# swacisko/ALGA

Measured on AMD Instinct MI355X. Metric: overlap_edges_per_sec, higher is better.
Workload: dtype u32; 1 GPU; cfg4_50M_150bp: 50000000 x 150 bp reads, genome 250000000, seed 11, err 0.00 -> 90621096 nodes (both strands, duplicates removed), min_overlap 82, rsoemo 116; generated on the device (alga_amd.workload.device_build) in 0.9 s; nodes=90621096, edges=92350115

## Files before the change

alga_amd/csrc/engine.hip:

```cpp
#include <hip/hip_runtime.h>

#include <algorithm>
#include <chrono>
#include <cstdio>
#include <cstdlib>
#include <cstring>
#include <new>
#include <string>
#include <thread>
#include <vector>

#include "engine_internal.h"
#include "prefsuf_shard.h"

using namespace alga;

namespace {

using Prepared = AlgaPrepared;

int prepare(alga_engine *e, const alga_nodes *nodes, const alga_prefsuf_params *p, hipStream_t s, Prepared &out) {
    if (!nodes || !p) return alga_fail(e, ALGA_ERR_INVALID_ARGUMENT, "nodes/params must not be NULL");
    if (nodes->n < 0) return alga_fail(e, ALGA_ERR_INVALID_ARGUMENT, "negative node count");
    if (nodes->n > 0 && (!nodes->words || !nodes->len)) return alga_fail(e, ALGA_ERR_INVALID_ARGUMENT, "words/len must not be NULL");
    if (nodes->stride_words <= 0 && nodes->n > 0) return alga_fail(e, ALGA_ERR_INVALID_ARGUMENT, "stride_words must be positive");
    if (p->min_overlap < 1 || p->min_overlap > 501) return alga_fail(e, ALGA_ERR_INVALID_ARGUMENT, "min_overlap must be in [1, 501]");
    if (p->soes != 3) return alga_fail(e, ALGA_ERR_INVALID_ARGUMENT, "soes must be 3 (the reference hard-codes SOES = 3)");
    if (p->max_len_cap < 1 || p->max_len_cap > 500) return alga_fail(e, ALGA_ERR_INVALID_ARGUMENT, "max_len_cap must be in [1, 500]");
    if (p->rsoe_min_overlap < 0) return alga_fail(e, ALGA_ERR_INVALID_ARGUMENT, "rsoe_min_overlap must be >= 0");
    if (p->keys_shared < 0 || p->keys_shared > 2) return alga_fail(e, ALGA_ERR_INVALID_ARGUMENT, "keys_shared must be 0, 1 or 2");
    int rc;
    if ((rc = alga_ensure(e, e->counters, (CNT_TOTAL + 2) * sizeof(unsigned long long)))) return rc;
    HIP_TRY(e, hipMemsetAsync(e->counters.p, 0, (CNT_TOTAL + 2) * sizeof(unsigned long long), s));
    NodesDev nd;
    nd.words = nodes->words; nd.len = nodes->len; nd.from = nodes->align_from; nd.to = nodes->align_to;
    nd.n = nodes->n; nd.stride = nodes->stride_words;
    unsigned long long *cnt = (unsigned long long *) e->counters.p;
    int *d_maxlen = (int *) (cnt + CNT_TOTAL);
    unsigned long long mask_asym = 0;
    int min_len = 0;
    if (p->keys_shared == 2 && e->store_n == nodes->n && e->store_words == (const void *) nodes->words && e->stat_len == (const void *) nodes->len &&
        e->stat_from == (const void *) nodes->align_from && e->stat_to == (const void *) nodes->align_to) {
        out.max_len = e->stat_max_len; out.live = e->stat_live; mask_asym = e->stat_mask_asym; min_len = e->stat_min_len;
    } else {
        launch_node_stats(nd, cnt, d_maxlen, s);
        if ((rc = alga_check_launch(e, "k_node_stats"))) return rc;
        HIP_TRY(e, hipMemcpyAsync(e->h_counters, e->counters.p, (CNT_TOTAL + 2) * sizeof(unsigned long long), hipMemcpyDeviceToHost, s));
        HIP_TRY(e, hipStreamSynchronize(s));
        out.max_len = (int) (e->h_counters[CNT_TOTAL] & 0xFFFFFFFFull);
        min_len = out.max_len > 0 ? 0x7FFFFFFF - (int) (e->h_counters[CNT_TOTAL] >> 32) : 0;
        out.live = e->h_counters[CNT_LIVE_NODES];
        mask_asym = e->h_counters[CNT_MASK_ASYM];
        e->stat_max_len = out.max_len; e->stat_min_len = min_len; e->stat_live = out.live; e->stat_mask_asym = mask_asym;
        e->stat_len = (const void *) nodes->len; e->stat_from = (const void *) nodes->align_from; e->stat_to = (const void *) nodes->align_to;
    }
    out.nd = nd;
    out.uniform_len = (out.max_len > 0 && min_len == out.max_len && !nodes->align_from) ? out.max_len : 0;
    if ((int64_t) blocks_of(out.max_len) > (int64_t) nodes->stride_words)
        return alga_fail(e, ALGA_ERR_INVALID_ARGUMENT, "stride_words is smaller than the longest read needs");
    if (out.max_len > OL_MAX_NODE_LEN) return alga_fail(e, ALGA_ERR_CAPACITY, "a node is longer than 4 194 303 nt (overlap records keep the offset in 22 bits)");
    PrefSufCfg c;
    c.Lmin = p->min_overlap;
    c.rsoemo = p->rsoe_min_overlap;
    c.Lcap = std::min(out.max_len, p->max_len_cap) + 1;
    c.soes = p->soes;
    const int seed_nt = std::min(c.Lmin, SEED_MAX_NT);
    c.seed_words = (2 * seed_nt + 31) >> 5;
    c.seed_last_mask = (2 * seed_nt & 31) ? ((1u << (2 * seed_nt & 31)) - 1u) : 0xFFFFFFFFu;
    c.reversed = (c.rsoemo > c.Lcap) ? 1 : 0;
    c.stats = p->collect_stats ? 1 : 0;
    out.cfg = c;
    if (p->reduction < ALGA_REDUCTION_AUTO || p->reduction > ALGA_REDUCTION_SOURCE_SIDE)
        return alga_fail(e, ALGA_ERR_INVALID_ARGUMENT, "reduction must be an alga_reduction value");
    out.local_ok = out.max_len <= p->max_len_cap && out.max_len - c.Lmin <= LOCAL_MAX_SPAN && c.Lmin <= c.rsoemo && c.rsoemo <= c.Lcap &&
                   mask_asym == 0;
    out.local_sw = out.max_len - c.Lmin <= 63 ? 1 : 2;
    out.cluster_eq = 0;
    const bool wide = out.local_sw == 2 || blocks_of(out.max_len) > 13;
    if (out.local_ok && e->opt_probe != ALGA_PROBE_TABLE && !(wide && e->opt_probe == ALGA_PROBE_AUTO && out.live < (4ull << 20))) {
        int eq = 0;
        if (cluster_plan(c, out.max_len, out.live, e->opt_cluster_bucket_bias, &out.cluster, &eq)) out.cluster_eq = eq;
    }
    out.keys_shared = p->keys_shared;
    out.reduction = p->reduction;
    if (out.reduction == ALGA_REDUCTION_AUTO && e->opt_force_per_target) out.reduction = ALGA_REDUCTION_PER_TARGET;
    return ALGA_OK;
}

int cluster_alloc(alga_engine *e, const Prepared &pp) {
    int rc;
    const uint64_t n = (uint64_t) pp.nd.n;
    for (int k = 0; k < 2; k++) {
        if ((rc = alga_ensure(e, e->cl_keys[k], (n + ALGA_KEY_ARRAY_SLACK + 1) * sizeof(uint32_t)))) return rc;
        if ((rc = alga_ensure(e, e->cl_vals[k], (n + 1) * sizeof(uint32_t)))) return rc;
    }
    if ((rc = alga_ensure(e, e->cl_meta, (n + ALGA_KEY_ARRAY_SLACK + 1) * sizeof(uint32_t)))) return rc;
    if ((rc = alga_ensure(e, e->cl_runs, (n + 1) * CL_RMAX * 8))) return rc;
    if ((rc = alga_ensure(e, e->cl_nruns, n + 16))) return rc;
    if ((rc = alga_ensure(e, e->cl_store, (n + 2) * 16 * (size_t) pp.cluster_eq))) return rc;
    if ((rc = alga_ensure(e, e->cl_dir, ((size_t) pp.cluster.n_buckets + 2) * 16))) return rc;
    return alga_ensure(e, e->sort_temp, cluster_sort_temp_bytes(n));
}

int pile_alloc(alga_engine *e, uint64_t n, uint32_t n_buckets, hipStream_t s) {
    int rc;
    if ((rc = alga_ensure(e, e->cl_pile_rec, pile_record_bytes(n)))) return rc;
    if ((rc = alga_ensure(e, e->cl_pile_rec2, pile_record_bytes(n)))) return rc;
    if ((rc = alga_ensure(e, e->cl_pile_succ, ((size_t) n + 64) * 16))) return rc;
    if ((rc = alga_ensure(e, e->cl_pile_cnt, PILE_CNT_WORDS * sizeof(unsigned long long)))) return rc;
    if ((rc = alga_ensure(e, e->cl_pile_own, pile_own_mask_bytes(n)))) return rc;
    if (e->opt_pile_runs_list && (rc = alga_ensure(e, e->cl_pile_list, pile_list_bytes(n)))) return rc;
    if ((rc = alga_ensure(e, e->cl_defer, (size_t) (n + 64) * sizeof(int32_t)))) return rc;
    const void *before = e->cl_pile_tab.p;
    const size_t cap_before = e->cl_pile_tab.cap;
    if ((rc = alga_ensure(e, e->cl_pile_tab, pile_table_bytes(n_buckets)))) return rc;
    if (e->cl_pile_tab.p != before || e->cl_pile_tab.cap != cap_before) {
        HIP_TRY(e, hipMemsetAsync(e->cl_pile_tab.p, 0, e->cl_pile_tab.cap, s));
        HIP_TRY(e, hipStreamSynchronize(s));
        e->pile_epoch = 0;
    }
    return ALGA_OK;
}

int discover_impl(alga_engine *e, const Prepared &pp, int32_t src_begin, int32_t src_end, hipStream_t s, uint64_t *n_rec, bool local = false,
                  bool *overflow = nullptr) {
    int rc;
    const NodesDev &nd = pp.nd;
    const PrefSufCfg &cfg = pp.cfg;
    unsigned long long *cnt = (unsigned long long *) e->counters.p;
    *n_rec = 0;
    HIP_TRY(e, hipEventRecord(e->ev[EV_START], s));
    if (pp.live >= (1ull << 31)) return alga_fail(e, ALGA_ERR_CAPACITY, "too many nodes for one seed table; shard the input");
    const bool clustered = local && pp.cluster_eq != 0;
    e->pairs_timed = false;
    e->store_timed = false;
    e->pile_timed = false;
    e->pile_deg_pending = false;
    const bool all_sources = src_begin == 0 && src_end == pp.nd.n;
    const bool pile_index_left = e->opt_pile_range != 0 && e->pile_n == pp.nd.n && e->pile_words == (const void *) pp.nd.words;
    bool pile = clustered && e->opt_pile != 0 && e->opt_cluster_pairs != 0 && e->opt_cluster_order != 0 && pp.local_sw == 1 &&
                      (pp.keys_shared == 0 || (pp.keys_shared == 2 && pile_index_left)) &&
                      (all_sources || (e->opt_pile_range != 0 && src_begin >= 0 && src_end <= pp.nd.n && src_begin < src_end)) && pile_plan(cfg, pp.cluster, pp.cluster_eq, pp.uniform_len, pp.nd.from != nullptr || pp.nd.to != nullptr);
    e->loc_second_used = false;
    bool keys_only = false;
    const bool need_vals = !e->opt_own_sort || e->opt_test_unsorted_index;
    uint32_t n_buckets = 0, filter_bits = 0;
    bool have_table = false;
    auto build_table = [&]() -> int {
        n_buckets = seed_buckets_for(pp.live, e->seed_fill_x10);
        const size_t table_bytes = (size_t) n_buckets * SEED_BUCKET * sizeof(unsigned long long);
        int r;
        if ((r = alga_ensure(e, e->table, table_bytes))) return r;
        HIP_TRY(e, hipMemsetAsync(e->table.p, 0xFF, table_bytes, s));
        filter_bits = seed_filter_bits_for(pp.live);
        if (filter_bits) {
            if ((r = alga_ensure(e, e->filter, filter_bits / 8))) return r;
            HIP_TRY(e, hipMemsetAsync(e->filter.p, 0, filter_bits / 8, s));
        }
        launch_seed_build(nd, cfg, (unsigned long long *) e->table.p, n_buckets, (uint32_t *) e->filter.p, filter_bits, s);
        if ((r = alga_check_launch(e, "k_seed_build"))) return r;
        e->stats.table_slots = (uint64_t) n_buckets * SEED_BUCKET;
        have_table = true;
        return ALGA_OK;
    };
    ClusterCfg cc{};
    if (clustered) {
        cc = pp.cluster;
        if ((rc = cluster_alloc(e, pp))) return rc;
        if (pp.keys_shared == 2) {
            const bool store_left = e->store_n == nd.n && e->store_words == (const void *) nd.words && e->store_eq == pp.cluster_eq && e->store_buckets == cc.n_buckets;
            const bool piles_serve = pile && e->pile_kept_pure && e->store_buckets == cc.n_buckets && e->store_eq == pp.cluster_eq;
            if (!(store_left || piles_serve) || src_begin < e->store_run_begin || src_end > e->store_run_end)
                return alga_fail(e, ALGA_ERR_INVALID_ARGUMENT, "keys_shared = 2: no entry array of this node set that covers the sources is left from the previous build");
            keys_only = pile && e->pile_keys_only;
        } else {
            int32_t run_begin = 0, run_end = nd.n;
            if (pp.keys_shared == 1) {
                if (e->keyed_n != nd.n || e->keyed_words != (const void *) nd.words || src_begin < e->keyed_begin || src_end > e->keyed_end)
                    return alga_fail(e, ALGA_ERR_INVALID_ARGUMENT, "keys_shared: alga_prefsuf_keys_device has not been called on this node set for a range that covers the sources");
                run_begin = e->keyed_begin; run_end = e->keyed_end;
            } else {
                keys_only = pile && e->opt_pile_runs != 0 && !e->expect_pairwise && !e->opt_pile_check;
                launch_cluster_keys(nd, cfg, cc, 0, nd.n, (uint32_t *) e->cl_keys[0].p, need_vals ? (uint32_t *) e->cl_vals[0].p : nullptr, (uint32_t *) e->cl_meta.p, e->cl_runs.p,
                                    (uint8_t *) e->cl_nruns.p, s, !keys_only);
                if ((rc = alga_check_launch(e, "k_node_runs"))) return rc;
            }
            HIP_TRY(e, hipEventRecord(e->ev[EV_KEYS], s));
            e->keyed_n = -1;
            e->store_n = -1;
            HIP_TRY(e, launch_cluster_sort(nd, cc, (uint32_t *) e->cl_keys[0].p, (uint32_t *) e->cl_vals[0].p, (uint32_t *) e->cl_keys[1].p,
                                           (uint32_t *) e->cl_vals[1].p, e->sort_temp.p, cluster_sort_temp_bytes((uint64_t) nd.n), pp.keys_shared == 1 || !need_vals,
                                           e->ev[EV_SORT], e->opt_test_unsorted_index != 0, s, e->opt_own_sort != 0));
            const bool dir_late = pile && e->opt_pile_dir >= 1;
            e->dir_late = dir_late;
            if (!dir_late) {
                HIP_TRY(e, launch_cluster_dir(nd, cc, (const uint32_t *) e->cl_keys[1].p, e->cl_dir.p, cnt + CNT_TOTAL + 1, nullptr, s));
                HIP_TRY(e, hipEventRecord(e->ev[EV_DIR], s));
            }
            e->pile_n = -1;
            if (pile) {
                rc = e->opt_test_pile_oom ? alga_fail(e, ALGA_ERR_OUT_OF_MEMORY, "pile_alloc (option test_pile_oom)") : pile_alloc(e, (uint64_t) nd.n, cc.n_buckets, s);
                if (rc == ALGA_ERR_OUT_OF_MEMORY) {
                    (void) hipGetLastError();
                    alga_release(e->cl_pile_tab); alga_release(e->cl_pile_rec); alga_release(e->cl_pile_rec2); alga_release(e->cl_pile_succ); alga_release(e->cl_pile_own);
                    alga_release(e->cl_pile_list);
                    e->pile_epoch = 0; e->pile_n = -1;
                    e->err.clear();
                    pile = false;
                    rc = ALGA_OK;
                    if (keys_only) {
                        launch_cluster_keys(nd, cfg, cc, 0, nd.n, (uint32_t *) e->cl_keys[0].p, (uint32_t *) e->cl_vals[0].p, (uint32_t *) e->cl_meta.p, e->cl_runs.p,
                                            (uint8_t *) e->cl_nruns.p, s, true);
                        if ((rc = alga_check_launch(e, "k_node_runs"))) return rc;
                        keys_only = false;
                    }
                } else if (rc) return rc;
            }
            if (pile) {
                launch_pile_sample(nd, cc, pp.uniform_len, (const uint32_t *) e->cl_keys[1].p, (const uint32_t *) e->cl_vals[1].p, e->cl_dir.p,
                                   (unsigned long long *) e->cl_pile_cnt.p, e->opt_pile >= 2 ? e->opt_pile - 1 : 0, s, e->opt_pile_dir >= 1);
                if ((rc = alga_check_launch(e, "k_pile_build<sample>"))) return rc;
            }
            e->pile_tab_index = pile && e->opt_pile_dir >= 2 && e->opt_pile_skip_gather && !cfg.stats;
            if (dir_late) {
                HIP_TRY(e, hipEventRecord(e->ev[EV_SAMPLE], s));
                HIP_TRY(e, launch_cluster_dir(nd, cc, (const uint32_t *) e->cl_keys[1].p, e->cl_dir.p, cnt + CNT_TOTAL + 1,
                                              e->pile_tab_index ? (const unsigned long long *) e->cl_pile_cnt.p : nullptr, s));
                HIP_TRY(e, hipEventRecord(e->ev[EV_DIR], s));
            }
            HIP_TRY(e, launch_cluster_gather(nd, cc, pp.cluster_eq, (const uint32_t *) e->cl_keys[1].p, (const uint32_t *) e->cl_vals[1].p, (const uint32_t *) e->cl_meta.p,
                                             pp.uniform_len, e->cl_store.p, (pile && e->opt_pile_skip_gather) ? (const unsigned long long *) e->cl_pile_cnt.p : nullptr, s));
            HIP_TRY(e, hipEventRecord(e->ev[EV_GATHER], s));
            if (pile) {
                if (e->pile_epoch >= 511u) {
                    HIP_TRY(e, hipMemsetAsync(e->cl_pile_tab.p, 0, e->cl_pile_tab.cap, s));
                    e->pile_epoch = 0;
                }
                e->pile_epoch++;
                const bool from_consensus = e->opt_pile_runs != 0;
                launch_pile_build(nd, cfg, cc, pp.uniform_len, (const uint32_t *) e->cl_keys[1].p, (const uint32_t *) e->cl_vals[1].p, e->cl_dir.p, e->cl_pile_rec.p, e->cl_pile_rec2.p, e->cl_pile_tab.p,
                                  e->pile_epoch, e->cl_pile_succ.p, e->cl_runs.p, pp.uniform_len - cfg.Lmin + 1, (const unsigned long long *) e->cl_pile_cnt.p,
                                  from_consensus ? (uint32_t *) e->cl_pile_own.p : nullptr, (from_consensus && e->opt_pile_runs_list) ? e->cl_pile_list.p : nullptr, s,
                                  e->opt_pile_dir >= 1, cnt + CNT_TOTAL + 1, e->pile_tab_index, e->opt_pile_runs_ahead != 0);
                if ((rc = alga_check_launch(e, "k_pile_build"))) return rc;
                if (keys_only) {
                    launch_pile_own_ids((const uint32_t *) e->cl_pile_own.p, (const uint32_t *) e->cl_vals[1].p, (uint64_t) nd.n, (int32_t *) e->cl_defer.p, (uint32_t) nd.n,
                                        (unsigned long long *) e->cl_pile_cnt.p, s);
                    launch_cluster_runs_list(nd, cfg, cc, (const int32_t *) e->cl_defer.p, (const unsigned long long *) e->cl_pile_cnt.p + 3, (uint32_t) nd.n, (uint32_t) e->n_cu * 16u,
                                             e->cl_runs.p, (uint8_t *) e->cl_nruns.p, s);
                    launch_cluster_keys(nd, cfg, cc, 0, nd.n, (uint32_t *) e->cl_keys[0].p, (uint32_t *) e->cl_vals[0].p, (uint32_t *) e->cl_meta.p, e->cl_runs.p,
                                        (uint8_t *) e->cl_nruns.p, s, true, (const unsigned long long *) e->cl_pile_cnt.p);
                    if ((rc = alga_check_launch(e, "k_node_runs (own lists)"))) return rc;
                }
                if (e->opt_pile_check && from_consensus)
                    launch_pile_check(e->cl_pile_succ.p, (uint64_t) nd.n, cc.n_buckets, e->cl_pile_tab.p, e->cl_pile_rec2.p, e->pile_epoch, e->cl_runs.p, nd.n, pp.uniform_len - cfg.Lmin + 1,
                                      (unsigned long long *) e->cl_pile_cnt.p, s);
                e->pile_n = nd.n; e->pile_words = (const void *) nd.words;
                e->pile_keys_only = keys_only; e->pile_kept_pure = false;
                e->pile_timed = nd.n > 0;
            }
            e->store_timed = nd.n > 0;
            e->store_n = pile ? -1 : nd.n;
            e->store_words = (const void *) nd.words; e->store_eq = pp.cluster_eq; e->store_buckets = cc.n_buckets;
            e->store_run_begin = run_begin; e->store_run_end = run_end;
        }
        e->stats.table_slots = cc.n_buckets;
    } else if ((rc = build_table())) return rc;
    HIP_TRY(e, hipEventRecord(e->ev[EV_SEED], s));

    const uint64_t n_src = (uint64_t) std::max<int64_t>(0, (int64_t) src_end - src_begin);
    const uint64_t slack = std::max(probe_record_slack(e->n_cu, n_src, local), clustered ? cluster_record_slack(e->n_cu, n_src) : 0);
    uint64_t &hint = local ? e->rec_cap_hint_local : e->rec_cap_hint;
    uint64_t cap = std::max<uint64_t>(hint, (local ? 2 : 16) * n_src + 4096) + slack;
    if (local) {
        if ((rc = alga_ensure(e, e->outdeg, (size_t) (n_src + 1) * sizeof(uint32_t)))) return rc;
        if ((rc = alga_ensure(e, e->loc_first, (size_t) (n_src + 1) * sizeof(unsigned long long)))) return rc;
    }
    const uint32_t big_list_cap = 1u << 20;
    if (local && (rc = alga_ensure(e, e->loc_big_list, big_list_cap * sizeof(int32_t)))) return rc;
    bool pure_streamed = false;
    for (int attempt = 0; attempt < 4; attempt++) {
        if (cap >= (1ull << 32) - 16) return alga_fail(e, ALGA_ERR_CAPACITY, "more than 2^32 overlap records; shard the input");
        if (local) HIP_TRY(e, hipMemsetAsync(e->outdeg.p, 0, (size_t) (n_src + 1) * sizeof(uint32_t), s));
        if ((rc = alga_ensure(e, e->rec_dst, cap * sizeof(uint32_t)))) return rc;
        if ((rc = alga_ensure(e, e->rec_val, cap * sizeof(unsigned long long)))) return rc;
        HIP_TRY(e, hipMemsetAsync(cnt, 0, CNT_TOTAL * sizeof(unsigned long long), s));
        ProbeBig big{(int32_t *) e->loc_big_list.p, big_list_cap, 0u, nullptr, 0u};
        e->defer_list_valid = clustered && e->opt_cluster_pairs && pp.local_sw == 1 && pp.cluster_eq <= 4;
        if (clustered) {
            if (e->opt_cluster_pairs && pp.local_sw == 1 && pp.cluster_eq <= 4) {
                if ((rc = alga_ensure(e, e->cl_defer, (size_t) (n_src + 64) * sizeof(int32_t)))) return rc;
                const uint32_t slot_stride = e->opt_stream_slots >= 4 ? (uint32_t) (n_src + 1) : 0u;
                if ((rc = alga_ensure(e, e->loc_second, (size_t) (slot_stride ? LOCAL_SLOTS_MAX - 1 : 1) * (n_src + 1) * sizeof(unsigned long long)))) return rc;
                e->loc_second_used = true;
                e->loc_slot_stride = slot_stride;
                const bool by_key = e->opt_cluster_order != 0 && src_begin == 0 && src_end == nd.n;
                const bool piled = pile && e->pile_n == nd.n && e->pile_words == (const void *) nd.words;
                if (piled) {
                    if (!all_sources) {
                        if ((rc = alga_ensure(e, e->cl_pile_side_r, (size_t) (n_src + 64) * 16))) return rc;
                        if ((rc = alga_ensure(e, e->cl_pile_cursor, 64))) return rc;
                    }
                    launch_pile_probe(nd, cfg, cc, pp.uniform_len, e->cl_pile_tab.p, e->pile_epoch, e->cl_pile_rec.p, e->cl_pile_rec2.p, e->cl_pile_succ.p,
                                      e->cl_runs.p, cnt, (uint32_t *) e->outdeg.p, (unsigned long long *) e->loc_first.p, (unsigned long long *) e->loc_second.p,
                                      (int32_t *) e->cl_defer.p, (uint32_t) n_src, (const unsigned long long *) e->cl_pile_cnt.p, e->n_cu, s, src_begin, src_end,
                                      e->cl_pile_side_r.p, (unsigned long long *) e->cl_pile_cursor.p, e->opt_pile_probe_lean != 0, e->opt_pile_probe_tail != 0);
                    if ((rc = alga_check_launch(e, "k_pile_probe"))) return rc;
                    if (keys_only)
                        launch_cluster_runs_list(nd, cfg, cc, (const int32_t *) e->cl_defer.p, cnt + CNT_DEFERRED, (uint32_t) std::min<uint64_t>(n_src + 64, 0xFFFFFFFFull),
                                                 (uint32_t) e->n_cu * 16u, e->cl_runs.p, (uint8_t *) e->cl_nruns.p, s);
                }
                launch_probe_stream(nd, cfg, cc, pp.cluster_eq, e->cl_store.p, e->cl_dir.p, e->cl_runs.p, (const uint8_t *) e->cl_nruns.p,
                                    src_begin, src_end, by_key, cnt, e->n_cu, (uint32_t *) e->outdeg.p, (unsigned long long *) e->loc_first.p,
                                    (unsigned long long *) e->loc_second.p, (int32_t *) e->cl_defer.p, (uint32_t) n_src,
                                    piled ? (const unsigned long long *) e->cl_pile_cnt.p : nullptr, s, slot_stride);
                if ((rc = alga_check_launch(e, "k_probe_stream"))) return rc;
                if (piled) {
                    if ((rc = alga_ensure(e, e->cl_defer2, (size_t) (n_src + 64) * sizeof(int32_t)))) return rc;
                    pure_streamed = launch_probe_stream_list(nd, cfg, cc, pp.cluster_eq, e->cl_store.p, e->cl_dir.p, e->cl_runs.p, (const uint8_t *) e->cl_nruns.p, (int32_t *) e->cl_defer.p,
                                             (uint32_t) n_src, cnt, e->n_cu, (uint32_t *) e->outdeg.p, (unsigned long long *) e->loc_first.p,
                                             (unsigned long long *) e->loc_second.p, (int32_t *) e->cl_defer2.p, (const unsigned long long *) e->cl_pile_cnt.p, s, slot_stride, src_begin,
                                             (const uint32_t *) e->cl_keys[1].p, (const uint32_t *) e->cl_vals[1].p, pp.uniform_len, e->opt_pile_stream_by_id != 0,
                                             e->pile_tab_index ? e->cl_pile_tab.p : nullptr, e->pile_epoch);
                    if ((rc = alga_check_launch(e, "k_probe_stream (list)"))) return rc;
                }
                HIP_TRY(e, hipEventRecord(e->ev[EV_PAIRS], s));
                e->pairs_timed = true;
                launch_probe_clustered(nd, cfg, cc, pp.cluster_eq, e->cl_store.p, e->cl_dir.p, e->cl_runs.p, (const uint8_t *) e->cl_nruns.p, 0,
                                       (int32_t) n_src, (const int32_t *) e->cl_defer.p, src_begin, (uint32_t *) e->rec_dst.p, (unsigned long long *) e->rec_val.p,
                                       cap, cnt, e->n_cu, (uint32_t *) e->outdeg.p, (unsigned long long *) e->loc_first.p, &big, cnt + CNT_DEFERRED, 1, s,
                                       (const uint32_t *) e->cl_keys[1].p, (const uint32_t *) e->cl_vals[1].p, pp.uniform_len,
                                       (piled && e->opt_pile_skip_gather) ? (const unsigned long long *) e->cl_pile_cnt.p : nullptr,
                                       (piled && e->pile_tab_index) ? e->cl_pile_tab.p : nullptr, e->pile_epoch);
                e->pile_deg_pending = piled && e->opt_pile_deg_fold != 0;
                if (piled && !e->pile_deg_pending) launch_pile_deg((int32_t) n_src, (unsigned long long *) e->loc_first.p, (uint32_t *) e->outdeg.p, (const unsigned long long *) e->cl_pile_cnt.p, s);
            } else {
                launch_probe_clustered(nd, cfg, cc, pp.cluster_eq, e->cl_store.p, e->cl_dir.p, e->cl_runs.p, (const uint8_t *) e->cl_nruns.p, src_begin,
                                       src_end, nullptr, src_begin, (uint32_t *) e->rec_dst.p, (unsigned long long *) e->rec_val.p, cap, cnt, e->n_cu,
                                       (uint32_t *) e->outdeg.p, (unsigned long long *) e->loc_first.p, &big, nullptr, pp.local_sw, s);
            }
        }
        else
            launch_probe(nd, cfg, (const unsigned long long *) e->table.p, n_buckets, (const uint32_t *) e->filter.p, filter_bits, src_begin, src_end,
                         (uint32_t *) e->rec_dst.p, (unsigned long long *) e->rec_val.p, cap, cnt, e->n_cu, local ? pp.local_sw : 0, (uint32_t *) e->outdeg.p,
                         (unsigned long long *) e->loc_first.p, local ? &big : nullptr, s);
        if ((rc = alga_check_launch(e, "k_probe_sources"))) return rc;
        HIP_TRY(e, hipEventRecord(e->ev[EV_PROBE], s));
        HIP_TRY(e, hipMemcpyAsync(e->h_counters, cnt, (CNT_TOTAL + 2) * sizeof(unsigned long long), hipMemcpyDeviceToHost, s));
        HIP_TRY(e, hipStreamSynchronize(s));
        if (clustered && e->h_counters[CNT_TOTAL + 1] != 0) {
            e->store_n = -1; e->keyed_n = -1;
            return alga_fail(e, ALGA_ERR_HIP, "clustered index: the sorted key array is not in order (entry directory invalid)");
        }
        if (local && e->h_counters[CNT_LOCAL_OVERFLOW] != 0) {
            const uint64_t n_big = e->h_counters[CNT_LOCAL_OVERFLOW], max_items = e->h_counters[CNT_LOCAL_MAXITEMS];
            const uint64_t limit = e->big_limit >= 0 ? (uint64_t) e->big_limit : (uint64_t) local_big_limit();
            if (n_big > big_list_cap || max_items > limit) { if (overflow) *overflow = true; *n_rec = 0; return ALGA_OK; }
            big.count = (uint32_t) n_big;
            big.item_cap = (uint32_t) ((max_items + 63) & ~63ull);
            if ((rc = alga_ensure(e, e->loc_big_items, probe_big_bytes(e->n_cu, big.count, pp.local_sw, big.item_cap)))) return rc;
            big.items = e->loc_big_items.p;
            if (!have_table && (rc = build_table())) return rc;
            if (e->pile_deg_pending) {
                launch_pile_deg((int32_t) n_src, (unsigned long long *) e->loc_first.p, (uint32_t *) e->outdeg.p, (const unsigned long long *) e->cl_pile_cnt.p, s);
                e->pile_deg_pending = false;
            }
            HIP_TRY(e, hipMemsetAsync(cnt + CNT_LOCAL_OVERFLOW, 0, sizeof(unsigned long long), s));
            launch_probe(nd, cfg, (const unsigned long long *) e->table.p, n_buckets, (const uint32_t *) e->filter.p, filter_bits, src_begin, src_end,
                         (uint32_t *) e->rec_dst.p, (unsigned long long *) e->rec_val.p, cap, cnt, e->n_cu, pp.local_sw, (uint32_t *) e->outdeg.p,
                         (unsigned long long *) e->loc_first.p, &big, s);
            if ((rc = alga_check_launch(e, "k_probe_sources (second pass)"))) return rc;
            HIP_TRY(e, hipEventRecord(e->ev[EV_PROBE], s));
            HIP_TRY(e, hipMemcpyAsync(e->h_counters, cnt, CNT_TOTAL * sizeof(unsigned long long), hipMemcpyDeviceToHost, s));
            HIP_TRY(e, hipStreamSynchronize(s));
            if (e->h_counters[CNT_LOCAL_OVERFLOW] != 0) { if (overflow) *overflow = true; *n_rec = 0; return ALGA_OK; }
            e->stats.big_sources = n_big;
        }
        const uint64_t need = e->h_counters[CNT_RECORDS];
        if (need <= cap) {
            *n_rec = need;
            hint = std::max<uint64_t>(hint, need + need / 16 + 4096);
            if (overflow) *overflow = false;
            if (local) { e->stats.transitive_compares = e->h_counters[CNT_TR_COMPARES]; e->stats.generic_sources = e->h_counters[CNT_LOCAL_GENERIC]; }
            e->stats.records = e->h_counters[CNT_VALID_RECORDS];
            e->stats.raw_overlaps = e->h_counters[CNT_RAW];
            e->stats.windows_probed = e->h_counters[CNT_WINDOWS];
            e->stats.slots_scanned = e->h_counters[CNT_SLOTS];
            e->stats.probe_rounds = e->h_counters[CNT_ROUNDS];
            e->stats.pile_buckets = e->h_counters[CNT_PILE_BUCKETS]; e->stats.pile_irregular = e->h_counters[CNT_PILE_IRREGULAR];
            e->stats.pile_own_lists = e->h_counters[CNT_PILE_OWN];
            if (pile && pp.keys_shared != 2 && e->pile_n == nd.n) {
                const bool kept = e->opt_pile == 2 || e->stats.pile_irregular * (uint64_t) ALGA_PILE_DECLINE_ONE_IN <= e->stats.pile_buckets;
                e->stats.pile_mixed = kept && e->stats.pile_irregular * (uint64_t) ALGA_PILE_IRREGULAR_ONE_IN > e->stats.pile_buckets;
                e->stats.pile_deferred = (e->stats.pile_mixed || (kept && pure_streamed)) ? e->h_counters[CNT_DEFERRED_PILE] : (kept ? e->h_counters[CNT_DEFERRED] : 0);
                if (!kept || e->stats.pile_mixed || !e->opt_pile_skip_gather) e->store_n = nd.n;
                e->expect_pairwise = !kept;
                e->pile_kept_pure = kept && !e->stats.pile_mixed && e->opt_pile_skip_gather != 0;
                e->stats.pile_list_checked = 0; e->stats.pile_list_mismatch = 0;
                if (e->opt_pile_check) {
                    unsigned long long chk[2] = {0ull, 0ull};
                    HIP_TRY(e, hipMemcpyAsync(chk, (const unsigned long long *) e->cl_pile_cnt.p + 4, sizeof(chk), hipMemcpyDeviceToHost, s));
                    HIP_TRY(e, hipStreamSynchronize(s));
                    e->stats.pile_list_checked = chk[0]; e->stats.pile_list_mismatch = chk[1];
                }
            }
            if (!pile) e->expect_pairwise = false;
            e->stats.probe_used = clustered ? ALGA_PROBE_CLUSTER : ALGA_PROBE_TABLE;
            if (clustered) e->stats.deferred_sources = e->defer_list_valid ? e->h_counters[CNT_DEFERRED] : n_src;
            return ALGA_OK;
        }
        cap = need + need / 16 + 4096 + slack;
    }
    return alga_fail(e, ALGA_ERR_HIP, "record buffer kept overflowing");
}

int key_bits_for(int64_t n_owned) {
    int b = 1;
    while (b < 31 && (1ll << b) < n_owned) b++;
    return std::min(32, b + 1);
}

int reduce_impl(alga_engine *e, const Prepared &pp, const uint32_t *rec_dst, const unsigned long long *rec_val, uint64_t n_rec,
                uint64_t n_valid_hint, int32_t dst_begin, int32_t dst_end, hipStream_t s, uint64_t *n_edges) {
    int rc;
    const NodesDev &nd = pp.nd;
    const PrefSufCfg &cfg = pp.cfg;
    unsigned long long *cnt = (unsigned long long *) e->counters.p;
    const int32_t n_owned = dst_end - dst_begin;
    *n_edges = 0;
    if (n_rec >= (1ull << 32) - 16) return alga_fail(e, ALGA_ERR_CAPACITY, "more than 2^32 overlap records; shard the input");
    const int bits = key_bits_for(n_owned);
    const size_t temp_bytes = sort_records_temp_bytes(n_rec, bits);
    if ((rc = alga_ensure(e, e->keys, (size_t) (n_rec + 1) * sizeof(uint32_t)))) return rc;
    if ((rc = alga_ensure(e, e->seg_key, (size_t) (n_rec + 1) * sizeof(uint32_t)))) return rc;
    if ((rc = alga_ensure(e, e->seg_val, (size_t) (n_rec + 1) * sizeof(unsigned long long)))) return rc;
    if ((rc = alga_ensure(e, e->sort_temp, temp_bytes))) return rc;
    if ((rc = alga_ensure(e, e->heads, (size_t) (n_rec + 1) * 16))) return rc;
    if ((rc = alga_ensure(e, e->rowptr, (size_t) (n_owned + 2) * sizeof(uint32_t)))) return rc;
    HIP_TRY(e, hipMemsetAsync(cnt + CNT_SORT_VALID, 0, sizeof(unsigned long long), s));
    launch_make_keys(rec_dst, n_rec, dst_begin, dst_end, (uint32_t *) e->keys.p, cnt + CNT_SORT_VALID, s);
    if ((rc = alga_check_launch(e, "k_make_keys"))) return rc;
    HIP_TRY(e, sort_records(e->sort_temp.p, temp_bytes, (const uint32_t *) e->keys.p, (uint32_t *) e->seg_key.p, rec_val,
                            (unsigned long long *) e->seg_val.p, n_rec, bits, s));
    launch_rowptr_from_sorted((const uint32_t *) e->seg_key.p, cnt + CNT_SORT_VALID, n_rec, n_owned, (uint32_t *) e->rowptr.p, s);
    if ((rc = alga_check_launch(e, "k_rowptr_from_sorted"))) return rc;
    launch_gather_heads(nd, (const unsigned long long *) e->seg_val.p, cnt + CNT_SORT_VALID, n_rec, e->heads.p, s);
    if ((rc = alga_check_launch(e, "k_gather_heads"))) return rc;
    HIP_TRY(e, hipEventRecord(e->ev[EV_GROUP], s));

    if ((rc = alga_ensure(e, e->out_cnt, (size_t) (n_owned + 1) * sizeof(uint32_t)))) return rc;
    if ((rc = alga_ensure(e, e->outdeg, (size_t) (nd.n + 1) * sizeof(uint32_t)))) return rc;
    HIP_TRY(e, hipMemsetAsync(e->outdeg.p, 0, (size_t) (nd.n + 1) * sizeof(uint32_t), s));
    const int tpb = reduce_targets_per_block(n_valid_hint, (uint64_t) std::max(1, n_owned));
    launch_reduce_targets(nd, cfg, dst_begin, n_owned, tpb, (const uint32_t *) e->rowptr.p, (unsigned long long *) e->seg_val.p,
                          e->heads.p, (uint32_t *) e->out_cnt.p, (uint32_t *) e->outdeg.p, cnt, s);
    if ((rc = alga_check_launch(e, "k_reduce_targets"))) return rc;
    HIP_TRY(e, hipEventRecord(e->ev[EV_REDUCE], s));

    if ((rc = alga_ensure(e, e->scan_scratch, scan_scratch_bytes((uint64_t) nd.n)))) return rc;
    if ((rc = alga_ensure(e, e->out_rowptr, (size_t) (nd.n + 1) * sizeof(uint32_t)))) return rc;
    launch_exclusive_scan((const uint32_t *) e->outdeg.p, (uint64_t) nd.n, (uint32_t *) e->out_rowptr.p, (uint64_t *) e->scan_scratch.p, s);
    if ((rc = alga_check_launch(e, "scan(outdeg)"))) return rc;
    uint64_t *d_total = (uint64_t *) e->scan_scratch.p + scan_total_index((uint64_t) nd.n);
    HIP_TRY(e, hipMemcpyAsync(&e->h_counters[CNT_TOTAL], d_total, sizeof(uint64_t), hipMemcpyDeviceToHost, s));
    HIP_TRY(e, hipMemcpyAsync(e->h_counters, cnt, CNT_TOTAL * sizeof(unsigned long long), hipMemcpyDeviceToHost, s));
    HIP_TRY(e, hipStreamSynchronize(s));
    const uint64_t E = e->h_counters[CNT_TOTAL];
    if (E >= (1ull << 32) - 16) return alga_fail(e, ALGA_ERR_CAPACITY, "more than 2^32 edges; shard the input");
    if ((rc = alga_ensure(e, e->edges, (size_t) (E + 1) * sizeof(alga_edge_dev)))) return rc;
    launch_scatter_by_source(cfg, dst_begin, n_owned, (const uint32_t *) e->rowptr.p, (const unsigned long long *) e->seg_val.p,
                             (const uint32_t *) e->out_cnt.p, (const uint32_t *) e->out_rowptr.p, (uint32_t *) e->outdeg.p,
                             (alga_edge_dev *) e->edges.p, s);
    if ((rc = alga_check_launch(e, "k_scatter_by_source"))) return rc;
    launch_sort_rows(nd.n, (const uint32_t *) e->out_rowptr.p, (alga_edge_dev *) e->edges.p, s);
    if ((rc = alga_check_launch(e, "k_sort_rows"))) return rc;
    HIP_TRY(e, hipEventRecord(e->ev[EV_EMIT], s));
    HIP_TRY(e, hipStreamSynchronize(s));
    *n_edges = E;
    e->stats.edges = E;
    e->stats.transitive_listed = e->h_counters[CNT_TR_LISTED];
    e->stats.transitive_compares = e->h_counters[CNT_TR_COMPARES];
    e->stats.transitive_removed = e->h_counters[CNT_TR_REMOVED];
    e->stats.max_in_records = e->h_counters[CNT_MAX_IN];
    return ALGA_OK;
}

int finalize_local(alga_engine *e, const Prepared &pp, int32_t src_begin, int32_t src_end, uint64_t n_rec, hipStream_t s, uint64_t *n_edges) {
    int rc;
    *n_edges = 0;
    const uint64_t n_src = (uint64_t) std::max<int64_t>(0, (int64_t) src_end - src_begin);
    if ((rc = alga_ensure(e, e->scan_scratch, scan_scratch_bytes(n_src)))) return rc;
    if ((rc = alga_ensure(e, e->out_rowptr, (size_t) (n_src + 1) * sizeof(uint32_t)))) return rc;
    if ((rc = alga_ensure(e, e->out_cnt, (size_t) (n_src + 1) * sizeof(uint32_t)))) return rc;
    HIP_TRY(e, hipEventRecord(e->ev[EV_GROUP], s));
    HIP_TRY(e, hipEventRecord(e->ev[EV_REDUCE], s));
    const bool fused = e->opt_emit_fused != 0;
    const unsigned long long *pile_cnt = e->pile_deg_pending ? (const unsigned long long *) e->cl_pile_cnt.p : nullptr;
    if (!fused) {
        if (e->pile_deg_pending)
            launch_exclusive_scan_pile_deg((uint32_t *) e->outdeg.p, n_src, (uint32_t *) e->out_rowptr.p, (uint64_t *) e->scan_scratch.p, (unsigned long long *) e->loc_first.p, pile_cnt, s);
        else
            launch_exclusive_scan((const uint32_t *) e->outdeg.p, n_src, (uint32_t *) e->out_rowptr.p, (uint64_t *) e->scan_scratch.p, s);
        if ((rc = alga_check_launch(e, "scan(outdeg)"))) return rc;
    }
    e->pile_deg_pending = false;
    const uint64_t E = e->stats.records;
    if (E >= (1ull << 32) - 16) return alga_fail(e, ALGA_ERR_CAPACITY, "more than 2^32 edges; shard the input");
    if ((rc = alga_ensure(e, e->edges, (size_t) (E + 1) * sizeof(alga_edge_dev)))) return rc;
    launch_local_emit(src_begin, (int32_t) n_src, (const uint32_t *) e->outdeg.p, (const unsigned long long *) e->loc_first.p,
                      e->loc_second_used ? (const unsigned long long *) e->loc_second.p : nullptr, (const uint32_t *) e->rec_dst.p, (const unsigned long long *) e->rec_val.p, n_rec, (uint32_t *) e->out_rowptr.p,
                      (uint32_t *) e->out_cnt.p, (alga_edge_dev *) e->edges.p,
                      e->defer_list_valid ? (const int32_t *) e->cl_defer.p : nullptr, (const unsigned long long *) e->counters.p + CNT_DEFERRED, (uint32_t) n_src, s,
                      e->loc_second_used ? e->loc_slot_stride : 0u, fused ? (uint64_t *) e->scan_scratch.p : nullptr, fused ? pile_cnt : nullptr);
    if ((rc = alga_check_launch(e, "k_local_emit"))) return rc;
    HIP_TRY(e, hipEventRecord(e->ev[EV_EMIT], s));
    uint64_t *d_total = (uint64_t *) e->scan_scratch.p + scan_total_index(n_src);
    HIP_TRY(e, hipMemcpyAsync(&e->h_counters[CNT_TOTAL], d_total, sizeof(uint64_t), hipMemcpyDeviceToHost, s));
    HIP_TRY(e, hipStreamSynchronize(s));
    if (e->h_counters[CNT_TOTAL] != E) return alga_fail(e, ALGA_ERR_HIP, "source-side emit: out-degrees and edge count disagree");
    *n_edges = E;
    e->stats.edges = E;
    return ALGA_OK;
}

int build_local(alga_engine *e, const Prepared &pp, int32_t src_begin, int32_t src_end, hipStream_t s, uint64_t *n_edges) {
    if (!pp.local_ok) return alga_fail(e, ALGA_ERR_UNSUPPORTED, "source-side reduction is not exact for this input (read lengths / masks / rsoemo)");
    uint64_t n_rec = 0;
    bool overflow = false;
    int rc = discover_impl(e, pp, src_begin, src_end, s, &n_rec, true, &overflow);
    if (rc) return rc;
    if (overflow) return alga_fail(e, ALGA_ERR_UNSUPPORTED, "a source node has more raw overlaps than the source-side reduction holds");
    if ((rc = finalize_local(e, pp, src_begin, src_end, n_rec, s, n_edges))) return rc;
    e->stats.reduction_used = ALGA_REDUCTION_SOURCE_SIDE;
    return ALGA_OK;
}

double now_ms_host() { return std::chrono::duration<double, std::milli>(std::chrono::steady_clock::now().time_since_epoch()).count(); }

float ev_ms(alga_engine *e, int a, int b) {
    float ms = 0.f;
    if (hipEventElapsedTime(&ms, e->ev[a], e->ev[b]) != hipSuccess) return 0.f;
    return ms;
}

void store_phase_stats(alga_engine *e) {
    if (!e->store_timed) return;
    e->stats.ms_keys = ev_ms(e, EV_START, EV_KEYS);
    e->stats.ms_sort = ev_ms(e, EV_KEYS, EV_SORT);
    e->stats.ms_dir = ev_ms(e, e->dir_late ? EV_SAMPLE : EV_SORT, EV_DIR);
    e->stats.ms_gather = ev_ms(e, EV_DIR, EV_GATHER) + (e->dir_late ? ev_ms(e, EV_SORT, EV_SAMPLE) : 0.0);
    e->stats.ms_pile = e->pile_timed ? ev_ms(e, EV_GATHER, EV_SEED) : 0.0;
}

}

int alga_prepare(alga_engine *e, const alga_nodes *nodes, const alga_prefsuf_params *p, hipStream_t s, AlgaPrepared &out) { return prepare(e, nodes, p, s, out); }
int alga_cluster_alloc(alga_engine *e, const AlgaPrepared &pp) { return cluster_alloc(e, pp); }

extern "C" {

int alga_abi_version(void) { return ALGA_AMD_ABI_VERSION; }

struct DeviceGuard {
    int prev = -1;
    DeviceGuard() { if (hipGetDevice(&prev) != hipSuccess) prev = -1; }
    ~DeviceGuard() { if (prev >= 0) (void) hipSetDevice(prev); }
};

static void engine_free_handles(alga_engine *e) {
    if (e->h_counters) (void) hipHostFree(e->h_counters);
    for (int i = 0; i < EV_COUNT; i++) if (e->ev[i]) (void) hipEventDestroy(e->ev[i]);
    if (e->own_stream) (void) hipStreamDestroy(e->own_stream);
    if (e->side_stream) (void) hipStreamDestroy(e->side_stream);
    if (e->ev_side) (void) hipEventDestroy(e->ev_side);
    e->h_counters = nullptr; e->own_stream = nullptr; e->side_stream = nullptr; e->ev_side = nullptr;
    for (int i = 0; i < EV_COUNT; i++) e->ev[i] = nullptr;
}

int alga_engine_create(int hip_device, alga_engine **out) {
    if (!out) return ALGA_ERR_INVALID_ARGUMENT;
    *out = nullptr;
    int ndev = 0;
    hipError_t err = hipGetDeviceCount(&ndev);
    if (err != hipSuccess || ndev <= 0) return ALGA_ERR_NO_DEVICE;
    if (hip_device < 0 || hip_device >= ndev) return ALGA_ERR_INVALID_ARGUMENT;
    DeviceGuard guard;
    if (hipSetDevice(hip_device) != hipSuccess) return ALGA_ERR_NO_DEVICE;
    alga_engine *e = new (std::nothrow) alga_engine();
    if (!e) return ALGA_ERR_OUT_OF_MEMORY;
    e->device = hip_device;
    memset(&e->stats, 0, sizeof(e->stats));
    hipDeviceProp_t prop;
    if (hipGetDeviceProperties(&prop, hip_device) == hipSuccess) {
        snprintf(e->dev_name, sizeof(e->dev_name), "%s (%s, %d CUs)", prop.name, prop.gcnArchName, prop.multiProcessorCount);
        if (prop.multiProcessorCount > 0) e->n_cu = prop.multiProcessorCount;
    }
    int rc = ALGA_OK;
    if (hipStreamCreateWithFlags(&e->own_stream, hipStreamNonBlocking) != hipSuccess) { e->own_stream = nullptr; rc = ALGA_ERR_HIP; }
    if (rc == ALGA_OK && hipStreamCreateWithFlags(&e->side_stream, hipStreamNonBlocking) != hipSuccess) { e->side_stream = nullptr; rc = ALGA_ERR_HIP; }
    if (rc == ALGA_OK && hipEventCreateWithFlags(&e->ev_side, hipEventDisableTiming) != hipSuccess) { e->ev_side = nullptr; rc = ALGA_ERR_HIP; }
    for (int i = 0; i < EV_COUNT && rc == ALGA_OK; i++)
        if (hipEventCreate(&e->ev[i]) != hipSuccess) { e->ev[i] = nullptr; rc = ALGA_ERR_HIP; }
    if (rc == ALGA_OK && hipHostMalloc((void **) &e->h_counters, (CNT_TOTAL + 2 + alga_engine::H_EXTRA) * sizeof(unsigned long long)) != hipSuccess) { e->h_counters = nullptr; rc = ALGA_ERR_OUT_OF_MEMORY; }
    if (rc == ALGA_OK && hipHostGetDevicePointer((void **) &e->h_counters_dev, e->h_counters, 0) != hipSuccess) rc = ALGA_ERR_HIP;
    if (rc != ALGA_OK) { engine_free_handles(e); delete e; return rc; }
    *out = e;
    return ALGA_OK;
}

void alga_engine_destroy(alga_engine *e) {
    if (!e) return;
    DeviceGuard guard;
    (void) hipSetDevice(e->device);
    if (e->own_stream) (void) hipStreamSynchronize(e->own_stream);
    if (e->side_stream) (void) hipStreamSynchronize(e->side_stream);
    for (DevBuf *b : e->owned) alga_release(*b);
    alga_release(e->up_raw);
    for (DevBuf *b : {&e->in_bytes[0], &e->in_bytes[1], &e->in_nl[0], &e->in_nl[1], &e->in_tiles, &e->in_tile_off}) alga_release(*b);
    for (DevBuf *b : {&e->sp_rowptr, &e->sp_sorted, &e->sp_list, &e->sp_cnt, &e->sp_orow, &e->sp_out, &e->sp_in}) alga_release(*b);
    alga_staging_release(e);
    for (void *&p : e->gfa_pin) { if (p) (void) hipHostFree(p); p = nullptr; }
    for (auto &kv : e->host_lists) free(kv.first);
    e->host_lists.clear();
    engine_free_handles(e);
    delete e;
}

const char *alga_last_error(const alga_engine *e) { return e ? e->err.c_str() : "no engine"; }

int alga_engine_device_name(const alga_engine *e, char *buf, size_t buflen) {
    if (!e || !buf || buflen == 0) return ALGA_ERR_INVALID_ARGUMENT;
    snprintf(buf, buflen, "%s", e->dev_name);
    return ALGA_OK;
}

int alga_engine_set_option(alga_engine *e, const char *name, int64_t value) {
    if (!e || !name) return ALGA_ERR_INVALID_ARGUMENT;
    e->err.clear();
    if (!strcmp(name, "probe")) {
        if (value < ALGA_PROBE_AUTO || value > ALGA_PROBE_CLUSTER) return alga_fail(e, ALGA_ERR_INVALID_ARGUMENT, "option probe: 0 auto, 1 table, 2 cluster");
        e->opt_probe = (int) value;
    } else if (!strcmp(name, "cluster_bucket_bias")) {
        if (value < -8 || value > 8) return alga_fail(e, ALGA_ERR_INVALID_ARGUMENT, "option cluster_bucket_bias: -8 .. 8");
        e->opt_cluster_bucket_bias = (int) value;
    } else if (!strcmp(name, "cluster_pairs")) {
        e->opt_cluster_pairs = value != 0;
    } else if (!strcmp(name, "pile")) {
        e->opt_pile = (value == 2 || value == 3) ? (int) value : (value != 0);
    } else if (!strcmp(name, "pile_runs")) {
        e->opt_pile_runs = value != 0;
    } else if (!strcmp(name, "pile_runs_list")) {
        e->opt_pile_runs_list = value != 0;
    } else if (!strcmp(name, "pile_dir")) {
        if (value < 0 || value > 2) return alga_fail(e, ALGA_ERR_INVALID_ARGUMENT, "option pile_dir: 0 directory records, 1 k_pile_build from the keys, 2 ... and no directory for a pure pile build");
        e->opt_pile_dir = (int) value;
    } else if (!strcmp(name, "pile_deg_fold")) {
        e->opt_pile_deg_fold = value != 0;
    } else if (!strcmp(name, "emit_fused")) {
        e->opt_emit_fused = value != 0;
    } else if (!strcmp(name, "pile_probe_lean")) {
        e->opt_pile_probe_lean = value != 0;
    } else if (!strcmp(name, "pile_probe_tail")) {
        e->opt_pile_probe_tail = value != 0;
    } else if (!strcmp(name, "pile_runs_ahead")) {
        e->opt_pile_runs_ahead = value != 0;
    } else if (!strcmp(name, "pile_stream_by_id")) {
        e->opt_pile_stream_by_id = value != 0;
    } else if (!strcmp(name, "pile_check")) {
        e->opt_pile_check = value != 0;
    } else if (!strcmp(name, "pile_skip_gather")) {
        e->opt_pile_skip_gather = value != 0;
    } else if (!strcmp(name, "cluster_order")) {
        e->opt_cluster_order = value != 0;
    } else if (!strcmp(name, "local_big_max")) {
        e->big_limit = value < 0 ? -1 : (int) std::min<int64_t>(value, 1 << 20);
    } else if (!strcmp(name, "shard_bucket_max")) {
        e->opt_shard_dmax = (int) std::max<int64_t>(1, std::min<int64_t>(value, 4096));
    } else if (!strcmp(name, "rsort_variant")) {
        if (value < 0 || value > 1) return alga_fail(e, ALGA_ERR_INVALID_ARGUMENT, "option rsort_variant: 0 tiles of 8192 pairs, 1 tiles of 16384 pairs");
        rsort_set_variant((int) value);
    } else if (!strcmp(name, "stream_slots")) {
        e->opt_stream_slots = value >= 4 ? 4 : 2;
    } else if (!strcmp(name, "pile_range")) {
        e->opt_pile_range = value != 0;
    } else if (!strcmp(name, "pkb_legacy")) {
        e->opt_pkb_legacy = (int) value;
    } else if (!strcmp(name, "own_sort")) {
        e->opt_own_sort = value != 0;
    } else if (!strcmp(name, "test_presort_oom")) {
        e->opt_test_presort_oom = value != 0;
    } else if (!strcmp(name, "test_pile_oom")) {
        e->opt_test_pile_oom = value != 0;
    } else if (!strcmp(name, "test_unsorted_index")) {
        e->opt_test_unsorted_index = value != 0;
    } else if (!strcmp(name, "gfa_chunk_mb")) {
        if (value < 1 || value > 4096) return alga_fail(e, ALGA_ERR_INVALID_ARGUMENT, "option gfa_chunk_mb: 1 .. 4096");
        e->opt_gfa_chunk_mb = (int) value;
    } else if (!strcmp(name, "mst_mid_nodes")) {
        if (value < 8 || value > (1 << 20)) return alga_fail(e, ALGA_ERR_INVALID_ARGUMENT, "option mst_mid_nodes: 8 .. 2^20");
        e->opt_mst_mid_nodes = (int) value;
    } else if (!strcmp(name, "consensus_max_blocks")) {
        if (value < 0 || value > (1 << 20)) return alga_fail(e, ALGA_ERR_INVALID_ARGUMENT, "option consensus_max_blocks: 0 .. 2^20");
        e->opt_consensus_max_blocks = (int) value;
    } else if (!strcmp(name, "unitig_ruling")) {
        if (value < -1 || value > 1) return alga_fail(e, ALGA_ERR_INVALID_ARGUMENT, "option unitig_ruling: -1, 0 or 1");
        e->opt_unitig_ruling = (int) value;
    } else if (!strcmp(name, "correct_slice_keys")) {
        if (value < 1 || value > (1ll << 31)) return alga_fail(e, ALGA_ERR_INVALID_ARGUMENT, "option correct_slice_keys: 1 .. 2^31");
        e->opt_correct_slice_keys = value;
    } else if (!strcmp(name, "correct_dir_bits")) {
        if (value < 0 || value > 28) return alga_fail(e, ALGA_ERR_INVALID_ARGUMENT, "option correct_dir_bits: 0 (auto) or 1 .. 28");
        e->opt_correct_dir_bits = (int) value;
    } else if (!strcmp(name, "place_dir_bits")) {
        if (value < 0 || value > 26) return alga_fail(e, ALGA_ERR_INVALID_ARGUMENT, "option place_dir_bits: 0 (auto) or 1 .. 26");
        e->opt_place_dir_bits = (int) value;
    } else if (!strcmp(name, "auto_reduction_per_target")) {
        e->opt_force_per_target = value != 0;
    } else return alga_fail(e, ALGA_ERR_INVALID_ARGUMENT, "unknown option");
    return ALGA_OK;
}

int alga_engine_reserve(alga_engine *e, int32_t n_nodes, int32_t max_len, int32_t min_overlap, uint64_t n_edges_hint) {
    if (!e) return ALGA_ERR_INVALID_ARGUMENT;
    e->err.clear();
    if (n_nodes < 0 || max_len < 1 || min_overlap < 1) return alga_fail(e, ALGA_ERR_INVALID_ARGUMENT, "alga_engine_reserve: n_nodes >= 0, max_len >= 1, min_overlap >= 1");
    DeviceGuard guard;
    HIP_TRY(e, hipSetDevice(e->device));
    int rc;
    const uint64_t n = (uint64_t) n_nodes;
    const uint64_t E = n_edges_hint ? n_edges_hint : n + n / 16 + 4096;
    if ((rc = alga_ensure(e, e->counters, (CNT_TOTAL + 2) * sizeof(unsigned long long)))) return rc;
    Prepared pp;
    pp.nd.n = n_nodes; pp.max_len = max_len; pp.live = n;
    pp.cfg.Lmin = min_overlap; pp.cfg.Lcap = std::min(max_len, 500) + 1; pp.cfg.rsoemo = min_overlap; pp.cfg.soes = 3;
    int eq = 0;
    const bool local = max_len <= 500 && max_len - min_overlap <= LOCAL_MAX_SPAN;
    const bool clustered = local && e->opt_probe != ALGA_PROBE_TABLE &&
                           cluster_plan(pp.cfg, max_len, n, e->opt_cluster_bucket_bias, &pp.cluster, &eq);
    if (clustered) {
        pp.cluster_eq = eq;
        if ((rc = cluster_alloc(e, pp))) return rc;
        if (max_len - min_overlap <= 63 && eq <= 4) {
            if ((rc = alga_ensure(e, e->cl_defer, (size_t) (n + 64) * sizeof(int32_t)))) return rc;
            if ((rc = alga_ensure(e, e->loc_second, (size_t) (e->opt_stream_slots >= 4 ? LOCAL_SLOTS_MAX - 1 : 1) * (n + 1) * sizeof(unsigned long long)))) return rc;
        }
        if (e->opt_pile != 0 && e->opt_cluster_pairs != 0 && e->opt_cluster_order != 0 && max_len - min_overlap <= 63 && pile_plan(pp.cfg, pp.cluster, eq, max_len, false)) {
            if ((rc = pile_alloc(e, n, pp.cluster.n_buckets, e->own_stream))) return rc;
        }
    } else {
        const uint32_t nb = seed_buckets_for(n, e->seed_fill_x10);
        if ((rc = alga_ensure(e, e->table, (size_t) nb * SEED_BUCKET * sizeof(unsigned long long)))) return rc;
        const uint32_t fb = seed_filter_bits_for(n);
        if (fb && (rc = alga_ensure(e, e->filter, fb / 8))) return rc;
    }
    if (local) {
        const uint64_t slack = std::max(probe_record_slack(e->n_cu, n, true), clustered ? cluster_record_slack(e->n_cu, n) : 0);
        const uint64_t cap = std::max<uint64_t>(e->rec_cap_hint_local, 2 * n + 4096) + slack;
        if ((rc = alga_ensure(e, e->outdeg, (size_t) (n + 1) * sizeof(uint32_t)))) return rc;
        if ((rc = alga_ensure(e, e->loc_first, (size_t) (n + 1) * sizeof(unsigned long long)))) return rc;
        if ((rc = alga_ensure(e, e->loc_big_list, (1u << 20) * sizeof(int32_t)))) return rc;
        if ((rc = alga_ensure(e, e->rec_dst, cap * sizeof(uint32_t)))) return rc;
        if ((rc = alga_ensure(e, e->rec_val, cap * sizeof(unsigned long long)))) return rc;
        if ((rc = alga_ensure(e, e->scan_scratch, scan_scratch_bytes(n)))) return rc;
        if ((rc = alga_ensure(e, e->out_rowptr, (size_t) (n + 1) * sizeof(uint32_t)))) return rc;
        if ((rc = alga_ensure(e, e->out_cnt, (size_t) (n + 1) * sizeof(uint32_t)))) return rc;
    }
    if ((rc = alga_ensure(e, e->edges, (size_t) (E + 1) * sizeof(alga_edge_dev)))) return rc;
    if (!e->warmed && n_nodes > 0) {
        const int W = blocks_of(max_len), stride = hbm_row_stride(W), wn = 4096;
        std::vector<uint32_t> rows((size_t) wn * stride, 0u);
        std::vector<int32_t> lens((size_t) wn, max_len);
        uint64_t x = 0x9E3779B97F4A7C15ull;
        for (int i = 0; i < wn; i++)
            for (int k = 0; k < W; k++) {
                x ^= x << 13; x ^= x >> 7; x ^= x << 17;
                uint32_t w = (uint32_t) (x >> 16);
                const int used = 2 * max_len - 32 * k;
                if (used < 32) w &= used <= 0 ? 0u : ((1u << used) - 1u);
                rows[(size_t) i * stride + k] = w;
            }
        void *d_rows = nullptr, *d_len = nullptr;
        if (hipMalloc(&d_rows, rows.size() * 4) == hipSuccess && hipMalloc(&d_len, lens.size() * 4) == hipSuccess &&
            hipMemcpy(d_rows, rows.data(), rows.size() * 4, hipMemcpyHostToDevice) == hipSuccess &&
            hipMemcpy(d_len, lens.data(), lens.size() * 4, hipMemcpyHostToDevice) == hipSuccess) {
            alga_nodes nd{(const uint32_t *) d_rows, stride, (const int32_t *) d_len, wn, nullptr, nullptr};
            alga_prefsuf_params wp;
            alga_prefsuf_default_params(&wp);
            wp.min_overlap = min_overlap; wp.rsoe_min_overlap = std::min(max_len, min_overlap + (max_len - min_overlap) / 2);
            const alga_edge *d = nullptr;
            uint64_t m = 0;
            const int wrc = alga_prefsuf_build_device(e, &nd, &wp, nullptr, &d, &m);
            (void) wrc;
            e->err.clear();
            e->warmed = true;
        }
        if (d_rows) (void) hipFree(d_rows);
        if (d_len) (void) hipFree(d_len);
        (void) hipGetLastError();
        alga_forget_node_set(e);
        memset(&e->stats, 0, sizeof(e->stats));
    }
    return ALGA_OK;
}

void alga_prefsuf_default_params(alga_prefsuf_params *p) {
    if (!p) return;
    memset(p, 0, sizeof(*p));
    p->min_overlap = 0;
    p->rsoe_min_overlap = 0;
    p->soes = 3;
    p->max_len_cap = 500;
    p->collect_stats = 0;
// ... 605 lines not shown
```

alga_amd/csrc/engine_internal.h:

```cpp
#pragma once
#include <hip/hip_runtime.h>

#include <cstdio>
#include <algorithm>
#include <string>
#include <vector>
#include <unordered_map>

#include "../../include/alga_amd.h"
#include "prefsuf_common.h"
#include "prefsuf_kernels.h"
#include "pkb_kernels.h"

struct DevBuf {
    void  *p = nullptr;
    size_t cap = 0;
};

enum { EV_START = 0, EV_SEED, EV_PROBE, EV_GROUP, EV_REDUCE, EV_EMIT, EV_PAIRS, EV_KEYS, EV_SORT, EV_GATHER, EV_DIR, EV_SAMPLE, EV_COUNT };
constexpr int ALGA_STAGE_THREADS = 8;

struct alga_engine {
    std::vector<DevBuf *> owned;
    int         device = -1;
    hipStream_t own_stream = nullptr;
    hipStream_t side_stream = nullptr;
    hipEvent_t  ev_side = nullptr;
    std::string err;
    char        dev_name[256] = {0};
    int         n_cu = 256;
    int         seed_fill_x10 = 20;
    int         opt_probe = 0;
    int         opt_cluster_bucket_bias = 0;
    int         opt_force_per_target = 0;
    int         opt_shard_dmax = 4096;
    int         opt_test_unsorted_index = 0;
    hipEvent_t  ev[EV_COUNT] = {};
    DevBuf table, filter, counters, rowptr, rec_dst, rec_val, keys, seg_key, seg_val, heads, sort_temp, out_cnt, outdeg, out_rowptr, edges, scan_scratch;
    DevBuf cl_defer;
    uint32_t h_first_hkey = 255;
    int32_t keyed_n = -1, keyed_begin = 0, keyed_end = 0;
    bool defer_list_valid = false;
    const void *keyed_words = nullptr;
    int32_t store_n = -1, store_run_begin = 0, store_run_end = 0, store_eq = 0;
    uint32_t store_buckets = 0;
    const void *store_words = nullptr;
    int stat_max_len = 0, stat_min_len = 0; uint64_t stat_live = 0; unsigned long long stat_mask_asym = 0;
    const void *stat_len = nullptr, *stat_from = nullptr, *stat_to = nullptr;
    bool   warmed = false;
    bool   pairs_timed = false;
    bool   store_timed = false;
    bool   pile_keys_only = false, pile_kept_pure = false;
    int    opt_pile_range = 1;
    int    opt_pile_skip_gather = 1;
    int    opt_pile = 1;
    int    opt_pile_runs = 1;
    int    opt_pile_runs_list = 1;
    DevBuf cl_pile_list;
    int    opt_pile_deg_fold = 1;
    int    opt_emit_fused = 1;
    int    opt_pile_dir = 2;
    bool   dir_late = false;
    bool   pile_tab_index = false;
    int    opt_pile_stream_by_id = 0;
    int    opt_pile_probe_lean = 1;
    int    opt_pile_probe_tail = 1;
    int    opt_pile_runs_ahead = 0;
    bool   pile_deg_pending = false;
    int    opt_pile_check = 0;
    bool   expect_pairwise = false;
    DevBuf cl_pile_side_r, cl_pile_cursor;
    DevBuf cl_pile_own;
    int    opt_pkb_legacy = 0;
    int    opt_own_sort = 1;
    int    opt_test_presort_oom = 0;
    int    opt_test_pile_oom = 0;
    bool   pile_timed = false;
    DevBuf cl_pile_succ;
    DevBuf cl_pile_rec2;
    DevBuf cl_pile_rec, cl_pile_cnt, cl_pile_tab;
    uint32_t pile_epoch = 0;
    int32_t pile_n = -1; const void *pile_words = nullptr;
    int    opt_cluster_order = 1;
    int    opt_cluster_pairs = 1;
    DevBuf cl_keys[2], cl_vals[2], cl_meta, cl_runs, cl_nruns, cl_store, cl_dir;
    DevBuf loc_second;
    bool   loc_second_used = false;
    uint32_t loc_slot_stride = 0;
    int    opt_stream_slots = 4;
    DevBuf loc_first, loc_big_list, loc_big_items;
    int    big_limit = -1;
    DevBuf edge_keys, edge_keys2, edge_vals, edge_vals2, edges_sorted, xs_dst, xs_val;
    DevBuf up_words, up_len, up_from, up_to;
    DevBuf up_len_narrow;
    DevBuf cp_deg, cp_dst, cp_off;
    DevBuf cl_defer2;
    DevBuf pk_keys, pk_keys2, pk_vals, pk_vals2, pk_marks, pk_big, pk_add, pk_ekeys, pk_ekeys2, pk_flag, pk_pos, pk_edges[2], pk_rowptr, pk_deg,
           pk_mask, pk_cnt, pk_io, pk_io2, pk_tips, pk_heads, pk_g[2], pk_addk, pk_addk2, pk_merged, pk_hsz, pk_hsz2, pk_heads2, pk_nadd, pk_koff,
           pk_gsz, pk_fixlist, pk_bounds, pk_tiprec, pk_tipidx, pk_keys_all, pk_vals_all;
    DevBuf pk_keys2b, pk_vals2b, pk_headsb, pk_hszb, sort_temp2, pk_fixlist2, pk_cnt2;
    DevBuf pp_rows, pp_len, pp_perm[2], pp_keys[2], pp_mark, pp_keep, pp_pos, pp_out_rows, pp_out_len, pp_out_pair, pp_tally;
    bool        stage_ready = false;
    void       *stage_pin[ALGA_STAGE_THREADS][2] = {};
    hipEvent_t  stage_ev[ALGA_STAGE_THREADS][2] = {};
    hipStream_t stage_stream[ALGA_STAGE_THREADS] = {};
    DevBuf      up_raw;
    std::unordered_map<void *, size_t> host_lists;
    void       *host_spare = nullptr;
    size_t      host_spare_cap = 0;
    DevBuf      in_bytes[2], in_nl[2], in_tiles, in_tile_off;
    DevBuf      sp_rowptr, sp_sorted, sp_list, sp_cnt, sp_orow, sp_out, sp_in;
    DevBuf      tp_cnt, tp_keys[2], tp_vals[2], tp_flag, tp_pos, tp_best, tp_est, tp_rev, tp_rfid, tp_rowptr[2], tp_alive, tp_kill, tp_rec[2], tp_branch,
                tp_overflow, tp_ws, tp_out;
    DevBuf      mp_cnt, mp_rowptr, mp_rows, mp_len, mp_owner, mp_pend[2], mp_win, mp_overflow, mp_overflow2, mp_ws, mp_ws_big, mp_orow, mp_out;
    struct MstFilled { const void *p = nullptr; size_t bytes = 0; uint32_t hbits = 0, cap_nodes = 0, cap_edges = 0; int32_t n_ws = 0; } mp_filled[2];
    int         opt_mst_mid_nodes = 4096;
    DevBuf      gfa_sizes, gfa_off, gfa_rowptr, gfa_tiles, gfa_bounds, gfa_buf;
    void       *gfa_pin[2] = {nullptr, nullptr};
    size_t      gfa_pin_cap = 0;
    int         opt_gfa_chunk_mb = 256;
    DevBuf      ut_cnt, ut_keys[2], ut_vals[2], ut_flag, ut_pos, ut_best, ut_estar, ut_rowptr, ut_nxt, ut_noff, ut_prv, ut_rank[2], ut_min[2], ut_tail,
                ut_win, ut_pair, ut_pcnt, ut_ulen, ut_ulen2, ut_uwords, ut_path_off, ut_word_off, ut_tiles, ut_path_node, ut_path_pos, ut_uid, ut_words,
                ut_edges, ut_link, ut_rnode, ut_rrec[2];
    int         opt_unitig_ruling = -1;
    uint64_t    ut_n_pairs = 0, ut_n_edges = 0;
    bool        ut_valid = false;
    int32_t     ut_n_nodes = 0;
    uint64_t    ut_total_bases = 0;
    bool        ut_is_contig = false;
    DevBuf      ex_cnt, ex_rowptr, ex_w, ex_kcnt, ex_dlink, ex_outcnt, ex_sole, ex_xhead, ex_xbase, ex_xrank, ex_uid, ex_scnt, ex_seam_off,
                ex_seam_entry, ex_pcnt, ex_uwords, ex_ulen, ex_ulen2, ex_path_off, ex_word_off, ex_path_node, ex_path_pos, ex_words, ex_edges;
    bool        ut_is_extended = false;
    DevBuf      ct_cnt, ct_B[2], ct_rowptr, ct_pflag, ct_runkey, ct_chain, ct_headchain, ct_drop, ct_flag, ct_pos, ct_keys[2], ct_vals[2], ct_hw, ct_hk, ct_H,
                ct_hrow, ct_hsorted, ct_hlist, ct_hcnt, ct_win, ct_pair, ct_oid, ct_cid, ct_deg, ct_epos, ct_ekeys[2], ct_evals[2], ct_names;
    DevBuf      cs_cnt, cs_words, cs_mask, cs_votes, cs_trim, cs_len, cs_changed;
    bool        cs_valid = false;
    bool        cs_has_votes = false;
    DevBuf      fc_cnt, fc_keys[2], fc_vals, fc_first, fc_min, fc_list[2], fc_flag, fc_ids, fc_verdict, fc_rank, fc_id, fc_new, fc_trim, fc_begin, fc_len,
                fc_order, fc_wbegin, fc_wlen, fc_rows, fc_rlen, fc_tid;
    bool        fc_valid = false;
    uint64_t    fc_n_accepted = 0;
    int         opt_consensus_max_blocks = 0;
    DevBuf      cr_cnt, cr_table, cr_hist, cr_keys[2], cr_flag, cr_pos, cr_solid, cr_dir;
    int64_t     opt_correct_slice_keys = 1ll << 28;
    int         opt_correct_dir_bits = 0;
    DevBuf      seed_keys[2], seed_vals[2], seed_dir, seed_ub;
    DevBuf      pl_cnt, pl_fbegin, pl_flen, pl_scan, pl_cols, pl_diff;
    DevBuf      pl_target, pl_pos, pl_mm, pl_hits, pl_state, pl_coloff, pl_cover, pl_tstat, pl_hist;
    bool        pl_valid = false;
    uint64_t    pl_targets = 0, pl_reads = 0;
    uint64_t    pl_ncolumns = 0, pl_nhist = 0;
    uint64_t    pl_final_epoch = 0;
    uint64_t    fc_epoch = 0;
    int         opt_place_dir_bits = 0;
    DevBuf      po_cnt, po_keys[2], po_vals[2], po_marks, po_pop, po_scan;
    DevBuf      po_coloff, po_words, po_ccols, po_cbases, po_tstat, po_counts;
    bool        po_valid = false;
    uint64_t    po_targets = 0, po_columns = 0;
    uint64_t    po_final_epoch = 0;
    uint64_t    pl_serial = 0, po_pl_serial = 0;
    DevBuf      sc_cnt, sc_keys[2], sc_vals[2], sc_span, sc_heads, sc_pos, sc_bstart, sc_best, sc_choice, sc_partner, sc_lists[2], sc_head, sc_first, sc_scan;
    DevBuf      sc_ba, sc_bb, sc_blinks, sc_bspan, sc_bgap, sc_bstate, sc_estate, sc_scaffold, sc_rank, sc_orient, sc_start, sc_gapafter, sc_jlinks, sc_soff,
                sc_smembers, sc_slen;
    bool        sc_valid = false;
    uint64_t    sc_targets = 0, sc_scaffolds = 0, sc_longest = 0;
    uint64_t    sc_pl_serial = 0;
    DevBuf      br_cnt, br_diff, br_starts, br_rpos, br_marks, br_rfirst, br_rlast, br_closed, br_cpos;
    DevBuf      br_span, br_ccols, br_cfirst, br_clast, br_tcuts, br_poff, br_begin, br_len, br_ptarget, br_pstart, br_words;
    bool        br_valid = false;
    uint64_t    br_targets = 0, br_pieces = 0, br_cuts = 0, br_columns = 0, br_longest = 0;
    DevBuf      gr_cnt, gr_flag, gr_pos, gr_cand, gr_elen, gr_eoff, gr_ecols, gr_x, gr_g;
    struct GrowSet { DevBuf end, over, mm, hits, state, count, estop, evoters, left, right, len, coloff, begin, words; } gr_set[2];
    int         gr_cur = 0;
    bool        gr_valid = false;
    uint64_t    gr_reads = 0, gr_targets = 0, gr_columns = 0, gr_longest = 0;
    DevBuf      mg_cnt, mg_elen, mg_epad, mg_eoff, mg_ecols, mg_pcols, mg_join, mg_lists[2], mg_head, mg_first, mg_scan;
    struct MergeSet { DevBuf partner, olen, mm, hits, estate, merged, rank, orient, start, ovafter, moff, mmembers, len, coloff, begin, words; } mg_set[2];
    int         mg_cur = 0;
    bool        mg_valid = false;
    uint64_t    mg_targets = 0, mg_merged = 0, mg_columns = 0, mg_longest = 0;
    DevBuf      sh_keys[2], sh_vals[2], sh_store, sh_dir, sh_desc_out, sh_dkey[2], sh_dval[2], sh_small_top, sh_pending, sh_bitmap, sh_small_out,
                sh_ssrc[2], sh_skey[2], sh_edges_out, sh_deg, sh_rowptr, sh_cursor, sh_edges, sh_flagged, sh_cnt, sh_gflag, sh_gpos, sh_gstart;
    struct {
        int      phase = 0;
        int      rank = 0, n_ranks = 1, eq = 0, uniform_len = 0;
        int32_t  n = 0;
        const void *words = nullptr;
        alga::PrefSufCfg cfg{};
        alga::ClusterCfg cc{};
        uint32_t bucket_base = 0, bpr = 0;
        uint64_t n_targets = 0, n_desc = 0, n_rec = 0;
        uint32_t *d_keys_sorted = nullptr;
        unsigned long long *d_vals_sorted = nullptr;
    } sh;
    alga_shard_stats shard_stats{};
    struct {
        int      phase = 0;
        int      rounds = 0, round = 0, rank = 0, n_ranks = 1, cur = 0, key_bits = 0;
        int32_t  prio[4] = {0, 1, 2, 3};
        uint64_t E = 0, nk = 0;
        uint32_t n_tips = 0;
        int      pre_set = 0, cur_set = 0;
        bool     no_look_ahead = false;
        int      pre_round = -1;
        bool     kmers_all = false;
        size_t   kmers_stride = 0;
        int      kmers_sort_bits = 0;
        alga_nodes dn{};
        alga::PkbCfg cfg{};
    } pkb;
    unsigned long long *h_counters = nullptr;
    static constexpr int H_EXTRA = 132 + 16, H_PRE = alga::CNT_TOTAL + 2 + 132;
    uint32_t *h_counters_dev = nullptr;
    uint64_t    rec_cap_hint = 0, rec_cap_hint_local = 0;
    alga_prefsuf_stats stats;
    double      stats_host[2] = {0.0, 0.0};
    alga_pkb_stats pkb_stats;
};

struct AlgaPrepared {
    alga::NodesDev   nd;
// ... 109 lines not shown
```

alga_amd/csrc/prefsuf_cluster_device.h:

```cpp
#pragma once
#include <hip/hip_runtime.h>
#include "prefsuf_common.h"
#include "../../include/alga_amd.h"
#include "prefsuf_device.h"

namespace alga {

__device__ __forceinline__ uint32_t kmer_hash(uint32_t lo, uint32_t hi) {
    return (lo ^ __funnelshift_l(hi, hi, 13) ^ (hi >> 7)) * 0x9E3779B1u;
}

__device__ __forceinline__ bool kmer_class0(uint32_t lo) { return (lo & 3u) == 0u && ((((lo >> 2) ^ (lo >> 3)) & 1u) != 0u); }
__device__ __forceinline__ uint32_t order_key0(uint32_t h, int pos) { return ((h >> 1) & 0x7FFFFF00u) | (uint32_t) pos; }
__device__ __forceinline__ uint32_t order_key(uint32_t h, uint32_t lo, int pos) { return order_key0(h, pos) | (kmer_class0(lo) ? 0u : 0x80000000u); }
__device__ __forceinline__ uint32_t class0_mask16(uint32_t cur, uint32_t nxt) {
    const uint32_t nx = __funnelshift_r(cur, nxt, 2);
    return ~(cur | (cur >> 1)) & (nx ^ (nx >> 1)) & 0x55555555u;
}
__device__ __forceinline__ uint32_t compress_even(uint32_t x) {
    x = (x | (x >> 1)) & 0x33333333u;
    x = (x | (x >> 2)) & 0x0F0F0F0Fu;
    x = (x | (x >> 4)) & 0x00FF00FFu;
    return (x | (x >> 8)) & 0x0000FFFFu;
}

__device__ __forceinline__ uint32_t cluster_key(uint32_t h, int fs) {
    uint32_t k = h * 0x9E3779B1u;
    k ^= k >> 15;
    k *= 0x85EBCA77u;
    k ^= k >> 13;
    k *= 0xC2B2AE3Du;
    return (k >> (fs + CL_MBITS)) == (0xFFFFFFFFu >> (fs + CL_MBITS)) ? k ^ 0x80000000u : k;
}

__device__ __forceinline__ uint32_t tgt_sort_key(uint32_t ckey, uint32_t m_c, int fs) {
    const uint32_t fm = ((1u << CL_MBITS) - 1u) << fs;
    return (ckey & ~fm) | ((m_c << fs) & fm);
}
__device__ __forceinline__ bool same_cluster(uint32_t entry_key, uint32_t ckey, int fs) {
    return ((entry_key ^ ckey) & ~(((1u << CL_MBITS) - 1u) << fs)) == 0u;
}

constexpr unsigned long long PILE_IRREGULAR_ONE_IN = ALGA_PILE_IRREGULAR_ONE_IN;
constexpr unsigned long long PILE_DECLINE_ONE_IN = ALGA_PILE_DECLINE_ONE_IN;
__device__ __forceinline__ bool pile_cnt_declines(const unsigned long long *c) { return c[1] * PILE_DECLINE_ONE_IN > c[0]; }
__device__ __forceinline__ bool pile_cnt_mixed(const unsigned long long *c) { return !pile_cnt_declines(c) && c[1] * PILE_IRREGULAR_ONE_IN > c[0]; }
__device__ __forceinline__ bool pile_cnt_pure(const unsigned long long *c) { return !pile_cnt_declines(c) && !pile_cnt_mixed(c); }
struct BucketIndex {
    const uint4 *tab;
    uint32_t epoch;
};
template <bool MAYBE_TAB>
__device__ __forceinline__ uint4 bucket_record(const uint4 *__restrict__ dir, const BucketIndex &bx, bool from_tab, uint32_t bucket) {
    if constexpr (!MAYBE_TAB) return dir[bucket];
    else {
        const uint4 *line = bx.tab + (size_t) bucket * 8;
        const uint4 *pr = from_tab ? line + 4 : dir + bucket;
        const uint32_t *pt = from_tab ? reinterpret_cast<const uint32_t *>(line + 3) + 3 : reinterpret_cast<const uint32_t *>(pr);
        const uint32_t *pf = from_tab ? reinterpret_cast<const uint32_t *>(line + 5) : reinterpret_cast<const uint32_t *>(pr);
        const uint4 r = *pr;
        const uint32_t tag = *pt, full = *pf;
        if (!from_tab) return r;
        const uint32_t n = r.x & 255u;
        const bool valid = (tag >> 23) == bx.epoch;
        return valid ? make_uint4(r.y, n == 127u ? full : n, r.z, r.w) : make_uint4(0u, 0u, 0u, 0u);
    }
}

__device__ __forceinline__ void run_slice(const uint4 &rec, uint32_t run_y, uint32_t &e0, uint32_t &cnt) {
    const int q = (int) (run_y & 255u), p0 = (int) ((run_y >> 8) & 255u), p1 = (int) ((run_y >> 16) & 255u);
    int mlo = q - p1 + 1, mhi = q - p0;
    mlo = mlo < 0 ? 0 : mlo; mhi = mhi > 63 ? 63 : mhi;
    e0 = rec.x; cnt = rec.y;
    if (mhi < mlo) { cnt = 0u; return; }
    if (rec.y > 255u) return;
    const int s0 = mlo >> 3, s1 = (mhi >> 3) + 1;
    const uint32_t b0 = ((s0 < 4 ? rec.z : rec.w) >> (8 * (s0 & 3))) & 255u;
    const uint32_t b1 = s1 >= 8 ? rec.y : (((s1 < 4 ? rec.z : rec.w) >> (8 * (s1 & 3))) & 255u);
    e0 = rec.x + b0; cnt = b1 - b0;
}

template <int RS = 1, int RW = 0>
__device__ __forceinline__ uint32_t row_word(const uint32_t *row, int k) {
    if (RW > 0) { const uint32_t v = row[(k < RW ? k : RW - 1) * RS]; return k < RW ? v : 0u; }
    return row[k * RS];
}

template <int RS = 1, int RW = 0>
__device__ __forceinline__ void kmer_key(const uint32_t *row, int i, bool valid, const ClusterCfg &cc, uint32_t &h, uint32_t &pk) {
    const int bit = 2 * i, q = bit >> 5, r = bit & 31;
    const uint32_t x0 = row_word<RS, RW>(row, q), x1 = row_word<RS, RW>(row, q + 1), x2 = row_word<RS, RW>(row, q + 2);
    const uint32_t lo = funnel(x0, x1, r) & cc.lo_mask;
    h = kmer_hash(lo, funnel(x1, x2, r) & cc.hi_mask);
    pk = valid ? order_key(h, lo, i) : 0xFFFFFFFFu;
}

constexpr int TK_ROWS = 128;
constexpr int NR_STACK = 8;

template <bool WIDE, int RCAP = CL_RMAX, int RS = 1, int RW = 0>
__device__ __forceinline__ void node_runs_core(const uint32_t *row, int nwin, bool act, const ClusterCfg &cc, uint32_t (*stk)[TK_ROWS], uint16_t (*rbuf)[TK_ROWS], int t,
                                               int &nr, bool &uncovered, bool &stack_ovf, uint32_t &cur0, int step = 64) {
    constexpr int S0 = NR_STACK + 1;
    const int w = cc.w;
    nr = 0; uncovered = false; stack_ovf = false; cur0 = 0xFFFFFFFFu;
    for (int hb = (WIDE && nwin > step) ? ((nwin - 1) / step) * step : 0; hb >= 0; hb -= step) {
        const int h0 = hb >> 4;
        auto rowh = [&](int k) -> uint32_t { return row_word<RS, RW>(row, h0 + k); };
        const int nwh = !WIDE ? nwin : (nwin - hb < step ? nwin - hb : step);
        const int nk = act ? nwh - 1 + w : 0;
        uint64_t m_lo, m_hi;
        {
            uint32_t dm[4];
#pragma unroll
            for (int d = 0; d < 4; d++) {
                const uint32_t x0 = rowh(2 * d), x1 = rowh(2 * d + 1), x2 = rowh(2 * d + 2);
                dm[d] = compress_even(class0_mask16(x0, x1)) | (compress_even(class0_mask16(x1, x2)) << 16);
            }
            m_lo = (uint64_t) dm[0] | ((uint64_t) dm[1] << 32);
            m_hi = (uint64_t) dm[2] | ((uint64_t) dm[3] << 32);
            m_lo &= nk >= 64 ? ~0ull : (nk <= 0 ? 0ull : ((1ull << nk) - 1ull));
            m_hi &= nk <= 64 ? 0ull : ((1ull << (nk - 64)) - 1ull);
        }
        uint64_t b0 = w >= 64 ? m_lo : (m_lo & ((1ull << w) - 1ull));
        uint64_t b1 = w >= 64 ? m_hi : ((m_lo >> w) | (m_hi << (64 - w)));
        auto key_at = [&](int pos) -> uint32_t {
            const int bit = 2 * pos, q = bit >> 5, r = bit & 31;
            const uint32_t x0 = rowh(q), x1 = rowh(q + 1), x2 = rowh(q + 2);
            return order_key0(kmer_hash(funnel(x0, x1, r) & cc.lo_mask, funnel(x1, x2, r) & cc.hi_mask), pos);
        };
        uint32_t cur1 = 0xFFFFFFFFu;
        int sp1 = 0;
        while (b1 != 0ull) {
            const int e = __builtin_ctzll(b1);
            b1 &= b1 - 1ull;
            const uint32_t pk = key_at(w + e);
            const bool push = pk < cur1;
            stk[(push && sp1 < NR_STACK) ? sp1 : NR_STACK][t] = pk;
            cur1 = push ? pk : cur1;
            sp1 += push ? 1 : 0;
        }
        uint32_t cur0h = 0xFFFFFFFFu;
        int sp0 = 0;
        while (b0 != 0ull) {
            const int e = 63 - __builtin_clzll(b0);
            b0 ^= 1ull << e;
            const uint32_t pk = key_at(e);
            const bool push = pk < cur0h;
            stk[S0 + ((push && sp0 < NR_STACK) ? sp0 : NR_STACK)][t] = pk;
            cur0h = push ? pk : cur0h;
            sp0 += push ? 1 : 0;
        }
        if (hb == 0) cur0 = cur0h;
        stack_ovf = stack_ovf || sp1 > NR_STACK || sp0 > NR_STACK;
        sp1 = sp1 > NR_STACK ? NR_STACK : sp1;
        sp0 = sp0 > NR_STACK ? NR_STACK : sp0;
        {
            const uint32_t hq = (uint32_t) hb | ((uint32_t) hb << 8);
            uint32_t top = sp1 > 0 ? stk[sp1 - 1][t] : 0xFFFFFFFFu;
            uint32_t nxt0 = stk[S0][t];
            uint32_t c0 = 0xFFFFFFFFu, win = top;
            int i0 = 0, p_hi = nwh - 1;
            int e0 = sp0 > 0 ? (int) (nxt0 & 255u) : -1;
            int e1 = sp1 > 0 ? (int) (top & 255u) - w : -1;
            while ((e0 > e1 ? e0 : e1) >= 0) {
                const int pe = e0 > e1 ? e0 : e1;
                const bool take0 = e0 >= e1;
                const int row_i = take0 ? S0 + i0 + 1 : (sp1 >= 2 ? sp1 - 2 : NR_STACK);
                const uint32_t v = stk[row_i][t];
                i0 += take0 ? 1 : 0;
                sp1 -= take0 ? 0 : 1;
                c0 = take0 ? nxt0 : c0;
                nxt0 = take0 ? v : nxt0;
                top = take0 ? top : (sp1 >= 1 ? v : 0xFFFFFFFFu);
                e0 = take0 ? (i0 < sp0 ? (int) (v & 255u) : -1) : e0;
                e1 = take0 ? e1 : (sp1 >= 1 ? (int) (v & 255u) - w : -1);
                const uint32_t wn = c0 < top ? c0 : top;
                const int pc = pe < p_hi ? pe : p_hi;
                const bool em = wn != win && pc < p_hi;
                rbuf[(em && nr < RCAP) ? nr : RCAP][t] = (uint16_t) (((win & 255u) | ((uint32_t) (pc + 1) << 8)) + hq);
                uncovered = uncovered || (em && win == 0xFFFFFFFFu);
                nr += em ? 1 : 0;
                p_hi = em ? pc : p_hi;
                win = wn;
            }
            if (act) {
                if (nr < RCAP) rbuf[nr][t] = (uint16_t) ((win & 255u) + hq);
                uncovered = uncovered || win == 0xFFFFFFFFu;
                nr++;
            }
        }
    }
}

__device__ __forceinline__ uint32_t bperm(uint32_t v, int src_lane) { return (uint32_t) __builtin_amdgcn_ds_bpermute(src_lane << 2, (int) v); }

}
```

alga_amd/csrc/prefsuf_kernels.h:

```cpp
#pragma once
#include <hip/hip_runtime.h>
#include <stddef.h>
#include <stdint.h>
#include "prefsuf_common.h"

namespace alga {

struct alga_edge_dev { int32_t src, dst, offset; };

void launch_restride(const uint32_t *in, int stride_in, uint32_t *out, int stride_out, uint64_t n, hipStream_t s);
void launch_widen_len(const void *in, int elem_bytes , int32_t *out, uint64_t n, hipStream_t s);
void launch_compact_edges(const alga_edge_dev *edges, int32_t n, uint64_t n_edges, uint8_t *deg, uint32_t *dst, uint8_t *off, unsigned long long *bad, hipStream_t s);
void launch_expand_twins(const uint32_t *in, int stride_in, const int32_t *len , uint32_t *out, int stride_out, uint64_t n_pairs, hipStream_t s);
void launch_node_stats(const NodesDev &nd, unsigned long long *counters, int *max_len , hipStream_t s);

uint32_t seed_buckets_for(uint64_t live_nodes, int fill_x10);
uint32_t seed_filter_bits_for(uint64_t live_nodes);
void launch_seed_build(const NodesDev &nd, const PrefSufCfg &cfg, unsigned long long *table, uint32_t n_buckets, uint32_t *filter,
                       uint32_t filter_bits, hipStream_t s);

struct ProbeBig { int32_t *list; uint32_t list_cap; uint32_t count; void *items; uint32_t item_cap; };
int    local_item_capacity();
int    local_big_limit();
size_t probe_big_bytes(int n_cu, uint32_t count, int local, uint32_t item_cap);

void launch_probe(const NodesDev &nd, const PrefSufCfg &cfg, const unsigned long long *table, uint32_t n_buckets,
                  const uint32_t *filter, uint32_t filter_bits, int32_t src_begin, int32_t src_end, uint32_t *rec_dst, unsigned long long *rec_val, uint64_t rec_cap,
                  unsigned long long *counters, int n_cu, int local , uint32_t *deg , unsigned long long *first ,
                  const ProbeBig *big , hipStream_t s);
uint64_t probe_record_slack(int n_cu, uint64_t n_src, bool local);
void launch_local_emit(int32_t src_base, int32_t n_src, const uint32_t *deg, const unsigned long long *first, const unsigned long long *second,
                       const uint32_t *rec_dst, const unsigned long long *rec_val, uint64_t n_rec, uint32_t *rowptr, uint32_t *cursor,
                       alga_edge_dev *edges, const int32_t *record_sources, const unsigned long long *record_sources_count, uint32_t record_sources_cap, hipStream_t s, uint32_t slot_stride = 0,
                       uint64_t *fused_scratch = nullptr, const unsigned long long *pile_cnt = nullptr);

bool       cluster_plan(const PrefSufCfg &cfg, int max_len, uint64_t live, int bucket_log2_bias, ClusterCfg *c, int *eq);
size_t     cluster_sort_temp_bytes(uint64_t n);
void       launch_cluster_keys(const NodesDev &nd, const PrefSufCfg &cfg, const ClusterCfg &cc, int32_t node_begin, int32_t node_end, uint32_t *keys,
                               uint32_t *vals, uint32_t *meta, void *runs, uint8_t *nruns, hipStream_t s, bool with_runs = true ,
                               const unsigned long long *only_if_declined = nullptr );
void       launch_cluster_runs_list(const NodesDev &nd, const PrefSufCfg &cfg, const ClusterCfg &cc, const int32_t *ids, const unsigned long long *count, uint32_t cap,
                                    uint32_t grid_blocks, void *runs, uint8_t *nruns, hipStream_t s);
hipError_t launch_cluster_store(const NodesDev &nd, const ClusterCfg &cc, uint32_t *keys, uint32_t *vals, uint32_t *keys2 , uint32_t *vals2, void *sort_temp,
                                size_t sort_temp_bytes, void *dir, bool fill_vals, hipEvent_t ev_sorted ,
                                unsigned long long *bad_flag ,
                                bool test_skip_sort , hipStream_t s, bool own_sort = true);
hipError_t launch_cluster_sort(const NodesDev &nd, const ClusterCfg &cc, uint32_t *keys, uint32_t *vals, uint32_t *keys2, uint32_t *vals2, void *sort_temp, size_t sort_temp_bytes,
                               bool fill_vals, hipEvent_t ev_sorted, bool test_skip_sort, hipStream_t s, bool own_sort = true);
hipError_t launch_cluster_dir(const NodesDev &nd, const ClusterCfg &cc, const uint32_t *keys2, void *dir, unsigned long long *bad_flag, const unsigned long long *only_if_no_pure_piles,
                              hipStream_t s);
hipError_t launch_cluster_gather(const NodesDev &nd, const ClusterCfg &cc, int eq, const uint32_t *keys2, const uint32_t *vals2, const uint32_t *meta,
                                 int uniform_len , void *store,
                                 const unsigned long long *pile_cnt , hipStream_t s);
uint64_t   cluster_record_slack(int n_cu, uint64_t n_src);
void       launch_probe_clustered(const NodesDev &nd, const PrefSufCfg &cfg, const ClusterCfg &cc, int eq, const void *store, const void *dir,
                                  const void *runs, const uint8_t *nruns, int32_t src_begin, int32_t src_end, const int32_t *src_list, int32_t src_base, uint32_t *rec_dst, unsigned long long *rec_val, uint64_t rec_cap,
                                  unsigned long long *counters, int n_cu, uint32_t *deg, unsigned long long *first, const ProbeBig *big,
                                  const unsigned long long *list_count ,
                                  int sw , hipStream_t s,
                                  const uint32_t *skeys = nullptr, const uint32_t *sids = nullptr, int uniform_len = 0,
                                  const unsigned long long *pile_cnt = nullptr ,
                                  const void *tab = nullptr , uint32_t epoch = 0);
void       launch_probe_stream(const NodesDev &nd, const PrefSufCfg &cfg, const ClusterCfg &cc, int eq, const void *store, const void *dir,
                               const void *runs, const uint8_t *nruns, int32_t src_begin, int32_t src_end, bool by_key ,
                               unsigned long long *counters, int n_cu, uint32_t *deg, unsigned long long *first, unsigned long long *second, int32_t *defer_list,
                               uint32_t defer_cap, const unsigned long long *pile_cnt ,
                               hipStream_t s, uint32_t slot_stride = 0 );
void       launch_pile_deg(int32_t n, unsigned long long *first, uint32_t *deg, const unsigned long long *pile_cnt, hipStream_t s);
bool       pile_plan(const PrefSufCfg &cfg, const ClusterCfg &cc, int eq, int uniform_len, bool masks);
size_t     pile_record_bytes(uint64_t n);
size_t     pile_table_bytes(uint32_t n_buckets);
void       launch_pile_sample(const NodesDev &nd, const ClusterCfg &cc, int uniform_len, const uint32_t *skeys , const uint32_t *sids , const void *dir,
                              unsigned long long *pile_cnt , int no_sample, hipStream_t s,
                              bool from_keys = false );
constexpr int PILE_CNT_WORDS = 6;
size_t     pile_own_mask_bytes(uint64_t n);
size_t     pile_list_bytes(uint64_t n);
void       launch_pile_build(const NodesDev &nd, const PrefSufCfg &cfg, const ClusterCfg &cc, int uniform_len, const uint32_t *skeys, const uint32_t *sids, const void *dir, void *rec,
                             void *rec2 , void *tab, uint32_t epoch, void *side, const void *runs, int nwin, const unsigned long long *pile_cnt,
                             uint32_t *own_mask ,
                             void *plist , hipStream_t s,
                             bool from_keys = false , unsigned long long *bad_flag = nullptr,
                             bool full_record = false ,
                             bool runs_ahead = false );
void       launch_pile_own_ids(const uint32_t *own_mask, const uint32_t *sids, uint64_t n_entries, int32_t *list, uint32_t cap, unsigned long long *pile_cnt, hipStream_t s);
void       launch_pile_check(const void *side, uint64_t n_entries, uint32_t n_buckets, const void *tab, const void *rec2, uint32_t epoch, const void *runs, int n_nodes, int nwin,
                             unsigned long long *pile_cnt, hipStream_t s);
bool       launch_probe_stream_list(const NodesDev &nd, const PrefSufCfg &cfg, const ClusterCfg &cc, int eq, const void *store, const void *dir, const void *runs, const uint8_t *nruns,
                                    int32_t *src_list, uint32_t list_cap, unsigned long long *counters, int n_cu, uint32_t *deg, unsigned long long *first,
                                    unsigned long long *second, int32_t *defer2, const unsigned long long *pile_cnt, hipStream_t s, uint32_t slot_stride = 0,
                                    int32_t src_base = 0 ,
                                    const uint32_t *skeys = nullptr, const uint32_t *sids = nullptr, int uniform_len = 0, bool by_id = false,
                                    const void *tab = nullptr , uint32_t epoch = 0);
void       launch_pile_probe(const NodesDev &nd, const PrefSufCfg &cfg, const ClusterCfg &cc, int uniform_len, const void *tab, uint32_t epoch, const void *rec, const void *rec2, const void *side,
                             const void *runs, unsigned long long *counters, uint32_t *deg, unsigned long long *first, unsigned long long *second, int32_t *defer_list,
                             uint32_t defer_cap, const unsigned long long *pile_cnt, int n_cu, hipStream_t s, int32_t src_begin, int32_t src_end,
                             void *side_range , unsigned long long *cursor ,
                             bool lean = true , bool tail = false );

size_t     rsort_u32_pairs_temp_bytes(uint64_t n);
void       rsort_set_variant(int v);
hipError_t rsort_u32_pairs(void *temp, size_t temp_bytes, const uint32_t *keys_in, uint32_t *keys_out, const uint32_t *vals_in, uint32_t *vals_out, uint64_t n,
                           int begin_bit, hipStream_t s);
size_t     sort_u32_pairs_temp_bytes(uint64_t n);
hipError_t sort_u32_pairs(void *temp, size_t temp_bytes, const uint32_t *keys_in, uint32_t *keys_out, const uint32_t *vals_in, uint32_t *vals_out,
                          uint64_t n, int begin_bit , hipStream_t s, bool own_sort = true );
size_t     rsort_u64_pairs_temp_bytes(uint64_t n);
hipError_t rsort_u64_pairs(void *temp, size_t temp_bytes, const unsigned long long *keys_in, unsigned long long *keys_out, const unsigned long long *vals_in,
                           unsigned long long *vals_out, uint64_t n, int bits, hipStream_t s);
hipError_t rsort_u32_u64(void *temp, size_t temp_bytes, const uint32_t *keys_in, uint32_t *keys_out, const unsigned long long *vals_in, unsigned long long *vals_out,
                         uint64_t n, int begin_bit, int end_bit, hipStream_t s);
size_t     sort_u64_pairs_temp_bytes(uint64_t n, int bits);
hipError_t sort_u64_pairs(void *temp, size_t temp_bytes, const unsigned long long *keys_in, unsigned long long *keys_out,
                          const unsigned long long *vals_in, unsigned long long *vals_out, uint64_t n, int bits, hipStream_t s);

void launch_make_keys(const uint32_t *rec_dst, uint64_t n_rec, int32_t dst_begin, int32_t dst_end, uint32_t *keys,
                      unsigned long long *n_valid, hipStream_t s);
size_t     sort_records_temp_bytes(uint64_t n, int bits);
hipError_t sort_records(void *temp, size_t temp_bytes, const uint32_t *keys_in, uint32_t *keys_out, const unsigned long long *vals_in,
                        unsigned long long *vals_out, uint64_t n, int bits, hipStream_t s);
void launch_rowptr_from_sorted(const uint32_t *keys, const unsigned long long *n_valid_ptr, uint64_t n_rec_max, int32_t n_owned,
                               uint32_t *rowptr, hipStream_t s);

size_t   scan_scratch_bytes(uint64_t n);
uint64_t scan_total_index(uint64_t n);
void launch_exclusive_scan(const uint32_t *in, uint64_t n, uint32_t *out, uint64_t *scratch, hipStream_t s);
void launch_exclusive_scan_pile_deg(uint32_t *deg, uint64_t n, uint32_t *out, uint64_t *scratch, unsigned long long *first, const unsigned long long *pile_cnt, hipStream_t s);
constexpr int MAIL_SEGS = 6;
struct MailSeg { const uint32_t *src; uint32_t words, dst; };
struct MailArgs {
    MailSeg seg[MAIL_SEGS];
    int n = 0;
    void add(const void *src, uint32_t words, uint32_t dst_word) { seg[n].src = (const uint32_t *) src; seg[n].words = words; seg[n].dst = dst_word; n++; }
};
void launch_mail(const MailArgs &a, uint32_t *host_block_dev, hipStream_t s);

int  reduce_targets_per_block(uint64_t n_records, uint64_t n_targets);
void launch_gather_heads(const NodesDev &nd, const unsigned long long *seg_val, const unsigned long long *n_valid_ptr, uint64_t n_rec_max,
                         void *heads , hipStream_t s);
void launch_reduce_targets(const NodesDev &nd, const PrefSufCfg &cfg, int32_t dst_begin, int32_t n_owned, int32_t targets_per_block,
                           const uint32_t *rowptr, unsigned long long *seg_val, const void *heads, uint32_t *out_cnt, uint32_t *outdeg,
                           unsigned long long *counters, hipStream_t s);
void launch_scatter_by_source(const PrefSufCfg &cfg, int32_t dst_begin, int32_t n_owned, const uint32_t *rowptr,
                              const unsigned long long *seg_val, const uint32_t *out_cnt, const uint32_t *out_rowptr, uint32_t *out_cursor,
                              alga_edge_dev *edges, hipStream_t s);
void launch_sort_rows(int32_t n, const uint32_t *out_rowptr, alga_edge_dev *edges, hipStream_t s);

void launch_edges_to_keys(const alga_edge_dev *e, uint64_t n, unsigned long long *keys, uint32_t *vals, hipStream_t s);
void launch_keys_to_edges(const unsigned long long *keys, const uint32_t *vals, uint64_t n, alga_edge_dev *e, hipStream_t s);
size_t     sort_edges_temp_bytes(uint64_t n);
hipError_t sort_edges(void *temp, size_t temp_bytes, const unsigned long long *keys_in, unsigned long long *keys_out, const uint32_t *vals_in,
                      uint32_t *vals_out, uint64_t n, int src_bits, hipStream_t s);

}
```

alga_amd/csrc/prefsuf_kernels.hip:

```cpp
#include <hip/hip_runtime.h>
#include <algorithm>
#include "prefsuf_common.h"
#include "prefsuf_kernels.h"
#include "prefsuf_device.h"
#include "prefsuf_cluster_device.h"

namespace alga {

__global__ void __launch_bounds__(256) k_node_stats(NodesDev nd, unsigned long long *counters, int *max_len) {
    __shared__ int s_max[4], s_min[4];
    __shared__ unsigned long long s_live[4];
    int m = 0, mn = 0x7FFFFFFF;
    unsigned long long live = 0, asym = 0;
    auto one = [&](int l, int64_t i) {
        m = l > m ? l : m;
        mn = (l > 0 && l < mn) ? l : mn;
        live += l > 0;
        if (nd.to && l > 0 && !nd.to[i] && (nd.from == nullptr || nd.from[i])) asym++;
    };
    const int64_t gid = (int64_t) blockIdx.x * blockDim.x + threadIdx.x, gsz = (int64_t) gridDim.x * blockDim.x;
    int64_t done = 0;
    if ((reinterpret_cast<uintptr_t>(nd.len) & 15u) == 0) {
        const int64_t nq = (int64_t) nd.n >> 2;
        const int4 *len4 = reinterpret_cast<const int4 *>(nd.len);
// ... 781 lines not shown
                const unsigned long long x = sv[i];
                const uint64_t kx = seg_key(x);
                uint32_t j = i;
                while (j > 0 && seg_key(sv[j - 1]) > kx) { sv[j] = sv[j - 1]; j--; }
                sv[j] = x;
            }
            for (uint32_t i = 0; i < k; i++) {
                const unsigned long long vb = sv[i];
                const uint32_t B = (uint32_t) vb, ol = (uint32_t) (vb >> 32);
                const int off = ol_off(ol), L = ol_len(ol);
                if (ol_small(ol)) {
                    bool found = false;
                    for (uint32_t u = 0; u < nlive; u++) {
                        const unsigned long long va = sv[u];
                        if ((uint32_t) va == B) { if (off < ol_off((uint32_t) (va >> 32))) sv[u] = vb; found = true; break; }
                    }
                    if (!found) { sv[nlive] = vb; nlive++; }
                } else {
                    if (STATS && off > 0) st_listed += nlive;
                    const uint32_t *rowB = nd.words + (size_t) B * nd.stride;
                    uint32_t w = 0;
                    for (uint32_t u = 0; u < nlive; u++) {
                        const unsigned long long va = sv[u];
                        const uint32_t A = (uint32_t) va, olA = (uint32_t) (va >> 32);
                        bool remove = (A == B);
                        if (!remove && off > 0) {
                            const int d = ol_off(olA) - off;
                            if (d >= 0) {
                                if (STATS) st_cmp++;
                                if (L - ol_len(olA) >= 0 && eq_shifted(nd.words + (size_t) A * nd.stride, rowB, d, off, nd.stride)) {
                                    remove = true;
                                    if (STATS) st_rem++;
                                }
                            }
                        }
                        if (!remove) { if (w != u) sv[w] = va; w++; }
                    }
                    sv[w] = vb;
                    nlive = w + 1;
                }
            }
        }
        out_cnt[t] = nlive;
        if (cfg.reversed) { if (nlive) outdeg[dst_begin + t] = nlive; }
        else for (uint32_t u = 0; u < nlive; u++) atomicAdd(&outdeg[(uint32_t) seg_val[gbeg + u]], 1u);
    }
    if (STATS) {
        st_listed = wave_sum_u64(st_listed); st_cmp = wave_sum_u64(st_cmp); st_rem = wave_sum_u64(st_rem);
        uint64_t mk = wave_max_u64((uint64_t) k);
        if (lane_id() == 0) {
            if (st_listed) atomicAdd(&counters[CNT_TR_LISTED], (unsigned long long) st_listed);
            if (st_cmp) atomicAdd(&counters[CNT_TR_COMPARES], (unsigned long long) st_cmp);
            if (st_rem) atomicAdd(&counters[CNT_TR_REMOVED], (unsigned long long) st_rem);
            atomicMax(&counters[CNT_MAX_IN], (unsigned long long) mk);
        }
    }
}

__global__ void __launch_bounds__(256)
k_scatter_by_source(PrefSufCfg cfg, int32_t dst_begin, int32_t n_owned, const uint32_t *__restrict__ rowptr,
                    const unsigned long long *__restrict__ seg_val, const uint32_t *__restrict__ out_cnt,
                    const uint32_t *__restrict__ out_rowptr, uint32_t *__restrict__ out_cursor, alga_edge_dev *__restrict__ edges) {
    const int t = blockIdx.x * blockDim.x + threadIdx.x;
    if (t >= n_owned) return;
    const uint32_t beg = rowptr[t], cnt = out_cnt[t];
    const int C = dst_begin + t;
    for (uint32_t u = 0; u < cnt; u++) {
        const unsigned long long v = seg_val[beg + u];
        const int A = (int) (uint32_t) v;
        const int off = ol_off((uint32_t) (v >> 32));
        const int row = cfg.reversed ? C : A;
        const int col = cfg.reversed ? A : C;
        const uint32_t pos = out_rowptr[row] + (atomicSub(&out_cursor[row], 1u) - 1u);
        edges[pos].src = row; edges[pos].dst = col; edges[pos].offset = off;
    }
}

__global__ void __launch_bounds__(256)
k_sort_rows(int32_t n, const uint32_t *__restrict__ out_rowptr, alga_edge_dev *__restrict__ edges) {
    const int a = blockIdx.x * blockDim.x + threadIdx.x;
    if (a >= n) return;
    const uint32_t beg = out_rowptr[a], k = out_rowptr[a + 1] - beg;
    alga_edge_dev *e = edges + beg;
    for (uint32_t i = 1; i < k; i++) {
        const alga_edge_dev x = e[i];
        uint32_t j = i;
        while (j > 0 && (e[j - 1].dst > x.dst || (e[j - 1].dst == x.dst && e[j - 1].offset > x.offset))) { e[j] = e[j - 1]; j--; }
        e[j] = x;
    }
}

__global__ void __launch_bounds__(256) k_edges_to_keys(const alga_edge_dev *__restrict__ e, uint64_t n, unsigned long long *__restrict__ keys,
                                                        uint32_t *__restrict__ vals) {
    for (uint64_t i = (uint64_t) blockIdx.x * blockDim.x + threadIdx.x; i < n; i += (uint64_t) gridDim.x * blockDim.x) {
        keys[i] = ((unsigned long long) (uint32_t) e[i].src << 32) | (uint32_t) e[i].dst;
        vals[i] = (uint32_t) e[i].offset;
    }
}

__global__ void __launch_bounds__(256) k_keys_to_edges(const unsigned long long *__restrict__ keys, const uint32_t *__restrict__ vals, uint64_t n,
                                                        alga_edge_dev *__restrict__ e) {
    for (uint64_t i = (uint64_t) blockIdx.x * blockDim.x + threadIdx.x; i < n; i += (uint64_t) gridDim.x * blockDim.x) {
        e[i].src = (int32_t) (keys[i] >> 32); e[i].dst = (int32_t) (uint32_t) keys[i]; e[i].offset = (int32_t) vals[i];
    }
}

__device__ __forceinline__ void local_emit_slots(int32_t src, size_t i, uint32_t dg, unsigned long long f, const unsigned long long *__restrict__ second,
                                                 uint32_t at, alga_edge_dev *__restrict__ edges, uint32_t slot_stride) {
    alga_edge_dev e;
    e.src = src; e.dst = (int32_t) (uint32_t) (f >> 32); e.offset = (int32_t) (uint32_t) f;
    edges[at] = e;
    if (dg >= 3u && dg <= (uint32_t) LOCAL_SLOTS_MAX && second != nullptr && slot_stride != 0u) {
        unsigned long long k[LOCAL_SLOTS_MAX];
        k[0] = f;
#pragma unroll
        for (int q = 1; q < LOCAL_SLOTS_MAX; q++) k[q] = (uint32_t) q < dg ? second[(size_t) (q - 1) * slot_stride + i] : ~0ull;
#pragma unroll
        for (int a = 0; a < LOCAL_SLOTS_MAX; a++)
#pragma unroll
            for (int b = (a & 1); b + 1 < LOCAL_SLOTS_MAX; b += 2) { const unsigned long long lo = min(k[b], k[b + 1]), hi = max(k[b], k[b + 1]); k[b] = lo; k[b + 1] = hi; }
#pragma unroll
        for (int q = 0; q < LOCAL_SLOTS_MAX; q++)
            if ((uint32_t) q < dg) { alga_edge_dev x; x.src = src; x.dst = (int32_t) (uint32_t) (k[q] >> 32); x.offset = (int32_t) (uint32_t) k[q]; edges[at + q] = x; }
        return;
    }
    if (dg == 2u && second != nullptr) {
        const unsigned long long g = second[i];
        alga_edge_dev e2 = e;
        e2.dst = (int32_t) (uint32_t) (g >> 32); e2.offset = (int32_t) (uint32_t) g;
        if (e2.dst < e.dst || (e2.dst == e.dst && e2.offset < e.offset)) { edges[at] = e2; e2 = e; }
        edges[at + 1] = e2;
    }
}

__global__ void __launch_bounds__(256) k_local_emit_first(int32_t src_base, int32_t n_src, const uint32_t *__restrict__ deg,
                                                           const unsigned long long *__restrict__ first, const unsigned long long *__restrict__ second,
                                                           const uint32_t *__restrict__ rowptr, alga_edge_dev *__restrict__ edges, uint32_t slot_stride) {
    const int i = blockIdx.x * blockDim.x + threadIdx.x;
    if (i >= n_src) return;
    const uint32_t dg = deg[i];
    if (dg == 0) return;
    const unsigned long long f = first[i];
    if (f == LOCAL_FIRST_NONE) return;
    local_emit_slots(src_base + i, (size_t) i, dg, f, second, rowptr[i], edges, slot_stride);
}

__device__ __forceinline__ uint32_t source_degree(uint32_t dg, bool piled, unsigned long long f) {
    if (dg != 0u) return dg;
    if (!piled || f == LOCAL_FIRST_NONE) return 0u;
    return 1u + (uint32_t) ((f >> 8) & 1ull);
}

__global__ void __launch_bounds__(SCAN_BLOCK) k_emit_tile_sums(const uint32_t *__restrict__ deg, const unsigned long long *__restrict__ first, uint64_t n,
                                                                const unsigned long long *__restrict__ pile_cnt, uint64_t *__restrict__ tile_sums) {
    __shared__ uint32_t lds[8];
    const bool piled = pile_cnt != nullptr && !pile_cnt_declines(pile_cnt);
    const uint64_t base = (uint64_t) blockIdx.x * SCAN_TILE;
    uint32_t s = 0;
    if (base + SCAN_TILE <= n && (reinterpret_cast<uintptr_t>(deg) & 15u) == 0 && (reinterpret_cast<uintptr_t>(first) & 15u) == 0) {
        constexpr int G = SCAN_ITEMS / 4;
        const uint4 *d4 = reinterpret_cast<const uint4 *>(deg + base);
        const ulonglong2 *f2 = reinterpret_cast<const ulonglong2 *>(first + base);
        uint4 v[G];
#pragma unroll
        for (int k = 0; k < G; k++) v[k] = d4[k * SCAN_BLOCK + threadIdx.x];
#pragma unroll
        for (int k = 0; k < G; k++) {
            const int g = 2 * (k * SCAN_BLOCK + (int) threadIdx.x);
            ulonglong2 a = make_ulonglong2(LOCAL_FIRST_NONE, LOCAL_FIRST_NONE), b = a;
            if (piled && (v[k].x == 0u || v[k].y == 0u)) a = f2[g];
            if (piled && (v[k].z == 0u || v[k].w == 0u)) b = f2[g + 1];
            s += source_degree(v[k].x, piled, a.x) + source_degree(v[k].y, piled, a.y) + source_degree(v[k].z, piled, b.x) + source_degree(v[k].w, piled, b.y);
        }
    } else {
        for (int k = 0; k < SCAN_ITEMS; k++) {
            const uint64_t i = base + (uint64_t) k * SCAN_BLOCK + threadIdx.x;
            if (i < n) { const uint32_t dg = deg[i]; s += source_degree(dg, piled, (piled && dg == 0u) ? first[i] : LOCAL_FIRST_NONE); }
        }
    }
    uint32_t tot;
    block_exclusive_scan(s, &tot, lds);
    if (threadIdx.x == 0) tile_sums[blockIdx.x] = tot;
}

__global__ void __launch_bounds__(1024) k_scan_spine_serial(uint64_t *tile_sums, uint32_t n_tiles) {
    __shared__ uint64_t lds[16];
    const int lane = lane_id(), wave = (int) (threadIdx.x >> 6);
    const uint64_t per = ((uint64_t) n_tiles + 1023u) / 1024u;
    const uint64_t beg = min((uint64_t) threadIdx.x * per, (uint64_t) n_tiles), end = min(beg + per, (uint64_t) n_tiles);
    uint64_t sum = 0;
    for (uint64_t i = beg; i < end; i++) sum += tile_sums[i];
    uint64_t inc = sum;
#pragma unroll
    for (int o = 1; o < 64; o <<= 1) {
        const uint32_t lo = (uint32_t) __shfl_up((int) (uint32_t) inc, o), hi = (uint32_t) __shfl_up((int) (uint32_t) (inc >> 32), o);
        if (lane >= o) inc += ((uint64_t) hi << 32) | lo;
    }
    if (lane == 63) lds[wave] = inc;
    __syncthreads();
    uint64_t run = inc - sum;
    for (int w = 0; w < wave; w++) run += lds[w];
    for (uint64_t i = beg; i < end; i++) { const uint64_t v = tile_sums[i]; tile_sums[i] = run; run += v; }
    if (threadIdx.x == 1023) tile_sums[n_tiles] = run;
}

__global__ void __launch_bounds__(SCAN_BLOCK) k_emit_scan_tiles(int32_t src_base, uint64_t n, const uint32_t *__restrict__ deg, const unsigned long long *__restrict__ first,
                                                                 const unsigned long long *__restrict__ second, const unsigned long long *__restrict__ pile_cnt,
                                                                 const uint64_t *__restrict__ tile_sums, uint32_t *__restrict__ out, alga_edge_dev *__restrict__ edges,
                                                                 uint32_t slot_stride) {
    __shared__ uint32_t lds[8];
    const bool piled = pile_cnt != nullptr && !pile_cnt_declines(pile_cnt);
    const int lane = lane_id(), wave = (int) (threadIdx.x >> 6);
    const uint64_t wbase = (uint64_t) blockIdx.x * SCAN_TILE + (uint64_t) wave * (64 * SCAN_ITEMS) + (uint64_t) lane;
    uint32_t d[SCAN_ITEMS];
    unsigned long long f[SCAN_ITEMS];
#pragma unroll
    for (int k = 0; k < SCAN_ITEMS; k++) { const uint64_t i = wbase + 64u * k; d[k] = i < n ? deg[i] : 0u; }
#pragma unroll
    for (int k = 0; k < SCAN_ITEMS; k++) { const uint64_t i = wbase + 64u * k; f[k] = (i < n && (piled || d[k] != 0u)) ? first[i] : LOCAL_FIRST_NONE; }
    uint32_t sum = 0;
#pragma unroll
    for (int k = 0; k < SCAN_ITEMS; k++) {
        const uint32_t dk = source_degree(d[k], piled, f[k]);
        if (d[k] == 0u && dk != 0u) f[k] &= 0xFFFFFFFF000000FFull;
        d[k] = dk; sum += dk;
    }
    sum = (uint32_t) wave_sum_u64(sum);
    if (lane == 0) lds[wave] = sum;
    __syncthreads();
    uint32_t run = (uint32_t) tile_sums[blockIdx.x];
    for (int w = 0; w < wave; w++) run += lds[w];
#pragma unroll
    for (int k = 0; k < SCAN_ITEMS; k++) {
        const uint64_t i = wbase + 64u * k;
        uint32_t inc = d[k];
#pragma unroll
        for (int o = 1; o < 64; o <<= 1) { const uint32_t t = (uint32_t) __shfl_up((int) inc, o); if (lane >= o) inc += t; }
        const uint32_t at = run + inc - d[k];
        run += (uint32_t) __shfl((int) inc, 63);
        if (i < n) {
            out[i] = at;
            if (d[k] != 0u && f[k] != LOCAL_FIRST_NONE) local_emit_slots(src_base + (int32_t) i, (size_t) i, d[k], f[k], second, at, edges, slot_stride);
        }
    }
    if (blockIdx.x == gridDim.x - 1 && threadIdx.x == 0) out[n] = (uint32_t) tile_sums[gridDim.x];
}

__global__ void __launch_bounds__(256) k_zero_cursors_list(const int32_t *__restrict__ list, const unsigned long long *__restrict__ count, uint32_t cap, int32_t src_base,
                                                            uint32_t *__restrict__ cursor) {
    unsigned long long m = *count;
    if (m > (unsigned long long) cap) m = cap;
    for (unsigned long long q = (unsigned long long) blockIdx.x * blockDim.x + threadIdx.x; q < m; q += (unsigned long long) gridDim.x * blockDim.x) cursor[list[q] - src_base] = 0u;
}

__global__ void __launch_bounds__(256) k_sort_rows_list(const int32_t *__restrict__ list, const unsigned long long *__restrict__ count, uint32_t cap, int32_t src_base,
                                                         const uint32_t *__restrict__ out_rowptr, alga_edge_dev *__restrict__ edges) {
    unsigned long long m = *count;
    if (m > (unsigned long long) cap) m = cap;
    for (unsigned long long q = (unsigned long long) blockIdx.x * blockDim.x + threadIdx.x; q < m; q += (unsigned long long) gridDim.x * blockDim.x) {
        const int a = list[q] - src_base;
        const uint32_t beg = out_rowptr[a], k = out_rowptr[a + 1] - beg;
        alga_edge_dev *e = edges + beg;
        for (uint32_t i = 1; i < k; i++) {
            const alga_edge_dev x = e[i];
            uint32_t j = i;
            while (j > 0 && (e[j - 1].dst > x.dst || (e[j - 1].dst == x.dst && e[j - 1].offset > x.offset))) { e[j] = e[j - 1]; j--; }
            e[j] = x;
        }
    }
}

__global__ void __launch_bounds__(256) k_local_emit_records(int32_t src_base, const uint32_t *__restrict__ rec_dst,
                                                             const unsigned long long *__restrict__ rec_val, uint64_t n_rec,
                                                             const uint32_t *__restrict__ rowptr, uint32_t *__restrict__ cursor,
                                                             alga_edge_dev *__restrict__ edges) {
    for (uint64_t i = (uint64_t) blockIdx.x * blockDim.x + threadIdx.x; i < n_rec; i += (uint64_t) gridDim.x * blockDim.x) {
        const uint32_t c = rec_dst[i];
        if (c == REC_INVALID) continue;
        const unsigned long long v = rec_val[i];
        const int32_t src = (int32_t) (uint32_t) v;
        alga_edge_dev e;
        e.src = src; e.dst = (int32_t) c; e.offset = ol_off((uint32_t) (v >> 32));
        edges[rowptr[src - src_base] + atomicAdd(&cursor[src - src_base], 1u)] = e;
    }
}

__global__ void __launch_bounds__(256) k_restride(const uint32_t *__restrict__ in, int stride_in, uint32_t *__restrict__ out, int stride_out, uint64_t n) {
    const uint64_t total = n * (uint64_t) stride_out;
    for (uint64_t i = (uint64_t) blockIdx.x * blockDim.x + threadIdx.x; i < total; i += (uint64_t) gridDim.x * blockDim.x) {
        const uint64_t r = i / (uint64_t) stride_out;
        const int c = (int) (i - r * (uint64_t) stride_out);
        out[i] = c < stride_in ? in[r * (uint64_t) stride_in + c] : 0u;
    }
}

__device__ __forceinline__ uint32_t nuc_revcomp32(uint32_t x) {
    x = __brev(x);
    x = ((x >> 1) & 0x55555555u) | ((x & 0x55555555u) << 1);
    return ~x;
}
__global__ void __launch_bounds__(256) k_expand_twins(const uint32_t *__restrict__ in, int stride_in, const int32_t *__restrict__ len, uint32_t *__restrict__ out, int stride_out,
                                                       uint64_t n_pairs) {
    const uint64_t total = n_pairs * (uint64_t) stride_out;
    for (uint64_t i = (uint64_t) blockIdx.x * blockDim.x + threadIdx.x; i < total; i += (uint64_t) gridDim.x * blockDim.x) {
        const uint64_t k = i / (uint64_t) stride_out;
        const int c = (int) (i - k * (uint64_t) stride_out);
        const uint32_t *row = in + k * (uint64_t) stride_in;
        out[(2 * k + 1) * (uint64_t) stride_out + c] = c < stride_in ? row[c] : 0u;
        const int n = len[2 * k];
        uint32_t v = 0u;
        if (n > 0) {
            const int wn = (2 * n + 31) >> 5, pad = 32 * wn - 2 * n;
            if (c < wn) {
                const uint32_t f0 = (wn - 1 - c) < stride_in ? nuc_revcomp32(row[wn - 1 - c]) : 0u;
                const uint32_t f1 = (c + 1 < wn && (wn - 2 - c) < stride_in) ? nuc_revcomp32(row[wn - 2 - c]) : 0u;
                v = pad ? ((f0 >> pad) | (f1 << (32 - pad))) : f0;
            }
        }
        out[(2 * k) * (uint64_t) stride_out + c] = v;
    }
}

template <typename T>
__global__ void __launch_bounds__(256) k_widen_len(const T *__restrict__ in, int32_t *__restrict__ out, uint64_t n) {
    for (uint64_t i = (uint64_t) blockIdx.x * blockDim.x + threadIdx.x; i < n; i += (uint64_t) gridDim.x * blockDim.x) out[i] = (int32_t) in[i];
}

__global__ void __launch_bounds__(256) k_compact_edges(const alga_edge_dev *__restrict__ edges, int32_t n, uint64_t n_edges,
                                                       uint8_t *__restrict__ deg, uint32_t *__restrict__ dst, uint8_t *__restrict__ off, unsigned long long *__restrict__ bad) {
    bool b = false;
    for (uint64_t i = (uint64_t) blockIdx.x * blockDim.x + threadIdx.x; i < n_edges; i += (uint64_t) gridDim.x * blockDim.x) {
        const alga_edge_dev e = edges[i];
        dst[i] = (uint32_t) e.dst; off[i] = (uint8_t) e.offset;
        b = b || (uint32_t) e.offset > 255u || e.src < 0 || e.src >= n;
        if ((i == 0 || edges[i - 1].src != e.src) && e.src >= 0 && e.src < n) {
            uint32_t d = 1;
            while (i + d < n_edges && d < 256u && edges[i + d].src == e.src) d++;
            deg[e.src] = (uint8_t) d;
            b = b || d > 255u;
        }
    }
    if (b) atomicOr(bad, 1ull);
}

static inline unsigned grid_for(uint64_t n, int block) { return (unsigned) ((n + (uint64_t) block - 1) / (uint64_t) block); }

void launch_widen_len(const void *in, int elem_bytes, int32_t *out, uint64_t n, hipStream_t s) {
    if (n == 0) return;
    const dim3 g((unsigned) std::min<uint64_t>((n + 255) / 256, 1u << 16)), b(256);
    if (elem_bytes == 1) hipLaunchKernelGGL((k_widen_len<uint8_t>), g, b, 0, s, (const uint8_t *) in, out, n);
    else hipLaunchKernelGGL((k_widen_len<uint16_t>), g, b, 0, s, (const uint16_t *) in, out, n);
}

void launch_compact_edges(const alga_edge_dev *edges, int32_t n, uint64_t n_edges, uint8_t *deg, uint32_t *dst, uint8_t *off, unsigned long long *bad, hipStream_t s) {
    if (n > 0) (void) hipMemsetAsync(deg, 0, (size_t) n, s);
    if (n_edges == 0) return;
    hipLaunchKernelGGL(k_compact_edges, dim3((unsigned) std::min<uint64_t>((n_edges + 255) / 256, 1u << 16)), dim3(256), 0, s, edges, n, n_edges, deg, dst, off, bad);
}

void launch_expand_twins(const uint32_t *in, int stride_in, const int32_t *len, uint32_t *out, int stride_out, uint64_t n_pairs, hipStream_t s) {
    if (n_pairs == 0) return;
    hipLaunchKernelGGL(k_expand_twins, dim3((unsigned) std::min<uint64_t>((n_pairs * (uint64_t) stride_out + 255) / 256, 1u << 16)), dim3(256), 0, s, in, stride_in, len, out,
                       stride_out, n_pairs);
}

void launch_restride(const uint32_t *in, int stride_in, uint32_t *out, int stride_out, uint64_t n, hipStream_t s) {
    if (n == 0) return;
    hipLaunchKernelGGL(k_restride, dim3((unsigned) std::min<uint64_t>((n * (uint64_t) stride_out + 255) / 256, 1u << 16)), dim3(256), 0, s, in, stride_in, out, stride_out, n);
}

void launch_node_stats(const NodesDev &nd, unsigned long long *counters, int *max_len, hipStream_t s) {
    if (nd.n <= 0) return;
    unsigned g = std::min<unsigned>(grid_for((uint64_t) nd.n, 256), 1024u);
    hipLaunchKernelGGL(k_node_stats, dim3(g), dim3(256), 0, s, nd, counters, max_len);
}

uint32_t seed_buckets_for(uint64_t live, int fill_x10) {
    if (fill_x10 < 5) fill_x10 = 5;
    if (fill_x10 > 60) fill_x10 = 60;
    uint64_t nb = (live * 10 + (uint64_t) fill_x10 - 1) / (uint64_t) fill_x10;
    if (nb < 64) nb = 64;
    return (uint32_t) std::min<uint64_t>(nb, 0x7FFFFFFFull);
}

uint32_t seed_filter_bits_for(uint64_t live) {
    const uint64_t want = live * 8;
    uint64_t bits = 1ull << 16;
    while (bits < want) bits <<= 1;
    if (bits <= (1ull << 25)) return (uint32_t) bits;
    if (live < (1ull << 24)) return 0;
    return (uint32_t) std::min<uint64_t>(bits, 1ull << 30);
}

void launch_seed_build(const NodesDev &nd, const PrefSufCfg &cfg, unsigned long long *table, uint32_t n_buckets, uint32_t *filter,
                       uint32_t filter_bits, hipStream_t s) {
    if (nd.n <= 0) return;
    hipLaunchKernelGGL(k_seed_build, dim3(grid_for((uint64_t) nd.n, 256)), dim3(256), 0, s, nd, cfg, table, n_buckets,
                       filter_bits ? filter : nullptr, filter_bits ? filter_bits - 1 : 0u);
}

static uint64_t probe_blocks(int n_cu, uint64_t n_src) {
    return std::max<uint64_t>(1, std::min<uint64_t>((n_src + PROBE_WAVES - 1) / PROBE_WAVES, (uint64_t) std::max(1, n_cu) * 8));
}

int local_item_capacity() { return ITEMMAX; }
int local_big_limit() { return ITEM_BIG_MAX; }
size_t probe_big_bytes(int n_cu, uint32_t count, int local, uint32_t item_cap) {
    return probe_blocks(n_cu, (uint64_t) count) * PROBE_WAVES * (size_t) item_cap * (8 + 16 * (size_t) local) + 64;
}

uint64_t probe_record_slack(int n_cu, uint64_t n_src, bool local) {
    return probe_blocks(n_cu, n_src) * PROBE_WAVES * (uint64_t) (local ? REC_CHUNK_LOCAL : REC_CHUNK);
}

struct ProbeTable { const unsigned long long *table; uint32_t n_buckets; const uint32_t *filter; uint32_t filter_mask; };

template <int NQ, int LOCAL>
static void launch_probe_nql(const NodesDev &nd, const PrefSufCfg &cfg, const ProbeTable &t,
                             int32_t src_begin, int32_t src_end, const ProbeOut &o, dim3 grid, dim3 block, hipStream_t s) {
    if constexpr (LOCAL != 0) {
        if (o.big_count) {
            hipLaunchKernelGGL((k_probe_sources<true, NQ, LOCAL, true>), grid, block, 0, s, nd, cfg, t.table, t.n_buckets, t.filter, t.filter_mask, src_begin, src_end, o);
            return;
        }
    }
    if (cfg.stats) hipLaunchKernelGGL((k_probe_sources<true, NQ, LOCAL>), grid, block, 0, s, nd, cfg, t.table, t.n_buckets, t.filter, t.filter_mask, src_begin, src_end, o);
    else           hipLaunchKernelGGL((k_probe_sources<false, NQ, LOCAL>), grid, block, 0, s, nd, cfg, t.table, t.n_buckets, t.filter, t.filter_mask, src_begin, src_end, o);
}
template <int NQ>
static void launch_probe_nq(const NodesDev &nd, const PrefSufCfg &cfg, const ProbeTable &t, int local,
                            int32_t src_begin, int32_t src_end, const ProbeOut &o, dim3 grid, dim3 block, hipStream_t s) {
    if (local == 1)      launch_probe_nql<NQ, 1>(nd, cfg, t, src_begin, src_end, o, grid, block, s);
    else if (local == 2) launch_probe_nql<NQ, 2>(nd, cfg, t, src_begin, src_end, o, grid, block, s);
    else                 launch_probe_nql<NQ, 0>(nd, cfg, t, src_begin, src_end, o, grid, block, s);
}

void launch_probe(const NodesDev &nd, const PrefSufCfg &cfg, const unsigned long long *table, uint32_t n_buckets,
                  const uint32_t *filter, uint32_t filter_bits,
                  int32_t src_begin, int32_t src_end, uint32_t *rec_dst, unsigned long long *rec_val, uint64_t rec_cap,
                  unsigned long long *counters, int n_cu, int local, uint32_t *deg, unsigned long long *first, const ProbeBig *big, hipStream_t s) {
    const int64_t ns = (int64_t) src_end - src_begin;
    if (ns <= 0) return;
    const bool second = local && big && big->count > 0;
    dim3 grid((unsigned) probe_blocks(n_cu, second ? (uint64_t) big->count : (uint64_t) ns)), block(PROBE_WAVES * 64);
    ProbeOut o{rec_dst, rec_val, rec_cap, counters, deg, first, src_begin};
    if (local && big) {
        o.big_list = big->list; o.big_list_cap = big->list_cap;
        if (second) {
            const size_t items = (size_t) grid.x * PROBE_WAVES * (size_t) big->item_cap;
            o.big_count = big->count;
            o.bigO = (uint4 *) big->items;
            o.bigC = (uint32_t *) (o.bigO + items * (size_t) local);
            o.bigM = o.bigC + items;
            o.big_cap = big->item_cap;
        }
    }
    ProbeTable t{table, n_buckets, filter_bits ? filter : nullptr, filter_bits ? filter_bits - 1 : 0u};
    const int need_q = (((2 * cfg.Lcap + 31) >> 5) + 3) >> 2;
    const bool aligned = (nd.stride & 3) == 0 && ((uintptr_t) nd.words & 15u) == 0;
    const int row_q = nd.stride >> 2;
    if (aligned && need_q <= 2 && row_q >= 2)      launch_probe_nq<2>(nd, cfg, t, local, src_begin, src_end, o, grid, block, s);
    else if (aligned && need_q <= 3 && row_q >= 3) launch_probe_nq<3>(nd, cfg, t, local, src_begin, src_end, o, grid, block, s);
    else if (aligned && need_q <= 4 && row_q >= 4) launch_probe_nq<4>(nd, cfg, t, local, src_begin, src_end, o, grid, block, s);
    else                                           launch_probe_nq<0>(nd, cfg, t, local, src_begin, src_end, o, grid, block, s);
}

void launch_local_emit(int32_t src_base, int32_t n_src, const uint32_t *deg, const unsigned long long *first, const unsigned long long *second,
                       const uint32_t *rec_dst, const unsigned long long *rec_val, uint64_t n_rec, uint32_t *rowptr, uint32_t *cursor,
                       alga_edge_dev *edges, const int32_t *record_sources, const unsigned long long *record_sources_count, uint32_t record_sources_cap, hipStream_t s,
                       uint32_t slot_stride, uint64_t *fused_scratch, const unsigned long long *pile_cnt) {
    if (n_src <= 0) {
        if (fused_scratch) launch_exclusive_scan(deg, 0, rowptr, fused_scratch, s);
        return;
    }
    if (record_sources) hipLaunchKernelGGL(k_zero_cursors_list, dim3(std::min<unsigned>(grid_for((uint64_t) record_sources_cap, 256), 2048u)), dim3(256), 0, s, record_sources, record_sources_count,
                                           record_sources_cap, src_base, cursor);
    else (void) hipMemsetAsync(cursor, 0, (size_t) (n_src + 1) * sizeof(uint32_t), s);
    if (fused_scratch) {
        const uint32_t tiles = (uint32_t) (((uint64_t) n_src + SCAN_TILE - 1) / SCAN_TILE);
        hipLaunchKernelGGL(k_emit_tile_sums, dim3(tiles), dim3(SCAN_BLOCK), 0, s, deg, first, (uint64_t) n_src, pile_cnt, fused_scratch);
        hipLaunchKernelGGL(k_scan_spine_serial, dim3(1), dim3(1024), 0, s, fused_scratch, tiles);
        hipLaunchKernelGGL(k_emit_scan_tiles, dim3(tiles), dim3(SCAN_BLOCK), 0, s, src_base, (uint64_t) n_src, deg, first, second, pile_cnt, (const uint64_t *) fused_scratch, rowptr, edges,
                           slot_stride);
    } else hipLaunchKernelGGL(k_local_emit_first, dim3(grid_for((uint64_t) n_src, 256)), dim3(256), 0, s, src_base, n_src, deg, first, second, (const uint32_t *) rowptr, edges, slot_stride);
    if (n_rec) {
        unsigned g = std::min<unsigned>(grid_for(n_rec, 256), 4096u);
        hipLaunchKernelGGL(k_local_emit_records, dim3(std::max(1u, g)), dim3(256), 0, s, src_base, rec_dst, rec_val, n_rec, rowptr, cursor, edges);
    }
    if (record_sources) {
        if (n_rec) hipLaunchKernelGGL(k_sort_rows_list, dim3(std::min<unsigned>(grid_for((uint64_t) record_sources_cap, 256), 2048u)), dim3(256), 0, s, record_sources, record_sources_count,
                                      record_sources_cap, src_base, rowptr, edges);
    } else hipLaunchKernelGGL(k_sort_rows, dim3(grid_for((uint64_t) n_src, 256)), dim3(256), 0, s, n_src, rowptr, edges);
}

void launch_make_keys(const uint32_t *rec_dst, uint64_t n_rec, int32_t dst_begin, int32_t dst_end, uint32_t *keys,
                      unsigned long long *n_valid, hipStream_t s) {
    if (n_rec == 0) return;
    unsigned g = std::min<unsigned>(grid_for(n_rec, 256 * 4), 4096u);
    hipLaunchKernelGGL(k_make_keys, dim3(std::max(1u, g)), dim3(256), 0, s, rec_dst, n_rec, dst_begin, dst_end, keys, n_valid);
}

void launch_rowptr_from_sorted(const uint32_t *keys, const unsigned long long *n_valid_ptr, uint64_t n_rec_max, int32_t n_owned,
                               uint32_t *rowptr, hipStream_t s) {
    unsigned g = std::min<unsigned>(grid_for(n_rec_max + 1, 256), 8192u);
    hipLaunchKernelGGL(k_rowptr_from_sorted, dim3(std::max(1u, g)), dim3(256), 0, s, keys, n_valid_ptr, n_owned, rowptr);
}

size_t scan_scratch_bytes(uint64_t n) {
    uint64_t tiles = (n + SCAN_TILE - 1) / SCAN_TILE;
    return (size_t) (tiles + 2) * sizeof(uint64_t);
}

void launch_exclusive_scan(const uint32_t *in, uint64_t n, uint32_t *out, uint64_t *scratch, hipStream_t s) {
    if (n == 0) { (void) hipMemsetAsync(out, 0, sizeof(uint32_t), s); (void) hipMemsetAsync(scratch, 0, 2 * sizeof(uint64_t), s); return; }
    const uint32_t tiles = (uint32_t) ((n + SCAN_TILE - 1) / SCAN_TILE);
    hipLaunchKernelGGL(k_scan_tile_sums, dim3(tiles), dim3(SCAN_BLOCK), 0, s, in, n, scratch);
    hipLaunchKernelGGL(k_scan_spine, dim3(1), dim3(1024), 0, s, scratch, tiles);
    hipLaunchKernelGGL(k_scan_tiles, dim3(tiles), dim3(SCAN_BLOCK), 0, s, in, n, scratch, out);
}

void launch_exclusive_scan_pile_deg(uint32_t *deg, uint64_t n, uint32_t *out, uint64_t *scratch, unsigned long long *first, const unsigned long long *pile_cnt, hipStream_t s) {
    if (n == 0) { launch_exclusive_scan(deg, n, out, scratch, s); return; }
    const uint32_t tiles = (uint32_t) ((n + SCAN_TILE - 1) / SCAN_TILE);
    hipLaunchKernelGGL(k_scan_tile_sums_pile_deg, dim3(tiles), dim3(SCAN_BLOCK), 0, s, deg, n, scratch, first, pile_cnt);
    hipLaunchKernelGGL(k_scan_spine, dim3(1), dim3(1024), 0, s, scratch, tiles);
    hipLaunchKernelGGL(k_scan_tiles, dim3(tiles), dim3(SCAN_BLOCK), 0, s, (const uint32_t *) deg, n, scratch, out);
}

uint64_t scan_total_index(uint64_t n) { return (n + SCAN_TILE - 1) / SCAN_TILE; }

__global__ void __launch_bounds__(256) k_mail(MailArgs a, uint32_t *__restrict__ dst) {
    for (int i = 0; i < a.n; i++)
        for (uint32_t w = threadIdx.x; w < a.seg[i].words; w += 256) dst[a.seg[i].dst + w] = a.seg[i].src[w];
}

void launch_mail(const MailArgs &a, uint32_t *host_block_dev, hipStream_t s) {
    if (a.n > 0) hipLaunchKernelGGL(k_mail, dim3(1), dim3(256), 0, s, a, host_block_dev);
}

int reduce_targets_per_block(uint64_t n_records, uint64_t n_targets) {
    const double avg = n_targets ? (double) n_records / (double) n_targets : 0.0;
    int tpb = avg > 0 ? (int) (0.6 * RED_CAP / avg) : RED_BLOCK;
    return std::max(16, std::min(RED_BLOCK, tpb));
}

void launch_gather_heads(const NodesDev &nd, const unsigned long long *seg_val, const unsigned long long *n_valid_ptr, uint64_t n_rec_max,
                         void *heads, hipStream_t s) {
    if (n_rec_max == 0) return;
    unsigned g = std::min<unsigned>(grid_for(n_rec_max, 256), 16384u);
    hipLaunchKernelGGL(k_gather_heads, dim3(std::max(1u, g)), dim3(256), 0, s, nd, seg_val, n_valid_ptr, (uint4 *) heads);
}

void launch_reduce_targets(const NodesDev &nd, const PrefSufCfg &cfg, int32_t dst_begin, int32_t n_owned, int32_t targets_per_block,
                           const uint32_t *rowptr, unsigned long long *seg_val, const void *heads, uint32_t *out_cnt, uint32_t *outdeg,
                           unsigned long long *counters, hipStream_t s) {
    if (n_owned <= 0) return;
    dim3 grid(grid_for((uint64_t) n_owned, targets_per_block)), block(RED_BLOCK);
    if (cfg.stats)
        hipLaunchKernelGGL(k_reduce_targets<true>, grid, block, 0, s, nd, cfg, dst_begin, n_owned, targets_per_block, rowptr, seg_val,
                           (const uint4 *) heads, out_cnt, outdeg, counters);
    else
        hipLaunchKernelGGL(k_reduce_targets<false>, grid, block, 0, s, nd, cfg, dst_begin, n_owned, targets_per_block, rowptr, seg_val,
                           (const uint4 *) heads, out_cnt, outdeg, counters);
}

void launch_scatter_by_source(const PrefSufCfg &cfg, int32_t dst_begin, int32_t n_owned, const uint32_t *rowptr,
                              const unsigned long long *seg_val, const uint32_t *out_cnt, const uint32_t *out_rowptr, uint32_t *out_cursor,
                              alga_edge_dev *edges, hipStream_t s) {
    if (n_owned <= 0) return;
    hipLaunchKernelGGL(k_scatter_by_source, dim3(grid_for((uint64_t) n_owned, 256)), dim3(256), 0, s, cfg, dst_begin, n_owned, rowptr, seg_val,
                       out_cnt, out_rowptr, out_cursor, edges);
}

void launch_edges_to_keys(const alga_edge_dev *e, uint64_t n, unsigned long long *keys, uint32_t *vals, hipStream_t s) {
    if (n == 0) return;
    hipLaunchKernelGGL(k_edges_to_keys, dim3(std::min<unsigned>(grid_for(n, 256), 8192u)), dim3(256), 0, s, e, n, keys, vals);
}

void launch_keys_to_edges(const unsigned long long *keys, const uint32_t *vals, uint64_t n, alga_edge_dev *e, hipStream_t s) {
    if (n == 0) return;
    hipLaunchKernelGGL(k_keys_to_edges, dim3(std::min<unsigned>(grid_for(n, 256), 8192u)), dim3(256), 0, s, keys, vals, n, e);
}

void launch_sort_rows(int32_t n, const uint32_t *out_rowptr, alga_edge_dev *edges, hipStream_t s) {
    if (n <= 0) return;
    hipLaunchKernelGGL(k_sort_rows, dim3(grid_for((uint64_t) n, 256)), dim3(256), 0, s, n, out_rowptr, edges);
}

}
```

alga_amd/csrc/prefsuf_pile.hip:

```cpp
#include <hip/hip_runtime.h>
#include <algorithm>
#include "prefsuf_common.h"
#include "prefsuf_kernels.h"
#include "prefsuf_device.h"
#include "prefsuf_cluster_device.h"

namespace alga {

constexpr int PB_TILE = 192, PB_HALO = 64, PB_THREADS = PB_TILE + PB_HALO;
constexpr int PILE_SW = 13;
constexpr int PILE_MAXSUB = 4;
constexpr int PILE_EQ = 3;

__device__ __forceinline__ bool pile_declines(const unsigned long long *pile_cnt) { return pile_cnt_declines(pile_cnt); }

__device__ __forceinline__ uint32_t pile_who(uint32_t group, uint32_t w, uint32_t n_buckets, uint64_t n_entries) {
    return group == 0u ? min(w, n_buckets) : (uint32_t) min((uint64_t) w, n_entries) | 0x80000000u;
}

__device__ __forceinline__ void load_row9(const NodesDev &nd, uint32_t id, uint32_t (&row)[9]) {
    const uint32_t *rp = nd.words + (size_t) id * nd.stride;
    if ((nd.stride & 3) == 0 && nd.stride >= 12 && ((uintptr_t) nd.words & 15u) == 0) {
        const uint4 v0 = reinterpret_cast<const uint4 *>(rp)[0], v1 = reinterpret_cast<const uint4 *>(rp)[1];
        row[0] = v0.x; row[1] = v0.y; row[2] = v0.z; row[3] = v0.w; row[4] = v1.x; row[5] = v1.y; row[6] = v1.z; row[7] = v1.w;
// ... 871 lines not shown
        const bool home = (!LEAN || PP_HOME_ANY_SLOT || a == 0) && on && row_from_pile && !got_row && ((ry[a] >> 8) & 255u) == 0u;
        got_row = got_row || home;
        take_record(li * PP_LSTRIDE, ((unsigned long long) R3.z << 32) | R3.y, a, 0u, ry[a], on, home);
    }
    dfr = dfr || (active && !got_row);
    more = dfr ? 0u : more;
    auto first_entry_of = [&](uint32_t m) -> uint32_t {
        const int a = m != 0u ? __builtin_ctz(m) >> 2 : 0;
        uint32_t ka = 0u;
#pragma unroll
        for (int k = 0; k < CL_RMAX; k++) ka |= rk[k] & (0u - (uint32_t) (a == k));
        return reinterpret_cast<const uint32_t *>(tab)[(size_t) (m != 0u ? min(ka >> cc.idx_shift, cc.n_buckets) : cc.n_buckets) * 32 + 17];
    };
    uint32_t xa_next = 0u;
    if constexpr (TAIL) xa_next = first_entry_of(more);
    {
        const uint4 *rp = run_list_of(next_side);
#pragma unroll
        for (int c = 0; c < CL_RMAX / 2; c++) Qr[c] = rp[c];
    }
    while (__ballot(more != 0u) != 0ull) {
        const bool on = more != 0u;
        const int bit = on ? __builtin_ctz(more) : 0;
        more &= more - 1u;
        const int a = bit >> 2;
        const uint32_t g = (uint32_t) (bit & 3);
        uint32_t ya = ry[0], ka = rk[0];
#pragma unroll
        for (int k = 1; k < CL_RMAX; k++) { ya = a == k ? ry[k] : ya; ka = a == k ? rk[k] : ka; }
        const uint32_t xa = TAIL ? xa_next : reinterpret_cast<const uint32_t *>(tab)[(size_t) min(ka >> cc.idx_shift, cc.n_buckets) * 32 + 17];
        const uint64_t se = min((uint64_t) xa + g, last);
        const uint4 Q0 = rec[se * 4], Q1 = rec[se * 4 + 1], Q2 = rec[se * 4 + 2], Q3 = rec[se * 4 + 3];
        if constexpr (TAIL) xa_next = first_entry_of(more);
        uint4 *mine = reinterpret_cast<uint4 *>(sl + lane * PP_LSTRIDE);
        mine[0] = Q0; mine[1] = Q1; mine[2] = Q2; mine[3] = Q3;
        wave_lds_fence();
        take_record(lane * PP_LSTRIDE, ((unsigned long long) Q3.w << 32) | Q3.z, a, g, ya, on, false);
        wave_lds_fence();
    }
    const unsigned long long kept = occ & ~smear_up(occ, G);
    const int nkept = __popcll(kept);
    if (nkept > 2) dfr = true;
    auto lookup = [&](int d) -> uint32_t {
        uint32_t ya = 0u, ka = 0u, ga = 0u;
#pragma unroll
        for (int k = 0; k < CL_RMAX; k++) {
            const bool in = ((vmask >> k) & 1u) != 0u && d >= (int) ((ry[k] >> 8) & 255u) && d < (int) ((ry[k] >> 16) & 255u);
            ya = in ? ry[k] : ya; ka = in ? rk[k] : ka; ga = in ? (grp >> (2 * k)) & 3u : ga;
        }
        const uint4 dd = tab[(size_t) min(ka >> cc.idx_shift, cc.n_buckets) * 8 + 4];
        const int mm = (int) (ya & 255u) - d;
        const int cl = (mm >> 3) & 7;
        const uint32_t b0 = ((cl < 4 ? dd.z : dd.w) >> (8 * (cl & 3))) & 255u;
        const uint32_t b1 = cl >= 7 ? (dd.x & 127u) : ((((cl + 1) < 4 ? dd.z : dd.w) >> (8 * ((cl + 1) & 3))) & 255u);
        uint32_t id = 0xFFFFFFFFu;
        for (uint32_t e = b0; e < b1 && e < 64u; e++) {
            const uint64_t ei = min((uint64_t) dd.y + e, last);
            const uint4 sd = side[ei];
            if ((int) ((sd.z >> 8) & 63u) == mm && ((sd.z >> 16) & 3u) == ga) id = sd.x;
        }
        return id;
    };
    uint32_t lk_id1 = 0xFFFFFFFFu, lk_id2 = 0xFFFFFFFFu;
    if constexpr (TAIL) {
        const bool fin = active && !dfr && nkept > 0;
        const int d1 = fin ? __builtin_ctzll(kept) : 0, d2 = (fin && nkept == 2) ? 63 - __clzll((long long) kept) : 0;
        uint32_t y1 = 0u, k1 = 0u, g1 = 0u, y2 = 0u, k2 = 0u, g2 = 0u;
        int p1_home = 0;
#pragma unroll
        for (int k = 0; k < CL_RMAX; k++) {
            const bool v = ((vmask >> k) & 1u) != 0u;
            const int p0 = (int) ((ry[k] >> 8) & 255u), p1 = (int) ((ry[k] >> 16) & 255u);
            const uint32_t gk = (grp >> (2 * k)) & 3u;
            p1_home = (v && p0 == 0) ? p1 : p1_home;
            const bool in1 = v && d1 >= p0 && d1 < p1, in2 = v && d2 >= p0 && d2 < p1;
            y1 = in1 ? ry[k] : y1; k1 = in1 ? rk[k] : k1; g1 = in1 ? gk : g1;
            y2 = in2 ? ry[k] : y2; k2 = in2 ? rk[k] : k2; g2 = in2 ? gk : g2;
        }
        const bool need1 = fin && !(d1 < p1_home && (int) (my.z & 255u) == d1 && my.y != 0xFFFFFFFFu), need2 = fin && nkept == 2;
        if (__ballot(need1 || need2) != 0ull) {
            uint4 dd1 = tab[(size_t) (need1 ? min(k1 >> cc.idx_shift, cc.n_buckets) : cc.n_buckets) * 8 + 4];
            uint4 dd2 = tab[(size_t) (need2 ? min(k2 >> cc.idx_shift, cc.n_buckets) : cc.n_buckets) * 8 + 4];
            asm volatile("" : "+v"(dd1.x), "+v"(dd1.y), "+v"(dd1.z), "+v"(dd1.w), "+v"(dd2.x), "+v"(dd2.y), "+v"(dd2.z), "+v"(dd2.w));
            auto class_of = [&](const uint4 &dd, int mm, bool need, uint32_t &b0, uint32_t &b1) {
                const int cl = (mm >> 3) & 7;
                b0 = ((cl < 4 ? dd.z : dd.w) >> (8 * (cl & 3))) & 255u;
                b1 = cl >= 7 ? (dd.x & 127u) : ((((cl + 1) < 4 ? dd.z : dd.w) >> (8 * ((cl + 1) & 3))) & 255u);
                b1 = need ? min(b1, 64u) : 0u;
                b0 = need ? b0 : 0u;
            };
            const int mm1 = (int) (y1 & 255u) - d1, mm2 = (int) (y2 & 255u) - d2;
            uint32_t e1, e1_end, e2, e2_end;
            class_of(dd1, mm1, need1, e1, e1_end);
            class_of(dd2, mm2, need2, e2, e2_end);
            do {
                uint32_t cx1[PP_TAIL_K], cz1[PP_TAIL_K], cx2[PP_TAIL_K], cz2[PP_TAIL_K];
#pragma unroll
                for (int i = 0; i < PP_TAIL_K; i++) {
                    const uint4 *c1 = side + min((uint64_t) dd1.y + e1 + (uint32_t) i, last), *c2 = side + min((uint64_t) dd2.y + e2 + (uint32_t) i, last);
                    cx1[i] = c1->x; cz1[i] = c1->z; cx2[i] = c2->x; cz2[i] = c2->z;
                }
                static_assert(PP_TAIL_K == 4, "the batch is pinned word by word");
                asm volatile("" : "+v"(cx1[0]), "+v"(cz1[0]), "+v"(cx1[1]), "+v"(cz1[1]), "+v"(cx1[2]), "+v"(cz1[2]), "+v"(cx1[3]), "+v"(cz1[3]),
                                  "+v"(cx2[0]), "+v"(cz2[0]), "+v"(cx2[1]), "+v"(cz2[1]), "+v"(cx2[2]), "+v"(cz2[2]), "+v"(cx2[3]), "+v"(cz2[3]));
#pragma unroll
                for (int i = 0; i < PP_TAIL_K; i++) {
                    if (e1 + (uint32_t) i < e1_end && (int) ((cz1[i] >> 8) & 63u) == mm1 && ((cz1[i] >> 16) & 3u) == g1) lk_id1 = cx1[i];
                    if (e2 + (uint32_t) i < e2_end && (int) ((cz2[i] >> 8) & 63u) == mm2 && ((cz2[i] >> 16) & 3u) == g2) lk_id2 = cx2[i];
                }
                e1 += PP_TAIL_K; e2 += PP_TAIL_K;
            } while (__ballot(e1 < e1_end || e2 < e2_end) != 0ull);
        }
    }
    unsigned long long slot_val = LOCAL_FIRST_NONE;
    if (active && !dfr && nkept > 0) {
        const int d1 = __builtin_ctzll(kept);
        int p1_home = 0;
#pragma unroll
        for (int k = 0; k < CL_RMAX; k++) p1_home = (((vmask >> k) & 1u) != 0u && ((ry[k] >> 8) & 255u) == 0u) ? (int) ((ry[k] >> 16) & 255u) : p1_home;
        const bool by_succ = d1 < p1_home && (int) (my.z & 255u) == d1 && my.y != 0xFFFFFFFFu;
        const uint32_t id1 = by_succ ? my.y : (TAIL ? lk_id1 : lookup(d1));
        uint32_t id2 = 0u;
        int d2 = 0;
        bool two = false;
        if (nkept == 2) {
            d2 = 63 - __clzll((long long) kept);
            id2 = TAIL ? lk_id2 : lookup(d2);
            const int ds0 = U - cfg.rsoemo + 1;
            const unsigned long long lowm = ds0 <= 0 ? 0ull : (ds0 >= 64 ? ~0ull : ((1ull << ds0) - 1ull));
            two = d2 < ds0 || __popcll(occ & ((1ull << d2) - 1ull) & ~lowm) < 3;
        }
        if (id1 == 0xFFFFFFFFu || (nkept == 2 && id2 == 0xFFFFFFFFu)) dfr = true;
        else {
            slot_val = ((unsigned long long) id1 << 32) | (uint32_t) d1 | (two ? 0x100u : 0u);
            if (two) o.second[Bs - o.src_base] = ((unsigned long long) id2 << 32) | (uint32_t) d2;
            st_rec += two ? 2 : 1;
        }
    }
    if (have) o.first[Bs - o.src_base] = slot_val;
    dfr = dfr && nr_code != 0;
    const uint64_t dm = __ballot(dfr);
    if (dm != 0ull) {
        if (dfr) sDefer[wave][n_defer + (int) __builtin_amdgcn_mbcnt_hi((uint32_t) (dm >> 32), __builtin_amdgcn_mbcnt_lo((uint32_t) dm, 0u))] = Bs;
        n_defer += __popcll(dm);
        wave_lds_fence();
        if (n_defer >= 64) flush_defer();
    }
    }
    flush_defer();
    st_rec = wave_sum_u64(st_rec);
    if (lane == 0 && st_rec) atomicAdd(&o.counters[CNT_VALID_RECORDS], (unsigned long long) st_rec);
}

__global__ void __launch_bounds__(256) k_pile_deg(int32_t n, unsigned long long *__restrict__ first, uint32_t *__restrict__ deg, const unsigned long long *__restrict__ pile_cnt) {
    if (pile_declines(pile_cnt)) return;
    const int64_t i = (int64_t) blockIdx.x * 256 + threadIdx.x;
    if (i >= n) return;
    const unsigned long long f = first[i];
    if (f == LOCAL_FIRST_NONE || deg[i] != 0u) return;
    deg[i] = 1u + (uint32_t) ((f >> 8) & 1ull);
    if (f & 0x100ull) first[i] = f & ~0x100ull;
}

bool pile_plan(const PrefSufCfg &cfg, const ClusterCfg &cc, int eq, int uniform_len, bool masks) {
    if (eq != PILE_EQ || uniform_len <= 0 || masks || cfg.stats) return false;
    if (uniform_len > 144 || blocks_of(uniform_len) > 9) return false;
    if (uniform_len - cfg.Lmin + 1 > 64 || cc.w > 64 || cc.w < 16 || cc.kk > 32 || cc.kk < 1) return false;
    return true;
}
size_t pile_record_bytes(uint64_t n) { return (size_t) (n + 2) * 64; }

size_t pile_table_bytes(uint32_t n_buckets) { return ((size_t) n_buckets + 2) * 128; }

__global__ void k_pile_sample_close(unsigned long long *__restrict__ pile_cnt) {
    const unsigned long long by_entries = pile_cnt[2] / 8ull;
    if (by_entries > pile_cnt[0]) pile_cnt[0] = by_entries;
}

__global__ void k_pile_sample_force(unsigned long long *__restrict__ pile_cnt, unsigned long long buckets, unsigned long long irregular) { pile_cnt[0] = buckets; pile_cnt[1] = irregular; }

void launch_pile_sample(const NodesDev &nd, const ClusterCfg &cc, int uniform_len, const uint32_t *skeys, const uint32_t *sids, const void *dir, unsigned long long *pile_cnt,
                        int no_sample, hipStream_t s, bool from_keys) {
    (void) hipMemsetAsync(pile_cnt, 0, PILE_CNT_WORDS * sizeof(unsigned long long), s);
    const uint64_t n_entries = nd.n > 0 ? (uint64_t) nd.n : 0;
    if (no_sample == 2) hipLaunchKernelGGL(k_pile_sample_force, dim3(1), dim3(1), 0, s, pile_cnt, 100ull, 1ull);
    if (n_entries == 0 || no_sample) return;
    const uint64_t tiles = (n_entries + PB_TILE - 1) / PB_TILE;
    const dim3 sample((unsigned) std::max<uint64_t>(1, std::min<uint64_t>(tiles, std::max<uint64_t>(64, tiles / 32)))), block(PB_THREADS);
    hipLaunchKernelGGL((from_keys ? k_pile_build<true, true> : k_pile_build<true, false>), sample, block, 0, s, nd, skeys, sids, n_entries, (const uint4 *) dir, cc, uniform_len, (uint4 *) nullptr,
                       (uint4 *) nullptr, 0u, (uint4 *) nullptr, pile_cnt, (uint32_t *) nullptr, (uint32_t *) nullptr, (uint32_t *) nullptr, (unsigned long long *) nullptr, 0u);
    hipLaunchKernelGGL(k_pile_sample_close, dim3(1), dim3(1), 0, s, pile_cnt);
}

void launch_pile_build(const NodesDev &nd, const PrefSufCfg &cfg, const ClusterCfg &cc, int uniform_len, const uint32_t *skeys, const uint32_t *sids, const void *dir, void *rec, void *rec2,
                       void *tab, uint32_t epoch, void *side, const void *runs, int nwin, const unsigned long long *pile_cnt, uint32_t *own_mask, void *plist, hipStream_t s,
                       bool from_keys, unsigned long long *bad_flag, bool full_record, bool runs_ahead) {
    const uint64_t n_entries = nd.n > 0 ? (uint64_t) nd.n : 0;
    if (n_entries == 0) return;
    const uint64_t tiles = (n_entries + PB_TILE - 1) / PB_TILE;
    if (!own_mask) plist = nullptr;
    uint32_t *pl = (uint32_t *) plist, *pc = pl ? pl + tiles * PB_THREADS : nullptr;
    if (own_mask) (void) hipMemsetAsync(own_mask, 0, pile_own_mask_bytes(n_entries), s);
    hipLaunchKernelGGL((from_keys ? k_pile_build<false, true> : k_pile_build<false, false>), dim3((unsigned) tiles), dim3(PB_THREADS), 0, s, nd, skeys, sids, n_entries, (const uint4 *) dir, cc, uniform_len,
                       (uint4 *) rec, (uint4 *) tab, epoch, (uint4 *) side, const_cast<unsigned long long *>(pile_cnt), own_mask, pl, pc, bad_flag, full_record ? 1u : 0u);
    if (pl)
        hipLaunchKernelGGL(k_pile_runs_consensus_list, dim3((unsigned) ((tiles + PR_SEGS - 1) / PR_SEGS)), dim3(TK_ROWS), 0, s, (const uint32_t *) pl, (const uint32_t *) pc, (uint32_t) tiles,
                           (const uint4 *) side, n_entries, (uint4 *) tab, (const uint4 *) rec, (uint4 *) rec2, cc, uniform_len, cfg.Lmin, pile_cnt, own_mask, runs_ahead ? 1 : 0);
    else if (own_mask)
        hipLaunchKernelGGL(k_pile_runs_consensus, dim3((unsigned) ((n_entries + PR_TILE - 1) / PR_TILE)), dim3(TK_ROWS), 0, s, (const uint4 *) side, n_entries, cc.n_buckets, (uint4 *) tab,
                           (const uint4 *) rec, (uint4 *) rec2, cc, uniform_len, cfg.Lmin, pile_cnt, own_mask);
    else
        hipLaunchKernelGGL(k_pile_runs, dim3((unsigned) ((n_entries + 255) / 256)), dim3(256), 0, s, (const uint4 *) side, n_entries, cc.n_buckets, (uint4 *) tab, (const uint2 *) runs, nd.n, nwin, pile_cnt);
}

size_t pile_own_mask_bytes(uint64_t n) { return (size_t) ((n + 31) / 32 + 1024) * 4; }

size_t pile_list_bytes(uint64_t n) { const uint64_t tiles = (n + PB_TILE - 1) / PB_TILE; return (size_t) (tiles * (PB_THREADS + 1) + 64) * 4; }

void launch_pile_own_ids(const uint32_t *own_mask, const uint32_t *sids, uint64_t n_entries, int32_t *list, uint32_t cap, unsigned long long *pile_cnt, hipStream_t s) {
    if (n_entries == 0) return;
    const uint64_t words = (n_entries + 31) / 32;
    hipLaunchKernelGGL(k_pile_own_ids, dim3((unsigned) ((words + 1023) / 1024)), dim3(256), 0, s, own_mask, sids, n_entries, list, cap, pile_cnt + 3, (const unsigned long long *) pile_cnt);
}

void launch_pile_check(const void *side, uint64_t n_entries, uint32_t n_buckets, const void *tab, const void *rec2, uint32_t epoch, const void *runs, int n_nodes, int nwin,
                       unsigned long long *pile_cnt, hipStream_t s) {
    if (n_entries == 0) return;
    hipLaunchKernelGGL(k_pile_list_check, dim3((unsigned) ((n_entries + 255) / 256)), dim3(256), 0, s, (const uint4 *) side, n_entries, n_buckets, (const uint4 *) tab, (const uint4 *) rec2, epoch,
                       (const uint2 *) runs,
                       n_nodes, nwin, pile_cnt + 4, (const unsigned long long *) pile_cnt);
}

constexpr int PSR_IPT = 4;
__global__ void __launch_bounds__(256) k_pile_side_range(const uint4 *__restrict__ side, uint64_t n_entries, uint32_t src_begin, uint32_t src_end, uint4 *__restrict__ out,
                                                         uint64_t out_cap, unsigned long long *__restrict__ cursor, const unsigned long long *__restrict__ pile_cnt) {
    if (pile_declines(pile_cnt)) return;
    __shared__ uint32_t cnt[PSR_IPT * 4];
    __shared__ unsigned long long base;
    const int wave = (int) (threadIdx.x >> 6);
    const uint64_t b0 = (uint64_t) blockIdx.x * (256 * PSR_IPT);
    uint4 v[PSR_IPT];
    uint32_t before[PSR_IPT];
    bool in[PSR_IPT];
#pragma unroll
    for (int k = 0; k < PSR_IPT; k++) {
        const uint64_t j = b0 + (uint64_t) k * 256 + threadIdx.x;
        v[k] = j < n_entries ? side[j] : make_uint4(0xFFFFFFFFu, 0u, 0u, 0u);
        in[k] = j < n_entries && v[k].x >= src_begin && v[k].x < src_end;
        const uint64_t m = __ballot(in[k]);
        before[k] = (uint32_t) __builtin_amdgcn_mbcnt_hi((uint32_t) (m >> 32), __builtin_amdgcn_mbcnt_lo((uint32_t) m, 0u));
        if ((threadIdx.x & 63u) == 0u) cnt[k * 4 + wave] = (uint32_t) __popcll(m);
    }
    __syncthreads();
    if (threadIdx.x == 0) {
        uint32_t tot = 0;
        for (int i = 0; i < PSR_IPT * 4; i++) tot += cnt[i];
        base = tot ? atomicAdd(cursor, (unsigned long long) tot) : 0ull;
    }
    __syncthreads();
    uint32_t run = 0;
#pragma unroll
    for (int k = 0; k < PSR_IPT; k++) {
        uint32_t mine = run;
        for (int w = 0; w < 4; w++) { if (w < wave) mine += cnt[k * 4 + w]; run += cnt[k * 4 + w]; }
        const unsigned long long at = base + mine + before[k];
        if (in[k] && at < out_cap) out[at] = v[k];
    }
}

void launch_pile_probe(const NodesDev &nd, const PrefSufCfg &cfg, const ClusterCfg &cc, int uniform_len, const void *tab, uint32_t epoch, const void *rec, const void *rec2,
                       const void *side, const void *runs, unsigned long long *counters, uint32_t *deg, unsigned long long *first, unsigned long long *second,
                       int32_t *defer_list, uint32_t defer_cap, const unsigned long long *pile_cnt, int n_cu, hipStream_t s, int32_t src_begin, int32_t src_end,
                       void *side_range, unsigned long long *cursor, bool lean, bool tail) {
    const uint64_t n_entries = nd.n > 0 ? (uint64_t) nd.n : 0;
    if (n_entries == 0 || src_end <= src_begin) return;
    ProbeOut o{};
    o.counters = counters; o.deg = deg; o.first = first; o.second = second; o.src_base = src_begin;
    uint64_t n_mine = n_entries;
    const void *side_src = side;
    if (src_begin != 0 || src_end != nd.n) {
        n_mine = (uint64_t) (src_end - src_begin);
        (void) hipMemsetAsync(cursor, 0, sizeof(unsigned long long), s);
        hipLaunchKernelGGL(k_pile_side_range, dim3((unsigned) ((n_entries + 256 * PSR_IPT - 1) / (256 * PSR_IPT))), dim3(256), 0, s, (const uint4 *) side, n_entries,
                           (uint32_t) src_begin, (uint32_t) src_end, (uint4 *) side_range, n_mine, cursor, pile_cnt);
        side_src = side_range;
    }
    const uint64_t tiles = (n_mine + PP_WAVES * 64 - 1) / (PP_WAVES * 64);
    const dim3 grid((unsigned) std::max<uint64_t>(1, std::min<uint64_t>(tiles, (uint64_t) std::max(1, n_cu) * (PP_OCC * 4 / PP_WAVES)))), block(PP_WAVES * 64);
    hipLaunchKernelGGL((lean ? (tail ? k_pile_probe<true, true> : k_pile_probe<true, false>) : k_pile_probe<false, false>), grid, block, 0, s, cfg, cc, uniform_len, nd, n_entries, n_mine, nd.n, (const uint4 *) tab, epoch, (const uint4 *) rec, (const uint4 *) rec2,
                       (const uint4 *) side, (const uint4 *) side_src, (const uint2 *) runs, o, defer_list, defer_cap, pile_cnt);
}

void launch_pile_deg(int32_t n, unsigned long long *first, uint32_t *deg, const unsigned long long *pile_cnt, hipStream_t s) {
    if (n <= 0) return;
    hipLaunchKernelGGL(k_pile_deg, dim3((unsigned) (((int64_t) n + 255) / 256)), dim3(256), 0, s, n, first, deg, pile_cnt);
}

}
```

Baseline: 5.655 billion edges/s.

## Encode source degree in first-slot words to skip degree array memset and reads

When the pile path is pure, the full memset of the out-degree array is skipped. Only deferred sources get their degree zeroed, and their degree is folded back into the first-slot word afterwards. The fused emit scan and pile_deg kernels then derive each source's degree from the first-slot encoding instead of reading a separate degree array. This removes a full-array memset and a full-array read in the emit pass, but adds two small list kernels and a more complex slot encoding that deferred and irregular sources must handle correctly.

```diff
diff --git a/alga_amd/csrc/engine.hip b/alga_amd/csrc/engine.hip
--- a/alga_amd/csrc/engine.hip
+++ b/alga_amd/csrc/engine.hip
@@ -136,6 +136,7 @@
     e->store_timed = false;
     e->pile_timed = false;
     e->pile_deg_pending = false;
+    e->emit_slots = false;
     const bool all_sources = src_begin == 0 && src_end == pp.nd.n;
     const bool pile_index_left = e->opt_pile_range != 0 && e->pile_n == pp.nd.n && e->pile_words == (const void *) pp.nd.words;
     bool pile = clustered && e->opt_pile != 0 && e->opt_cluster_pairs != 0 && e->opt_cluster_order != 0 && pp.local_sw == 1 &&
@@ -279,9 +280,13 @@
     const uint32_t big_list_cap = 1u << 20;
     if (local && (rc = alga_ensure(e, e->loc_big_list, big_list_cap * sizeof(int32_t)))) return rc;
     bool pure_streamed = false;
+    const bool emit_slots = local && clustered && e->opt_emit_slots != 0 && e->opt_emit_fused != 0 && e->opt_pile_deg_fold != 0 && e->opt_pile_stream_by_id == 0 &&
+                            e->opt_cluster_pairs && pp.local_sw == 1 && pp.cluster_eq <= 4 && pile && e->pile_n == nd.n && e->pile_words == (const void *) nd.words;
+    e->emit_slots = emit_slots;
     for (int attempt = 0; attempt < 4; attempt++) {
         if (cap >= (1ull << 32) - 16) return alga_fail(e, ALGA_ERR_CAPACITY, "more than 2^32 overlap records; shard the input");
-        if (local) HIP_TRY(e, hipMemsetAsync(e->outdeg.p, 0, (size_t) (n_src + 1) * sizeof(uint32_t), s));
+        if (emit_slots) launch_deg_fill_unless_pure((uint32_t *) e->outdeg.p, n_src + 1, (const unsigned long long *) e->cl_pile_cnt.p, s);
+        else if (local) HIP_TRY(e, hipMemsetAsync(e->outdeg.p, 0, (size_t) (n_src + 1) * sizeof(uint32_t), s));
         if ((rc = alga_ensure(e, e->rec_dst, cap * sizeof(uint32_t)))) return rc;
         if ((rc = alga_ensure(e, e->rec_val, cap * sizeof(unsigned long long)))) return rc;
         HIP_TRY(e, hipMemsetAsync(cnt, 0, CNT_TOTAL * sizeof(unsigned long long), s));
@@ -309,6 +314,9 @@
                     if (keys_only)
                         launch_cluster_runs_list(nd, cfg, cc, (const int32_t *) e->cl_defer.p, cnt + CNT_DEFERRED, (uint32_t) std::min<uint64_t>(n_src + 64, 0xFFFFFFFFull),
                                                  (uint32_t) e->n_cu * 16u, e->cl_runs.p, (uint8_t *) e->cl_nruns.p, s);
+                    if (emit_slots)
+                        launch_zero_deg_list((const int32_t *) e->cl_defer.p, cnt + CNT_DEFERRED, (uint32_t) std::min<uint64_t>(n_src + 64, 0xFFFFFFFFull), src_begin, (uint32_t) n_src,
+                                             (uint32_t *) e->outdeg.p, (const unsigned long long *) e->cl_pile_cnt.p, s);
                 }
                 launch_probe_stream(nd, cfg, cc, pp.cluster_eq, e->cl_store.p, e->cl_dir.p, e->cl_runs.p, (const uint8_t *) e->cl_nruns.p,
                                     src_begin, src_end, by_key, cnt, e->n_cu, (uint32_t *) e->outdeg.p, (unsigned long long *) e->loc_first.p,
@@ -333,6 +341,9 @@
                                        (piled && e->opt_pile_skip_gather) ? (const unsigned long long *) e->cl_pile_cnt.p : nullptr,
                                        (piled && e->pile_tab_index) ? e->cl_pile_tab.p : nullptr, e->pile_epoch);
                 e->pile_deg_pending = piled && e->opt_pile_deg_fold != 0;
+                if (emit_slots)
+                    launch_fold_deg_list((const int32_t *) e->cl_defer.p, cnt + CNT_DEFERRED, (uint32_t) std::min<uint64_t>(n_src + 64, 0xFFFFFFFFull), src_begin, (uint32_t) n_src,
+                                         (const uint32_t *) e->outdeg.p, (unsigned long long *) e->loc_first.p, (const unsigned long long *) e->cl_pile_cnt.p, s);
                 if (piled && !e->pile_deg_pending) launch_pile_deg((int32_t) n_src, (unsigned long long *) e->loc_first.p, (uint32_t *) e->outdeg.p, (const unsigned long long *) e->cl_pile_cnt.p, s);
             } else {
                 launch_probe_clustered(nd, cfg, cc, pp.cluster_eq, e->cl_store.p, e->cl_dir.p, e->cl_runs.p, (const uint8_t *) e->cl_nruns.p, src_begin,
@@ -362,7 +373,7 @@
             big.items = e->loc_big_items.p;
             if (!have_table && (rc = build_table())) return rc;
             if (e->pile_deg_pending) {
-                launch_pile_deg((int32_t) n_src, (unsigned long long *) e->loc_first.p, (uint32_t *) e->outdeg.p, (const unsigned long long *) e->cl_pile_cnt.p, s);
+                launch_pile_deg((int32_t) n_src, (unsigned long long *) e->loc_first.p, (uint32_t *) e->outdeg.p, (const unsigned long long *) e->cl_pile_cnt.p, s, emit_slots);
                 e->pile_deg_pending = false;
             }
             HIP_TRY(e, hipMemsetAsync(cnt + CNT_LOCAL_OVERFLOW, 0, sizeof(unsigned long long), s));
@@ -503,6 +514,7 @@
             launch_exclusive_scan((const uint32_t *) e->outdeg.p, n_src, (uint32_t *) e->out_rowptr.p, (uint64_t *) e->scan_scratch.p, s);
         if ((rc = alga_check_launch(e, "scan(outdeg)"))) return rc;
     }
+    const bool by_slot = fused && e->emit_slots && e->pile_deg_pending;
     e->pile_deg_pending = false;
     const uint64_t E = e->stats.records;
     if (E >= (1ull << 32) - 16) return alga_fail(e, ALGA_ERR_CAPACITY, "more than 2^32 edges; shard the input");
@@ -511,7 +523,7 @@
                       e->loc_second_used ? (const unsigned long long *) e->loc_second.p : nullptr, (const uint32_t *) e->rec_dst.p, (const unsigned long long *) e->rec_val.p, n_rec, (uint32_t *) e->out_rowptr.p,
                       (uint32_t *) e->out_cnt.p, (alga_edge_dev *) e->edges.p,
                       e->defer_list_valid ? (const int32_t *) e->cl_defer.p : nullptr, (const unsigned long long *) e->counters.p + CNT_DEFERRED, (uint32_t) n_src, s,
-                      e->loc_second_used ? e->loc_slot_stride : 0u, fused ? (uint64_t *) e->scan_scratch.p : nullptr, fused ? pile_cnt : nullptr);
+                      e->loc_second_used ? e->loc_slot_stride : 0u, fused ? (uint64_t *) e->scan_scratch.p : nullptr, fused ? pile_cnt : nullptr, by_slot);
     if ((rc = alga_check_launch(e, "k_local_emit"))) return rc;
     HIP_TRY(e, hipEventRecord(e->ev[EV_EMIT], s));
     uint64_t *d_total = (uint64_t *) e->scan_scratch.p + scan_total_index(n_src);
@@ -658,6 +670,8 @@
         e->opt_pile_deg_fold = value != 0;
     } else if (!strcmp(name, "emit_fused")) {
         e->opt_emit_fused = value != 0;
+    } else if (!strcmp(name, "emit_slots")) {
+        e->opt_emit_slots = value != 0;
     } else if (!strcmp(name, "pile_probe_lean")) {
         e->opt_pile_probe_lean = value != 0;
     } else if (!strcmp(name, "pile_probe_tail")) {
diff --git a/alga_amd/csrc/engine_internal.h b/alga_amd/csrc/engine_internal.h
--- a/alga_amd/csrc/engine_internal.h
+++ b/alga_amd/csrc/engine_internal.h
@@ -67,6 +67,8 @@
     int    opt_pile_probe_tail = 1;
     int    opt_pile_runs_ahead = 0;
     bool   pile_deg_pending = false;
+    int    opt_emit_slots = 1;
+    bool   emit_slots = false;
     int    opt_pile_check = 0;
     bool   expect_pairwise = false;
     DevBuf cl_pile_side_r, cl_pile_cursor;
diff --git a/alga_amd/csrc/prefsuf_cluster_device.h b/alga_amd/csrc/prefsuf_cluster_device.h
--- a/alga_amd/csrc/prefsuf_cluster_device.h
+++ b/alga_amd/csrc/prefsuf_cluster_device.h
@@ -46,6 +46,9 @@
 __device__ __forceinline__ bool pile_cnt_declines(const unsigned long long *c) { return c[1] * PILE_DECLINE_ONE_IN > c[0]; }
 __device__ __forceinline__ bool pile_cnt_mixed(const unsigned long long *c) { return !pile_cnt_declines(c) && c[1] * PILE_IRREGULAR_ONE_IN > c[0]; }
 __device__ __forceinline__ bool pile_cnt_pure(const unsigned long long *c) { return !pile_cnt_declines(c) && !pile_cnt_mixed(c); }
+constexpr unsigned long long SLOT_DEG_MASK = 0x300ull;
+__device__ __forceinline__ bool slot_bears_no_edge(unsigned long long f) { return (uint32_t) (f >> 32) == 0xFFFFFFFFu; }
+__device__ __forceinline__ uint32_t slot_degree(unsigned long long f) { return slot_bears_no_edge(f) ? (uint32_t) f + 1u : 1u + (uint32_t) ((f & SLOT_DEG_MASK) >> 8); }
 struct BucketIndex {
     const uint4 *tab;
     uint32_t epoch;
diff --git a/alga_amd/csrc/prefsuf_kernels.h b/alga_amd/csrc/prefsuf_kernels.h
--- a/alga_amd/csrc/prefsuf_kernels.h
+++ b/alga_amd/csrc/prefsuf_kernels.h
@@ -32,7 +32,13 @@
 void launch_local_emit(int32_t src_base, int32_t n_src, const uint32_t *deg, const unsigned long long *first, const unsigned long long *second,
                        const uint32_t *rec_dst, const unsigned long long *rec_val, uint64_t n_rec, uint32_t *rowptr, uint32_t *cursor,
                        alga_edge_dev *edges, const int32_t *record_sources, const unsigned long long *record_sources_count, uint32_t record_sources_cap, hipStream_t s, uint32_t slot_stride = 0,
-                       uint64_t *fused_scratch = nullptr, const unsigned long long *pile_cnt = nullptr);
+                       uint64_t *fused_scratch = nullptr, const unsigned long long *pile_cnt = nullptr,
+                       bool slots = false );
+void launch_deg_fill_unless_pure(uint32_t *deg, uint64_t n, const unsigned long long *pile_cnt, hipStream_t s);
+void launch_zero_deg_list(const int32_t *list, const unsigned long long *count , uint32_t cap, int32_t src_base, uint32_t n_src, uint32_t *deg, const unsigned long long *pile_cnt,
+                          hipStream_t s);
+void launch_fold_deg_list(const int32_t *list, const unsigned long long *count , uint32_t cap, int32_t src_base, uint32_t n_src, const uint32_t *deg, unsigned long long *first,
+                          const unsigned long long *pile_cnt, hipStream_t s);
 
 bool       cluster_plan(const PrefSufCfg &cfg, int max_len, uint64_t live, int bucket_log2_bias, ClusterCfg *c, int *eq);
 size_t     cluster_sort_temp_bytes(uint64_t n);
@@ -66,7 +72,8 @@
                                unsigned long long *counters, int n_cu, uint32_t *deg, unsigned long long *first, unsigned long long *second, int32_t *defer_list,
                                uint32_t defer_cap, const unsigned long long *pile_cnt ,
                                hipStream_t s, uint32_t slot_stride = 0 );
-void       launch_pile_deg(int32_t n, unsigned long long *first, uint32_t *deg, const unsigned long long *pile_cnt, hipStream_t s);
+void       launch_pile_deg(int32_t n, unsigned long long *first, uint32_t *deg, const unsigned long long *pile_cnt, hipStream_t s,
+                           bool slots = false );
 bool       pile_plan(const PrefSufCfg &cfg, const ClusterCfg &cc, int eq, int uniform_len, bool masks);
 size_t     pile_record_bytes(uint64_t n);
 size_t     pile_table_bytes(uint32_t n_buckets);
diff --git a/alga_amd/csrc/prefsuf_kernels.hip b/alga_amd/csrc/prefsuf_kernels.hip
--- a/alga_amd/csrc/prefsuf_kernels.hip
+++ b/alga_amd/csrc/prefsuf_kernels.hip
@@ -957,12 +957,28 @@
 }
 
 __global__ void __launch_bounds__(SCAN_BLOCK) k_emit_tile_sums(const uint32_t *__restrict__ deg, const unsigned long long *__restrict__ first, uint64_t n,
-                                                                const unsigned long long *__restrict__ pile_cnt, uint64_t *__restrict__ tile_sums) {
+                                                                const unsigned long long *__restrict__ pile_cnt, uint64_t *__restrict__ tile_sums, uint32_t slots) {
     __shared__ uint32_t lds[8];
     const bool piled = pile_cnt != nullptr && !pile_cnt_declines(pile_cnt);
+    const bool by_slot = slots != 0u && pile_cnt != nullptr && pile_cnt_pure(pile_cnt);
     const uint64_t base = (uint64_t) blockIdx.x * SCAN_TILE;
     uint32_t s = 0;
-    if (base + SCAN_TILE <= n && (reinterpret_cast<uintptr_t>(deg) & 15u) == 0 && (reinterpret_cast<uintptr_t>(first) & 15u) == 0) {
+    if (by_slot) {
+        if (base + SCAN_TILE <= n && (reinterpret_cast<uintptr_t>(first) & 15u) == 0) {
+            constexpr int G = SCAN_ITEMS / 2;
+            const ulonglong2 *f2 = reinterpret_cast<const ulonglong2 *>(first + base);
+            ulonglong2 v[G];
+#pragma unroll
+            for (int k = 0; k < G; k++) v[k] = f2[k * SCAN_BLOCK + threadIdx.x];
+#pragma unroll
+            for (int k = 0; k < G; k++) s += slot_degree(v[k].x) + slot_degree(v[k].y);
+        } else {
+            for (int k = 0; k < SCAN_ITEMS; k++) {
+                const uint64_t i = base + (uint64_t) k * SCAN_BLOCK + threadIdx.x;
+                if (i < n) s += slot_degree(first[i]);
+            }
+        }
+    } else if (base + SCAN_TILE <= n && (reinterpret_cast<uintptr_t>(deg) & 15u) == 0 && (reinterpret_cast<uintptr_t>(first) & 15u) == 0) {
         constexpr int G = SCAN_ITEMS / 4;
         const uint4 *d4 = reinterpret_cast<const uint4 *>(deg + base);
         const ulonglong2 *f2 = reinterpret_cast<const ulonglong2 *>(first + base);
@@ -1012,23 +1028,35 @@
 __global__ void __launch_bounds__(SCAN_BLOCK) k_emit_scan_tiles(int32_t src_base, uint64_t n, const uint32_t *__restrict__ deg, const unsigned long long *__restrict__ first,
                                                                  const unsigned long long *__restrict__ second, const unsigned long long *__restrict__ pile_cnt,
                                                                  const uint64_t *__restrict__ tile_sums, uint32_t *__restrict__ out, alga_edge_dev *__restrict__ edges,
-                                                                 uint32_t slot_stride) {
+                                                                 uint32_t slot_stride, uint32_t slots) {
     __shared__ uint32_t lds[8];
     const bool piled = pile_cnt != nullptr && !pile_cnt_declines(pile_cnt);
+    const bool by_slot = slots != 0u && pile_cnt != nullptr && pile_cnt_pure(pile_cnt);
     const int lane = lane_id(), wave = (int) (threadIdx.x >> 6);
     const uint64_t wbase = (uint64_t) blockIdx.x * SCAN_TILE + (uint64_t) wave * (64 * SCAN_ITEMS) + (uint64_t) lane;
     uint32_t d[SCAN_ITEMS];
     unsigned long long f[SCAN_ITEMS];
-#pragma unroll
-    for (int k = 0; k < SCAN_ITEMS; k++) { const uint64_t i = wbase + 64u * k; d[k] = i < n ? deg[i] : 0u; }
-#pragma unroll
-    for (int k = 0; k < SCAN_ITEMS; k++) { const uint64_t i = wbase + 64u * k; f[k] = (i < n && (piled || d[k] != 0u)) ? first[i] : LOCAL_FIRST_NONE; }
     uint32_t sum = 0;
-#pragma unroll
-    for (int k = 0; k < SCAN_ITEMS; k++) {
-        const uint32_t dk = source_degree(d[k], piled, f[k]);
-        if (d[k] == 0u && dk != 0u) f[k] &= 0xFFFFFFFF000000FFull;
-        d[k] = dk; sum += dk;
+    if (by_slot) {
+#pragma unroll
+        for (int k = 0; k < SCAN_ITEMS; k++) { const uint64_t i = wbase + 64u * k; f[k] = i < n ? first[i] : LOCAL_FIRST_NONE; }
+#pragma unroll
+        for (int k = 0; k < SCAN_ITEMS; k++) {
+            d[k] = slot_degree(f[k]);
+            f[k] = slot_bears_no_edge(f[k]) ? LOCAL_FIRST_NONE : (f[k] & ~SLOT_DEG_MASK);
+            sum += d[k];
+        }
+    } else {
+#pragma unroll
+        for (int k = 0; k < SCAN_ITEMS; k++) { const uint64_t i = wbase + 64u * k; d[k] = i < n ? deg[i] : 0u; }
+#pragma unroll
+        for (int k = 0; k < SCAN_ITEMS; k++) { const uint64_t i = wbase + 64u * k; f[k] = (i < n && (piled || d[k] != 0u)) ? first[i] : LOCAL_FIRST_NONE; }
+#pragma unroll
+        for (int k = 0; k < SCAN_ITEMS; k++) {
+            const uint32_t dk = source_degree(d[k], piled, f[k]);
+            if (d[k] == 0u && dk != 0u) f[k] &= 0xFFFFFFFF000000FFull;
+            d[k] = dk; sum += dk;
+        }
     }
     sum = (uint32_t) wave_sum_u64(sum);
     if (lane == 0) lds[wave] = sum;
@@ -1056,6 +1084,44 @@
     unsigned long long m = *count;
     if (m > (unsigned long long) cap) m = cap;
     for (unsigned long long q = (unsigned long long) blockIdx.x * blockDim.x + threadIdx.x; q < m; q += (unsigned long long) gridDim.x * blockDim.x) cursor[list[q] - src_base] = 0u;
+}
+
+__global__ void __launch_bounds__(256) k_deg_fill_unless_pure(uint32_t *__restrict__ deg, uint64_t n, const unsigned long long *__restrict__ pile_cnt) {
+    if (pile_cnt_pure(pile_cnt)) return;
+    const uint64_t n4 = n / 4u;
+    uint4 *d4 = reinterpret_cast<uint4 *>(deg);
+    for (uint64_t i = (uint64_t) blockIdx.x * blockDim.x + threadIdx.x; i < n4; i += (uint64_t) gridDim.x * blockDim.x) d4[i] = make_uint4(0u, 0u, 0u, 0u);
+    if (blockIdx.x == 0 && 4u * n4 + threadIdx.x < n) deg[4u * n4 + threadIdx.x] = 0u;
+}
+
+__global__ void __launch_bounds__(256) k_zero_deg_list(const int32_t *__restrict__ list, const unsigned long long *__restrict__ count, uint32_t cap, int32_t src_base, uint32_t n_src,
+                                                        uint32_t *__restrict__ deg, const unsigned long long *__restrict__ pile_cnt) {
+    if (!pile_cnt_pure(pile_cnt)) return;
+    unsigned long long m = *count;
+    if (m > (unsigned long long) cap) m = cap;
+    for (unsigned long long q = (unsigned long long) blockIdx.x * blockDim.x + threadIdx.x; q < m; q += (unsigned long long) gridDim.x * blockDim.x) {
+        const uint32_t a = (uint32_t) (list[q] - src_base);
+        if (a < n_src) deg[a] = 0u;
+    }
+}
+
+__global__ void __launch_bounds__(256) k_fold_deg_list(const int32_t *__restrict__ list, const unsigned long long *__restrict__ count, uint32_t cap, int32_t src_base, uint32_t n_src,
+                                                        const uint32_t *__restrict__ deg, unsigned long long *__restrict__ first, const unsigned long long *__restrict__ pile_cnt) {
+    if (!pile_cnt_pure(pile_cnt)) return;
+    unsigned long long m = *count;
+    if (m > (unsigned long long) cap) m = cap;
+    for (unsigned long long q = (unsigned long long) blockIdx.x * blockDim.x + threadIdx.x; q < m; q += (unsigned long long) gridDim.x * blockDim.x) {
+        const uint32_t a = (uint32_t) (list[q] - src_base);
+        if (a >= n_src) continue;
+        const uint32_t dg = deg[a];
+        const unsigned long long f = first[a];
+        unsigned long long v = LOCAL_FIRST_NONE;
+        if (dg != 0u) {
+            if (slot_bears_no_edge(f)) v = 0xFFFFFFFF00000000ull | (unsigned long long) (dg - 1u);
+            else v = (f & ~SLOT_DEG_MASK) | ((unsigned long long) (min(dg, (uint32_t) LOCAL_SLOTS_MAX) - 1u) << 8);
+        }
+        first[a] = v;
+    }
 }
 
 __global__ void __launch_bounds__(256) k_sort_rows_list(const int32_t *__restrict__ list, const unsigned long long *__restrict__ count, uint32_t cap, int32_t src_base,
@@ -1273,7 +1339,7 @@
 void launch_local_emit(int32_t src_base, int32_t n_src, const uint32_t *deg, const unsigned long long *first, const unsigned long long *second,
                        const uint32_t *rec_dst, const unsigned long long *rec_val, uint64_t n_rec, uint32_t *rowptr, uint32_t *cursor,
                        alga_edge_dev *edges, const int32_t *record_sources, const unsigned long long *record_sources_count, uint32_t record_sources_cap, hipStream_t s,
-                       uint32_t slot_stride, uint64_t *fused_scratch, const unsigned long long *pile_cnt) {
+                       uint32_t slot_stride, uint64_t *fused_scratch, const unsigned long long *pile_cnt, bool slots) {
     if (n_src <= 0) {
         if (fused_scratch) launch_exclusive_scan(deg, 0, rowptr, fused_scratch, s);
         return;
@@ -1283,10 +1349,11 @@
     else (void) hipMemsetAsync(cursor, 0, (size_t) (n_src + 1) * sizeof(uint32_t), s);
     if (fused_scratch) {
         const uint32_t tiles = (uint32_t) (((uint64_t) n_src + SCAN_TILE - 1) / SCAN_TILE);
-        hipLaunchKernelGGL(k_emit_tile_sums, dim3(tiles), dim3(SCAN_BLOCK), 0, s, deg, first, (uint64_t) n_src, pile_cnt, fused_scratch);
+        const uint32_t by_slot = (slots && pile_cnt != nullptr) ? 1u : 0u;
+        hipLaunchKernelGGL(k_emit_tile_sums, dim3(tiles), dim3(SCAN_BLOCK), 0, s, deg, first, (uint64_t) n_src, pile_cnt, fused_scratch, by_slot);
         hipLaunchKernelGGL(k_scan_spine_serial, dim3(1), dim3(1024), 0, s, fused_scratch, tiles);
         hipLaunchKernelGGL(k_emit_scan_tiles, dim3(tiles), dim3(SCAN_BLOCK), 0, s, src_base, (uint64_t) n_src, deg, first, second, pile_cnt, (const uint64_t *) fused_scratch, rowptr, edges,
-                           slot_stride);
+                           slot_stride, by_slot);
     } else hipLaunchKernelGGL(k_local_emit_first, dim3(grid_for((uint64_t) n_src, 256)), dim3(256), 0, s, src_base, n_src, deg, first, second, (const uint32_t *) rowptr, edges, slot_stride);
     if (n_rec) {
         unsigned g = std::min<unsigned>(grid_for(n_rec, 256), 4096u);
@@ -1296,6 +1363,24 @@
         if (n_rec) hipLaunchKernelGGL(k_sort_rows_list, dim3(std::min<unsigned>(grid_for((uint64_t) record_sources_cap, 256), 2048u)), dim3(256), 0, s, record_sources, record_sources_count,
                                       record_sources_cap, src_base, rowptr, edges);
     } else hipLaunchKernelGGL(k_sort_rows, dim3(grid_for((uint64_t) n_src, 256)), dim3(256), 0, s, n_src, rowptr, edges);
+}
+
+void launch_deg_fill_unless_pure(uint32_t *deg, uint64_t n, const unsigned long long *pile_cnt, hipStream_t s) {
+    if (n == 0) return;
+    if ((reinterpret_cast<uintptr_t>(deg) & 15u) != 0) { (void) hipMemsetAsync(deg, 0, (size_t) n * sizeof(uint32_t), s); return; }
+    hipLaunchKernelGGL(k_deg_fill_unless_pure, dim3(std::max(1u, std::min<unsigned>(grid_for(n / 4, 256), 4096u))), dim3(256), 0, s, deg, n, pile_cnt);
+}
+
+void launch_zero_deg_list(const int32_t *list, const unsigned long long *count, uint32_t cap, int32_t src_base, uint32_t n_src, uint32_t *deg, const unsigned long long *pile_cnt,
+                          hipStream_t s) {
+    if (n_src == 0) return;
+    hipLaunchKernelGGL(k_zero_deg_list, dim3(std::max(1u, std::min<unsigned>(grid_for((uint64_t) cap, 256), 2048u))), dim3(256), 0, s, list, count, cap, src_base, n_src, deg, pile_cnt);
+}
+
+void launch_fold_deg_list(const int32_t *list, const unsigned long long *count, uint32_t cap, int32_t src_base, uint32_t n_src, const uint32_t *deg, unsigned long long *first,
+                          const unsigned long long *pile_cnt, hipStream_t s) {
+    if (n_src == 0) return;
+    hipLaunchKernelGGL(k_fold_deg_list, dim3(std::max(1u, std::min<unsigned>(grid_for((uint64_t) cap, 256), 2048u))), dim3(256), 0, s, list, count, cap, src_base, n_src, deg, first, pile_cnt);
 }
 
 void launch_make_keys(const uint32_t *rec_dst, uint64_t n_rec, int32_t dst_begin, int32_t dst_end, uint32_t *keys,
diff --git a/alga_amd/csrc/prefsuf_pile.hip b/alga_amd/csrc/prefsuf_pile.hip
--- a/alga_amd/csrc/prefsuf_pile.hip
+++ b/alga_amd/csrc/prefsuf_pile.hip
@@ -1047,11 +1047,18 @@
     if (lane == 0 && st_rec) atomicAdd(&o.counters[CNT_VALID_RECORDS], (unsigned long long) st_rec);
 }
 
-__global__ void __launch_bounds__(256) k_pile_deg(int32_t n, unsigned long long *__restrict__ first, uint32_t *__restrict__ deg, const unsigned long long *__restrict__ pile_cnt) {
+__global__ void __launch_bounds__(256) k_pile_deg(int32_t n, unsigned long long *__restrict__ first, uint32_t *__restrict__ deg, const unsigned long long *__restrict__ pile_cnt,
+                                                   uint32_t slots) {
     if (pile_declines(pile_cnt)) return;
     const int64_t i = (int64_t) blockIdx.x * 256 + threadIdx.x;
     if (i >= n) return;
     const unsigned long long f = first[i];
+    if (slots != 0u && pile_cnt_pure(pile_cnt)) {
+        deg[i] = slot_degree(f);
+        const unsigned long long g = slot_bears_no_edge(f) ? LOCAL_FIRST_NONE : (f & ~SLOT_DEG_MASK);
+        if (g != f) first[i] = g;
+        return;
+    }
     if (f == LOCAL_FIRST_NONE || deg[i] != 0u) return;
     deg[i] = 1u + (uint32_t) ((f >> 8) & 1ull);
     if (f & 0x100ull) first[i] = f & ~0x100ull;
@@ -1186,9 +1193,9 @@
                        (const uint4 *) side, (const uint4 *) side_src, (const uint2 *) runs, o, defer_list, defer_cap, pile_cnt);
 }
 
-void launch_pile_deg(int32_t n, unsigned long long *first, uint32_t *deg, const unsigned long long *pile_cnt, hipStream_t s) {
+void launch_pile_deg(int32_t n, unsigned long long *first, uint32_t *deg, const unsigned long long *pile_cnt, hipStream_t s, bool slots) {
     if (n <= 0) return;
-    hipLaunchKernelGGL(k_pile_deg, dim3((unsigned) (((int64_t) n + 255) / 256)), dim3(256), 0, s, n, first, deg, pile_cnt);
-}
-
-}
+    hipLaunchKernelGGL(k_pile_deg, dim3((unsigned) (((int64_t) n + 255) / 256)), dim3(256), 0, s, n, first, deg, pile_cnt, slots ? 1u : 0u);
+}
+
+}
```

After: 5.638 billion edges/s. Within noise of the previous version (-0.3%).
